# alex-petrenko/sample-factory

Hardware: AMD Instinct MI355X
Metric: env-steps/sec (whole node), 4096 envs, 84x84x4 obs (higher is better)
Workload: dtype f32

## Files before the change

### include/sf_hip.h

```cpp
#ifndef SF_HIP_H
#define SF_HIP_H

#include <stdint.h>

#ifdef __cplusplus
extern "C" {
#endif

#define SF_OK 0
#define SF_ERR_ARG (-1)
#define SF_ERR_LAUNCH (-2)
#define SF_ERR_UNSUPPORTED (-3)
#define SF_MAX_ACTION_HEADS 64

const char *sf_last_error(void);
int sf_abi_version(void);

int sf_valid_mask(const int32_t *policy_id, const float *policy_version, uint8_t *valids, uint8_t *valids_flat,
                  float *actions, int num_actions, float *log_prob_actions, int E, int T, int my_policy_id,
                  int train_step, int max_policy_lag, int32_t *num_invalid, void *stream);

int sf_gae_returns(float *rewards, const uint8_t *dones, const uint8_t *time_outs, const float *values,
                   const uint8_t *valids, const double *rms_stats, int E, int T, float gamma, float gae_lambda,
                   int value_bootstrap, float *advantages, float *returns, void *stream);
// ... 197 lines not shown
                       int R, int Cn, int H, int env_major, void *stream);

#define SF_DP_UNIQUE_ID_BYTES 128
int sf_dp_unique_id(void *out_id);
int sf_dp_comm_create(const void *id_bytes, int nranks, int rank, void **comm_out);
int sf_dp_comm_destroy(void *comm);
int sf_dp_comm_info(void *comm, int *nranks, int *rank);
int sf_allreduce_grads(void *comm, float *grads, int64_t n, void *stream);
int sf_dp_allreduce_f64(void *comm, double *buf, int64_t n, int op, void *stream);
int sf_dp_broadcast(void *comm, void *buf, int64_t nbytes, int root, void *stream);

#define SF_DP_IPC_HANDLE_BYTES 64
int sf_dp_oneshot_create(int nranks, int rank, int64_t max_bytes, void **ctx_out, void *handle_out);
int sf_dp_oneshot_connect(void *ctx, const void *all_handles );
int sf_dp_oneshot_allreduce_f32(void *ctx, float *buf, int64_t n, void *stream);
int sf_dp_oneshot_allreduce_f64(void *ctx, double *buf, int64_t n, int op, void *stream);
int sf_dp_oneshot_status(void *ctx);
int sf_dp_oneshot_destroy(void *ctx);

int sf_tanh_scale_fwd(float *x, int ld, int64_t n, int col0, int ncols, float scale, void *stream);
int sf_tanh_scale_bwd(float *g, const float *y, int ld, int64_t n, int col0, int ncols, float scale, void *stream);

int sf_linear_fwd_dual_supported(int64_t n, int N, int K1, int K2);
int sf_linear_fwd_dual(const float *a1, int64_t lda1, const float *w1t, const float *bias1, int K1, const float *a2,
                       int64_t lda2, const float *w2t, const float *bias2, int K2, float *out, int64_t n, int N,
                       int gru_H, void *stream);

int sf_conv_fwd_t_supported(int64_t n, const sf_conv_desc *desc);
int64_t sf_conv_fwd_t_workspace(int64_t n, const sf_conv_desc *desc);
int sf_conv_fwd_t(const float *in, int64_t in_sample_stride, const float *wt, const float *bias, float *out,
                  int64_t n, const sf_conv_desc *desc, void *workspace, int64_t workspace_bytes, void *stream);
int sf_transpose(const float *w, float *wt, int K, int N, void *stream);

int sf_conv_kernel_name(int op, int64_t n, const sf_conv_desc *desc, int split_k_allowed, char *out, int cap);
int sf_linear_fwd(const float *in, const float *w, const float *bias, float *out, int64_t M, int K, int N, int relu,
                  void *stream);
int64_t sf_linear_wgrad_workspace(int64_t M, int K, int N);
int sf_linear_wgrad(const float *in, const float *dout, float *dw, float *db, int64_t M, int K, int N,
                    void *workspace, void *stream);
int sf_linear_dgrad(const float *dout, const float *w, const float *in_act, float *din, int64_t M, int K, int N,
                    void *stream);
int sf_relu_mask(float *g, const float *act, int64_t n, void *stream);

typedef struct {
    int32_t Cin, H, W, Cout;
    int32_t in_u8;
    int32_t act_in;
    int32_t traj_T;
    float sub_mean, inv_scale;
} sf_res_desc;

int sf_res_conv_fwd(const void *in, int64_t in_sample_stride, const int32_t *index, int64_t offset, const float *w,
                    const float *bias, const float *residual, float *out, float *out_act, int act_out, int64_t n,
                    const sf_res_desc *h_desc, void *stream);
int sf_res_conv_fwd_norm(const void *in, int64_t in_sample_stride, const int32_t *index, int64_t offset, const float *mu,
                         const float *rstd, const float *w, const float *bias, float *out, int64_t n,
                         const sf_res_desc *h_desc, void *stream);
int sf_res_pool_fwd(const float *in, float *out, uint8_t *argmax, int64_t n, int H, int W, int C, void *stream);
int sf_res_pool_bwd(const float *dout, const uint8_t *argmax, float *din, int64_t n, int H, int W, int C, void *stream);
int sf_res_conv_dgrad(const float *dout, const float *w, const float *pre, const float *g_add, float *din, int64_t n,
                      const sf_res_desc *h_desc, void *stream);
int64_t sf_res_conv_wgrad_workspace(int64_t n, const sf_res_desc *h_desc);
int sf_res_conv_wgrad(const void *in, int64_t in_sample_stride, const int32_t *index, int64_t offset, const float *dout,
                      float *dw, float *db, int64_t n, const sf_res_desc *h_desc, void *workspace,
                      int64_t workspace_bytes, void *stream);
int sf_res_conv_wgrad_norm(const void *in, int64_t in_sample_stride, const int32_t *index, int64_t offset, const float *mu,
// ... 8 lines not shown
```

### sample_factory_amd/algo/learning/learner.py

```python
from __future__ import annotations

import glob
import time
import os
from os.path import join
from typing import Dict, List, Optional, Tuple

import numpy as np
import torch

from sample_factory_amd import lib
from sample_factory_amd.algo.learning.dp import ReplicaGroup
from sample_factory_amd.algo.utils.tensor_dict import TensorDict
from sample_factory_amd.envs.spaces import (action_head_sizes, calc_num_action_parameters, calc_num_actions, is_box,
                                             is_discrete)
from sample_factory_amd.model.actor_critic import ActorCritic
from sample_factory_amd.model.model_factory import create_actor_critic
from sample_factory_amd.utils.attr_dict import AttrDict
from sample_factory_amd.utils.decay import LinearDecay

LEARNER_ENV_STEPS, POLICY_ID_KEY, STATS_KEY, TRAIN_STATS = "learner_env_steps", "policy_id", "stats", "train"


class LearningRateScheduler:
# ... 81 lines not shown

    def init(self, actor_critic, policy_version, device):
        self.actor_critic, self.device = actor_critic, device
        self.policy_versions[self.policy_id] = policy_version


class Learner:
    def __init__(self, cfg, env_info, policy_versions_tensor: torch.Tensor, policy_id: int, param_server,
                 process_group=None):
        self.cfg = cfg
        self.env_info = env_info
        self.policy_id = policy_id
        self.policy_versions_tensor = policy_versions_tensor
        self.param_server = param_server
        self.device: Optional[torch.device] = None
        self.actor_critic: Optional[ActorCritic] = None
        self.curr_lr: Optional[float] = None
        self.lr_scheduler: Optional[LearningRateScheduler] = None
        self.train_step = 0
        self.env_steps = 0
        self.best_performance = -1e9
        self.new_cfg: Optional[Dict] = None
        self.policy_to_load = None
        self.is_initialized = False
        self.last_summary: Dict = {}
        self.pg = process_group
        dp_on = process_group is not None or (getattr(cfg, "data_parallel", False) and torch.distributed.is_initialized())
        self.group = ReplicaGroup(process_group, bool(getattr(cfg, "dp_force_collectives", False)),
                                  bool(getattr(cfg, "dp_native_rccl", False)),
                                  oneshot_bytes=int(getattr(cfg, "dp_oneshot_bytes", 0) or 0)) if dp_on else None
        self.world = self.group.world if self.group is not None else 1
        self.dp = self.group is not None and self.group.on
        self._grad_norms: List[float] = []

    def _all_reduce(self, t: torch.Tensor) -> None:
        if self.dp:
            self.group.all_reduce_sum(t)

    def init(self):
        cfg = self.cfg
        if cfg.exploration_loss not in ("entropy", "symmetric_kl"):
            raise NotImplementedError(f"{cfg.exploration_loss} not supported!")
        if cfg.optimizer not in ("adam", "lamb"):
            raise RuntimeError(f"Unknown optimizer {cfg.optimizer}")
        if cfg.seed is not None:
            torch.manual_seed(cfg.seed)
            np.random.seed(cfg.seed)
        if not torch.cuda.is_available():
            raise lib.SfHipError("Learner.init(): no GPU visible. sample_factory_amd has no CPU path.")
        lib.load()
        self.device = torch.device("cuda", torch.cuda.current_device())
        ar = self._all_reduce if self.dp else None
        cfg.dp_world = self.world
        self.actor_critic = create_actor_critic(cfg, self.env_info.obs_space, self.env_info.action_space, self.device,
                                                all_reduce=ar)
        self.actor_critic.train()
        if self.dp:
            self.group.broadcast(self.actor_critic.flat_params, src=0)
            self.actor_critic.params_changed()
        P = self.actor_critic.num_flat
        self.exp_avg = torch.zeros(P, dtype=torch.float32, device=self.device)
        self.exp_avg_sq = torch.zeros(P, dtype=torch.float32, device=self.device)
        self.adam_step_count = 0
        self._dp_reduce_each_mb = True
        self._dp_split = None
        ac_ = self.actor_critic
# ... 216 lines not shown
            idx = torch.empty(experience_size, dtype=torch.int32, device=self.device)
            if getattr(cfg, "device_shuffle", False):
                seed = (cfg.seed or 0) * 7919 + self.policy_id
                lib.minibatch_indices(idx, experience_size, cfg.recurrence, True, seed, self._shuffle_epoch)
                self._shuffle_epoch += 1
            else:
                starts = np.random.permutation(np.arange(0, experience_size, cfg.recurrence))
                starts_dev = torch.from_numpy(starts.astype(np.int32)).to(self.device, non_blocking=True)
                lib.minibatch_expand(starts_dev, idx, experience_size, cfg.recurrence)
            return [(idx[i * batch_size:(i + 1) * batch_size], 0, batch_size) for i in range(experience_size // batch_size)]
        return [(None, i * batch_size, batch_size) for i in range(n_mb)]

    _shuffle_epoch = 0

    def _calculate_losses(self, mb: AttrDict, num_invalids: int):
        from sample_factory_amd.algo.utils.action_distributions import get_action_distribution
        buff, part = (mb if isinstance(mb, tuple) else (mb, None))
        if part is None:
            part = (None, 0, buff.E * buff.T)
        acts, g_heads, sc = self._losses_native(buff, part, num_invalids)
        index, offset, n = part
        heads = acts[-1]
        A = self.num_action_params
        space = self.env_info.action_space
        dist = get_action_distribution(space, heads[:n, 1:1 + A])
        dist.raw_logits, dist.values = heads[:n, 1:1 + A], heads[:n, 0]
        rows = index.long() if index is not None else torch.arange(offset, offset + n, device=self.device)
        kl_old = dist.kl_divergence(get_action_distribution(space, buff.action_logits[rows]))[buff.valids[rows]]
        summaries = AttrDict(adv_mean=sc[6], adv_std=sc[7], num_valid=sc[8], entropy=sc[9], kl_divergence_max=sc[5],
                             kl_old_mean=sc[4].clone(), ratio=self._ratio[:n], values=heads[:n, 0], g_heads=g_heads)
        return dist, sc[0].clone(), sc[1].clone(), kl_old, sc[2].clone(), sc[3].clone(), summaries

    def _losses_native(self, buff: AttrDict, mb, num_invalids: int, scalars_out: Optional[torch.Tensor] = None,
                       moments: Optional[torch.Tensor] = None):
        cfg, ac = self.cfg, self.actor_critic
        index, offset, n = mb
        A = self.num_action_params
        rnn = None
        if cfg.use_rnn:
            R, Cn = cfg.recurrence, n // cfg.recurrence
            keep_tm = ac._buf(("rnn", "keep_tm"), (R, Cn))
            h0 = ac._buf(("rnn", "h0"), (Cn, buff.rnn_states.shape[-1]))
            lib.rnn_chunk_setup(buff.dones, buff.valids, buff.rnn_states, index, offset, Cn, R, keep_tm, h0, traj_T=buff.T)
            rnn = dict(R=R, h0=h0, keep_tm=keep_tm)
        acts = ac.forward_heads(buff.obs, n, sample_stride=ac.obs_elems, index=index, offset=offset,
                                traj_T=buff.T, tag="train", rnn=rnn)
        heads = acts[-1]
        ld = ac.heads_ld
        params, values = heads[:, 1:], heads[:, 0]
        g_heads = ac._zbuf(("g", "heads"), (n, ld))
        if cfg.with_vtrace:
            vs = ac._buf(("vt", "vs"), (n,))
            adv = ac._buf(("vt", "adv"), (n,))
            lib.vtrace(params, ld, values, ld, buff.actions, buff.log_prob_actions, buff.rewards, buff.dones, index,
                       offset, n, A, self.loss_cfg.action_kind, cfg.recurrence, cfg.gamma, cfg.vtrace_rho,
                       cfg.vtrace_c, vs, adv, head_sizes=self._head_sizes)
            lib.moments(adv, buff.valids, index, n, self._moments, offset=offset, dense_x=True)
            adv_arr, tgt_arr = adv, vs
        elif moments is None:
            lib.moments(buff.advantages, buff.valids, index, n, self._moments, offset=offset)
            adv_arr, tgt_arr = buff.advantages, buff.returns
        else:
            adv_arr, tgt_arr = buff.advantages, buff.returns
        if moments is None:
            moments = self._moments
            self._all_reduce(moments)
        self._ratio = ac._buf(("loss", "ratio"), (n,))
        self.loss_cfg.old_values_T = buff.T
        lib.ppo_loss(params, ld, values, ld, buff.actions, buff.log_prob_actions, buff.action_logits, buff["values"],
                     adv_arr, tgt_arr, buff.valids, index, offset, n, A, self.loss_cfg, moments, self._sums,
                     g_heads[:, 1:], g_heads[:, 0], ratio_out=self._ratio, head_sizes=self._head_sizes)
        self._last_mb = (index, offset, n, values, adv_arr)
        if self.dp and self._dp_reduce_each_mb:
            self.group.loss_sums(self._sums)
        out = scalars_out if scalars_out is not None else torch.zeros(16, dtype=torch.float32, device=self.device)
        lib.loss_scalars(self._sums, moments, self.loss_cfg, out)
        return acts, g_heads, out

    def _epoch_moments(self, buff: AttrDict, minibatches) -> Optional[torch.Tensor]:
# ... 1 lines not shown
            return None
        tab = self.actor_critic._buf(("loss", "epoch_moments"), (len(minibatches), 3), dtype=torch.float64)
        for i, (index, offset, n) in enumerate(minibatches):
            lib.moments(buff.advantages, buff.valids, index, n, tab[i], offset=offset)
        self._all_reduce(tab)
        return tab

    def _train(self, buff: AttrDict, batch_size: int, experience_size: int, num_invalids: int) -> Optional[AttrDict]:
        cfg, ac = self.cfg, self.actor_critic
        early_stopping_tolerance = 1e-6
        prev_epoch_actor_loss = 1e9
        recent_kls: List[float] = []
        num_sgd_steps = 0
        n_mb = cfg.num_batches_per_epoch
        self._scalars = ac._buf(("loss", "scalars"), (cfg.num_epochs * n_mb, 16))
        global_size = experience_size * self.world
        need_kl_each_mb = self.lr_scheduler.invoke_after_each_minibatch() and isinstance(self.lr_scheduler, KlAdaptiveScheduler)
        self._dp_reduce_each_mb = need_kl_each_mb
        lr_on_device = need_kl_each_mb and cfg.optimizer == "adam"
        if lr_on_device:
            if not hasattr(self, "_lr_dev"):
                self._lr_dev = torch.zeros(1, dtype=torch.float32, device=self.device)
            self._lr_dev.fill_(float(self.curr_lr))
        self._grad_norms = []
        skip = ac.rnn_abort_word() if hasattr(ac, "rnn_abort_word") else None
        if skip is not None:
            ac.rnn_abort_clear()
        for epoch in range(cfg.num_epochs):
            minibatches = self._get_minibatches(batch_size, experience_size)
            mom_tab = self._epoch_moments(buff, minibatches)
            for batch_num, mb in enumerate(minibatches):
                row = self._scalars[epoch * n_mb + batch_num]
                acts, g_heads, _ = self._losses_native(buff, mb, num_invalids, row,
                                                       moments=None if mom_tab is None else mom_tab[batch_num])
                index, offset, n = mb
                if self._dp_split is not None:
                    cut = ac._segs[self._dp_split][0]
                    pending = []
                    ac.backward(acts, g_heads, buff.obs, n, sample_stride=ac.obs_elems, index=index, offset=offset,
                                traj_T=buff.T,
                                on_layer_done=lambda li: pending.append(self.group.all_reduce_grads_async(
                                    ac.flat_grads[cut:])) if li == self._dp_split else None)
                    self.group.all_reduce_grads(ac.flat_grads[:cut])
                    for work in pending:
                        work.wait()
                else:
                    ac.backward(acts, g_heads, buff.obs, n, sample_stride=ac.obs_elems, index=index, offset=offset,
                                traj_T=buff.T)
                    if self.dp:
                        self.group.all_reduce_grads(ac.flat_grads)
                actual_lr = self.curr_lr
                valid_frac = 1.0
                if self._global_invalids > 0:
                    valid_frac = (global_size - self._global_invalids) / global_size
                    actual_lr = self.curr_lr * valid_frac
                self.adam_step_count += 1
                use_clip = cfg.max_grad_norm > 0.0
                if use_clip or getattr(cfg, "record_grad_norm", False):
                    lib.grad_sumsq(ac.flat_grads, self._sumsq)
                    if getattr(cfg, "record_grad_norm", False):
                        self._grad_norms.append(float(self._sumsq.sqrt().item()))
                if cfg.optimizer == "lamb":
                    if self._lamb is None:
                        seg, nseg = ac.tensor_segment_ids()
                        self._lamb = (seg, nseg, torch.empty_like(ac.flat_params),
                                      torch.zeros(128, dtype=torch.float64, device=self.device))
                    seg, nseg, scratch, seg_sums = self._lamb
# ... 110 lines not shown
```

### sample_factory_amd/algo/sampling/batched_sampling.py

```python
from __future__ import annotations

import ctypes as C
import time
from typing import Dict, Optional

import numpy as np
import torch

from sample_factory_amd import lib
from sample_factory_amd.algo.utils.tensor_dict import TensorDict
from sample_factory_amd.envs.spaces import action_head_sizes, heads_mixed, is_box, split_tuple_actions


class BatchedVectorEnvRunner:
    def __init__(self, cfg, env_info, env, actor_critic, traj: TensorDict, policy_id: int = 0,
                 policy_versions: Optional[torch.Tensor] = None, sample_seed: int = 0, row0: int = 0, tag: str = "inf"):
        self.cfg, self.env_info, self.env, self.ac = cfg, env_info, env, actor_critic
        self.tag = tag
        self.traj = traj
        self.policy_id = policy_id
        self.policy_versions = policy_versions
        self.B = env.num_agents
        self.T = cfg.rollout
        dev = actor_critic.device
# ... 4 lines not shown
        self.env_actions = torch.zeros((self.B, len(self.heads)) if len(self.heads) > 1 else self.B, dtype=torch.int32,
                                       device=dev)
        self.ep_return = torch.zeros(self.B, dtype=torch.float32, device=dev)
        self.ep_len = torch.zeros(self.B, dtype=torch.int32, device=dev)
        self.ep_stats = torch.zeros(3, dtype=torch.float64, device=dev)
        self.sample_seed = int(sample_seed)
        self.row0 = int(row0)
        self.global_step = 0
        self.obs_keys = sorted(k for k in traj["obs"].keys() if k != "action_mask")
        self.multi_key = len(self.obs_keys) > 1
        self.zero_copy = hasattr(env, "step_into") and not self.multi_key
        self.obs = traj["obs"]["obs" if "obs" in traj["obs"] else self.obs_keys[0]]
        self.rnn = actor_critic.rnn_kind is not None
        traj["rnn_states"].zero_()
        self._dummy_state_rows = {traj["rnn_states"].data_ptr()}
        self._started = False
        self.A = actor_critic.num_action_params
        self.ld = actor_critic.heads_ld
        self.continuous = is_box(self.env_info.action_space)
        self.host_env = None
        self.async_env = hasattr(env, "step_async") and hasattr(env, "step_wait")
        self._pin, self._pin_flip, self._direct_ok = {}, {}, {}
        self._act_event = torch.cuda.Event()
        self.h2d_bytes = 0
        self.ingest_prof: Optional[dict] = None
        self._rew = torch.zeros(self.B, dtype=torch.float32, device=dev)
        self._term = torch.zeros(self.B, dtype=torch.bool, device=dev)
        self._trunc = torch.zeros(self.B, dtype=torch.bool, device=dev)
        self._c_step, self._c_ver = C.c_uint32(0), C.c_float(0.0)
        self._progs: Dict = {}
        self._progs_layout = None
        self.program_replays = 0
        self._launch_key = getattr(actor_critic, "launch_key", None) if lib.LAUNCH_PROGRAMS else None
        self.masked = "action_mask" in traj["obs"]
        if self.masked and (self.continuous or len(self.heads) != 1):
            raise NotImplementedError("action masks are supported for a single Discrete action space")
        if self.masked and self.zero_copy:
            raise NotImplementedError("action masks with a zero-copy (step_into) env")

    def reset(self) -> None:
        if self.zero_copy:
            self.env.reset_into(self.obs[:, 0])
        else:
            o, _ = self.env.reset()
            first = (o["obs"] if "obs" in o else o[self.obs_keys[0]]) if isinstance(o, dict) else o
            self.host_env = not (isinstance(first, torch.Tensor) and first.is_cuda)
            self._store_obs(o, 0)
        self._started = True

    def _pinned(self, key, shape, dtype, nbuf=1):
        bufs = self._pin.get(key)
        if bufs is None or bufs[0].shape != torch.Size(shape) or bufs[0].dtype != dtype:
            bufs = [torch.empty(shape, dtype=dtype, pin_memory=True) for _ in range(nbuf)]
            self._pin[key] = bufs
        self._pin_flip[key] = (self._pin_flip.get(key, -1) + 1) % len(bufs)
        return bufs[self._pin_flip[key]]

    def _to_device(self, key, src, dst: torch.Tensor) -> None:
        if isinstance(src, torch.Tensor) and src.is_cuda:
            dst.copy_(src)
            return
        prof = self.ingest_prof
        t0 = time.perf_counter() if prof is not None else 0.0
        a = np.asarray(src.cpu() if isinstance(src, torch.Tensor) else src)
        stage = None
        if getattr(self.env, "pages_registered", False) and isinstance(src, np.ndarray) and src.flags.c_contiguous and \
# ... 59 lines not shown
        self.rollout_step_finish(t)

    def _program(self, half: str, t: int, extra=()):
        if self._launch_key is None:
            return None, None
        layout, weights = self._launch_key(self.tag)
        if layout != self._progs_layout:
            self._progs.clear()
            self._progs_layout = layout
        key = (half, t, self.traj["rewards"].data_ptr(), self._deterministic, torch.cuda.current_stream().cuda_stream,
               weights, extra)
        slot = self._progs.get(key)
        if slot is None:
            if len(self._progs) > 64 * self.T:
                self._progs.clear()
            self._progs[key] = False
            return None, None
        if slot is False:
            return None, key
        return (slot, None) if slot.unsafe is None else (None, None)

    def rollout_step_begin(self, t: int) -> None:
        self._c_step.value, self._c_ver.value = self.global_step & 0xFFFFFFFF, self._ver
        prog, rec_key = self._program("policy", t)
        if prog is not None:
            prog.replay()
            self.program_replays += 1
        elif rec_key is not None:
            with lib.record_launches() as prog:
                self._policy_and_sample(t)
            self._progs[rec_key] = prog
        else:
            self._policy_and_sample(t)
        tr = self.traj
        env_actions = tr["actions"][:, t] if (self.continuous or self.mixed) else self.env_actions
        if self.async_env:
            self.env.step_async(self._actions_to_host(env_actions))
            return
        self._env_step_and_record(t, env_actions)

    def _policy_and_sample(self, t: int) -> None:
        tr, T, B, A = self.traj, self.T, self.B, self.A
        ver, deterministic, cfg, step = self._c_ver, self._deterministic, self.cfg, self._c_step
        rnn = dict(states=tr["rnn_states"][:, t]) if self.rnn else None
        x = {k: tr["obs"][k][:, t] for k in self.obs_keys} if self.multi_key else self.obs[:, t]
        heads = self.ac.forward_heads(x, B, sample_stride=self.obs.stride(0), tag=self.tag, rnn=rnn)[-1]
        if self.masked:
            mk = tr["obs"]["action_mask"][:, t]
            lib.sample_write_step_masked(heads[:, 1:], self.ld, heads[:, 0], self.ld, mk, mk.stride(0), B, A, T, t,
                                         self.sample_seed, step, self.row0, ver, deterministic,
                                         tr["actions"], tr["action_logits"], tr["log_prob_actions"], tr["values"],
                                         tr["policy_version"], self.env_actions)
        elif len(self.heads) > 1:
            lib.sample_write_step_tuple(heads[:, 1:], self.ld, heads[:, 0], self.ld, B, self.heads, T, t,
                                        self.sample_seed, step, self.row0, ver, deterministic,
                                        tr["actions"], tr["action_logits"], tr["log_prob_actions"], tr["values"],
                                        tr["policy_version"], None if self.mixed else self.env_actions)
        else:
            lib.sample_write_step(heads[:, 1:], self.ld, heads[:, 0], self.ld, B, A, T, t, self.sample_seed,
                                  step, self.row0, ver, deterministic, tr["actions"],
                                  tr["action_logits"], tr["log_prob_actions"], tr["values"], tr["policy_version"],
                                  None if self.continuous else self.env_actions, action_kind=int(self.continuous))

    def rollout_step_finish(self, t: int) -> None:
        if self.async_env:
            self._env_step_and_record(t, None)

    def _env_step_and_record(self, t: int, env_actions) -> None:
        tr, T, cfg = self.traj, self.T, self.cfg
        if self.zero_copy:
            if self.mixed:
                env_actions = split_tuple_actions(env_actions, self.heads)
            rew, term, trunc = self.env.step_into(env_actions, self.obs[:, t + 1])
        else:
            if self.host_env is None:
                self.host_env = False
            t0 = time.perf_counter()
            if self.async_env:
                o, rew, term, trunc, _ = self.env.step_wait()
# ... 78 lines not shown
```

### sample_factory_amd/cfg/arguments.py

```python
from __future__ import annotations

import argparse
import os
from typing import List, Optional, Tuple


def _bool(v):
    if isinstance(v, bool):
        return v
    if v.lower() in ("true", "1", "yes", "y", "t"):
        return True
    if v.lower() in ("false", "0", "no", "n", "f"):
        return False
    raise argparse.ArgumentTypeError(f"boolean expected, got {v}")


FLAGS = [
    ("algo", str, "APPO"), ("env", str, None), ("experiment", str, "default_experiment"),
    ("train_dir", str, os.path.join(os.getcwd(), "train_dir")), ("restart_behavior", str, "resume"),
    ("device", str, "gpu"), ("seed", int, None),
    ("num_policies", int, 1), ("async_rl", _bool, True), ("serial_mode", _bool, False),
    ("batched_sampling", _bool, False), ("num_batches_to_accumulate", int, 2), ("worker_num_splits", int, 2),
    ("policy_workers_per_policy", int, 1), ("max_policy_lag", int, 1000),
    ("num_workers", int, 8), ("num_envs_per_worker", int, 2),
# ... 10 lines not shown
    ("lr_schedule_kl_threshold", float, 0.008), ("lr_adaptive_min", float, 1e-6), ("lr_adaptive_max", float, 1e-2),
    ("obs_subtract_mean", float, 0.0), ("obs_scale", float, 1.0), ("normalize_input", _bool, True),
    ("normalize_input_keys", str, None, "*"),
    ("decorrelate_experience_max_seconds", int, 0), ("decorrelate_envs_on_one_worker", _bool, True),
    ("actor_worker_gpus", int, [], "*"), ("set_workers_cpu_affinity", _bool, True),
    ("force_envs_single_thread", _bool, False), ("default_niceness", int, 0),
    ("log_to_file", _bool, True), ("experiment_summaries_interval", int, 10), ("flush_summaries_interval", int, 30),
    ("stats_avg", int, 100), ("summaries_use_frameskip", _bool, True), ("heartbeat_interval", int, 20),
    ("heartbeat_reporting_interval", int, 180),
    ("train_for_env_steps", int, int(1e10)), ("train_for_seconds", int, int(1e10)),
    ("save_every_sec", int, 120), ("keep_checkpoints", int, 2), ("load_checkpoint_kind", str, "latest"),
    ("save_milestones_sec", int, -1), ("save_best_every_sec", int, 5), ("save_best_metric", str, "reward"),
    ("save_best_after", int, 100000), ("benchmark", _bool, False),
    ("encoder_mlp_layers", int, [512, 512], "*"), ("encoder_conv_architecture", str, "convnet_simple"),
    ("encoder_conv_mlp_layers", int, [512], "*"), ("use_rnn", _bool, True), ("rnn_size", int, 512),
    ("rnn_type", str, "gru"), ("rnn_num_layers", int, 1), ("decoder_mlp_layers", int, [], "*"),
    ("nonlinearity", str, "elu"), ("policy_initialization", str, "orthogonal"), ("policy_init_gain", float, 1.0),
    ("actor_critic_share_weights", _bool, True), ("adaptive_stddev", _bool, True),
    ("continuous_tanh_scale", float, 0.0), ("initial_stddev", float, 1.0),
    ("use_env_info_cache", _bool, False), ("env_gpu_actions", _bool, False), ("env_gpu_observations", _bool, True),
    ("env_frameskip", int, 1), ("env_framestack", int, 1), ("pixel_format", str, "CHW"),
    ("use_record_episode_statistics", _bool, False), ("with_wandb", _bool, False), ("with_pbt", _bool, False),
    ("help", _bool, False),
]


ENGINE_FLAGS = [
    ("data_parallel", _bool, False),
    ("dp_overlap", _bool, True),
    ("dp_epoch_moments", _bool, True),
    ("dp_oneshot_bytes", int, 0),
    ("dp_native_rccl", _bool, False),
    ("dp_force_collectives", _bool, False),
    ("device_shuffle", _bool, False),
    ("sampler_thread", _bool, None),
    ("record_grad_norm", _bool, False),
    ("env_workers_mode", str, "auto"),
    ("env_worker_start_method", str, "spawn"),
]


def parse_sf_args(argv: Optional[List[str]] = None, evaluation: bool = False) -> Tuple[argparse.ArgumentParser, argparse.Namespace]:
    import sys

    if argv is None:
        argv = sys.argv[1:]
    p = argparse.ArgumentParser(formatter_class=argparse.ArgumentDefaultsHelpFormatter, add_help=False)
    for spec in FLAGS + ENGINE_FLAGS:
        name, typ, default = spec[:3]
        kw = dict(type=typ, default=default)
        if len(spec) > 3:
            kw["nargs"] = spec[3]
        p.add_argument(f"--{name}", **kw)
    if evaluation:
        p.add_argument("--max_num_episodes", type=int, default=int(1e9))
        p.add_argument("--max_num_frames", type=int, default=int(1e9))
        p.add_argument("--eval_deterministic", type=_bool, default=False)
        p.add_argument("--no_render", type=_bool, default=True)
        p.add_argument("--policy_index", type=int, default=0)
    args, _ = p.parse_known_args(argv)
    return p, args


def parse_full_cfg(parser: argparse.ArgumentParser, argv: Optional[List[str]] = None) -> argparse.Namespace:
    import sys

# ... 18 lines not shown
    return cfg


def preprocess_cfg(cfg, env_info) -> bool:
    if cfg.recurrence == -1:
        cfg.recurrence = cfg.rollout if cfg.use_rnn else 1
    return verify_cfg(cfg, env_info)


def verify_cfg(cfg, env_info) -> bool:
    ok = True

    def err(msg):
        nonlocal ok
        ok = False
        print(f"[sample_factory_amd] config error: {msg}")

    if cfg.num_policies != 1:
        err(f"{cfg.num_policies=}: this engine trains ONE policy per process group (multi-policy / PBT populations are "
            "outside the hot-path scope)")
    if cfg.num_envs_per_worker % cfg.worker_num_splits != 0:
        err(f"{cfg.num_envs_per_worker=} must be a multiple of {cfg.worker_num_splits=}"
            " (for double-buffered sampling you need to use even number of envs per worker)")
    if cfg.normalize_returns and cfg.with_vtrace:
        err("Normalized returns are not supported with vtrace!")
    if cfg.with_vtrace and not (cfg.recurrence == cfg.rollout and cfg.recurrence > 1):
        err("V-trace requires recurrence == rollout > 1")
    if cfg.rollout % cfg.recurrence != 0:
        err(f"{cfg.rollout=} must be a multiple of {cfg.recurrence=}")
    if cfg.batch_size % cfg.rollout != 0:
        err(f"{cfg.batch_size=} must be a multiple of {cfg.rollout=}")
    if cfg.use_rnn and cfg.recurrence <= 1:
        err("RNN policies need recurrence > 1")
    total_agents = cfg.num_workers * cfg.num_envs_per_worker * env_info.num_agents
    per_iter = cfg.num_batches_per_epoch * cfg.batch_size
    per_rollout = total_agents * cfg.rollout // cfg.num_policies
    if not cfg.async_rl and not (per_iter % per_rollout == 0 and per_iter >= per_rollout):
        err(f"sync mode needs batch_size*num_batches_per_epoch ({per_iter}) to be a multiple of "
            f"agents*rollout ({per_rollout})")
    return ok


def cfg_dict(cfg) -> dict:
    return dict(cfg) if isinstance(cfg, dict) else dict(vars(cfg))


def cfg_str(cfg) -> str:
    return "\n".join(f"{k}={v}" for k, v in cfg_dict(cfg).items())


def load_from_checkpoint(cfg):
    import json

    from sample_factory_amd.utils.attr_dict import AttrDict
    name = os.path.join(cfg.train_dir, cfg.experiment, "config.json")
    if not os.path.isfile(name):
        raise FileNotFoundError(f"Could not load saved parameters for experiment {cfg.experiment} (file {name} not found). "
                                "Check that you have the correct experiment name and --train_dir is set correctly.")
    with open(name) as f:
        loaded = AttrDict(json.load(f))
    for key, value in getattr(cfg, "cli_args", {}).items():
        if key in loaded and loaded[key] != value:
            loaded[key] = value
    for key, value in cfg_dict(cfg).items():
        if key not in loaded:
            loaded[key] = value
# ... 20 lines not shown
```

### sample_factory_amd/csrc/sf_nn.hip

```cpp
#include "sf_common.h"
#include <stdarg.h>
#include <stdlib.h>
#include <string.h>
#ifndef SF_GLDS_ABLATE
#define SF_GLDS_ABLATE 0
#endif
#include <type_traits>
#include <algorithm>

#define STREAM(s) reinterpret_cast<hipStream_t>(s)

typedef float f32x16 __attribute__((ext_vector_type(16)));

struct FastDiv {
    uint32_t d, mul, shr;
};
static inline FastDiv make_fastdiv(uint32_t d) {
    FastDiv f;
    f.d = d;
    if (d <= 1) { f.mul = 0; f.shr = 0; return f; }
    uint32_t s = 0;
    while ((1u << s) < d) ++s;
    f.mul = (uint32_t)((((uint64_t)1) << (31 + s)) / d + 1);
    f.shr = s - 1;
// ... 267 lines not shown
}

#define FRAG_ROW(r, lane) (((r) & 3) + 8 * ((r) >> 2) + 4 * ((lane) >> 5))

template <int KIND>
__device__ __forceinline__ float act_fwd_c(float x, int kind) {
    if (KIND == 0) return x;
    if (KIND == 1) return fmaxf(x, 0.f);
    return act_fwd(x, kind);
}

template <int TM, int TN, int KIND, bool FULL>
__device__ __forceinline__ void store_fwd_tile(const f32x16 (&acc)[TM][TN], float *__restrict__ ob, uint32_t voff, int N,
                                               int rows_left, int cols_left, const float *__restrict__ bias0, int lcol,
                                               int kind) {
#pragma unroll
    for (int tn = 0; tn < TN; ++tn) {
        const bool cok = FULL || tn * 32 < cols_left;
        const float bv = (bias0 && cok) ? bias0[tn * 32 + lcol] : 0.f;
#pragma unroll
        for (int tm = 0; tm < TM; ++tm)
#pragma unroll
            for (int r = 0; r < 16; ++r) {
                const int rr = tm * 32 + (r & 3) + 8 * (r >> 2);
                float *p = ob + (int64_t)rr * N + tn * 32;
                const float v = act_fwd_c<KIND>(acc[tm][tn][r] + bv, kind);
#if SF_GLDS_ABLATE & 4
                if (v == 1.2345e30f) p[voff] = v;
#else
                if (FULL || (cok && rr < rows_left)) p[voff] = v;
#endif
            }
    }
}

template <int TM, int TN, int KIND, bool FULL>
__device__ __forceinline__ void store_dgrad_tile(const f32x16 (&acc)[TM][TN], float *__restrict__ ob,
                                                 const float *__restrict__ mk, uint32_t voff, int N, int rows_left,
                                                 int cols_left, int kind) {
#pragma unroll
    for (int tn = 0; tn < TN; ++tn) {
        const bool cok = FULL || tn * 32 < cols_left;
#pragma unroll
        for (int tm = 0; tm < TM; ++tm) {
            float y[16];
#pragma unroll
            for (int r = 0; r < 16; ++r) {
                const int rr = tm * 32 + (r & 3) + 8 * (r >> 2);
                const bool ok = FULL || (cok && rr < rows_left);
                y[r] = (KIND != 0 && ok) ? (mk + (int64_t)rr * N + tn * 32)[voff] : 1.f;
            }
#pragma unroll
            for (int r = 0; r < 16; ++r) {
                const int rr = tm * 32 + (r & 3) + 8 * (r >> 2);
                const float v = act_bwd_mul<KIND>(acc[tm][tn][r], y[r], kind);
                if (FULL || (cok && rr < rows_left)) (ob + (int64_t)rr * N + tn * 32)[voff] = v;
            }
        }
    }
}


template <int BM, int BN, int WM, int WN>
struct Tile {
    static constexpr int TM = BM / WM / 32, TN = BN / WN / 32;
    static constexpr int SA = BM / 32, SB = BN / 32;
// ... 476 lines not shown
};
struct TileArgs { int BM, BN, WM, WN; };
struct ConvPlan {
    int kernel;
    char name[64];
    TileArgs t;
    int variant;
    dim3 grid, block;
    unsigned lds;
    int splits;
    int64_t per_split;
    int partials;
    int rx, ry, rtot;
    int main_tiles;
    QuadrowClasses qr;
    bool recommended;
};
static ConvPlan plan_init() {
    ConvPlan p{};
    p.block = dim3(256); p.splits = p.partials = 1;
    return p;
}
static void plan_kernel(ConvPlan &p, int kernel, const char *fmt, ...) {
    p.kernel = kernel;
    va_list ap;
    va_start(ap, fmt);
    vsnprintf(p.name, sizeof(p.name), fmt, ap);
    va_end(ap);
}
static void plan_tile(ConvPlan &p, int kernel, const char *base, TileArgs t, const char *tail = "") {
    p.t = t;
    plan_kernel(p, kernel, "%s<%d, %d, %d, %d%s>", base, t.BM, t.BN, t.WM, t.WN, tail);
}
static void plan_raster(ConvPlan &p, bool on) {
    p.rx = (int)p.grid.x; p.ry = (int)p.grid.y;
    p.rtot = on ? (int)(p.grid.x * p.grid.y * p.grid.z) : 0;
    if (p.rtot > 0) p.grid = dim3((unsigned)(8 * ((p.rtot + 7) / 8)), 1, 1);
}

struct Operands {
    const void *in;
    int64_t stride;
    bool index;
    const void *w, *dout, *out;
    int64_t ws_floats;
};
static Operands query_operands(const sf_conv_desc *d, bool split_k_workspace) {
    return Operands{nullptr, (int64_t)d->H * d->W * d->Cin, false, nullptr, nullptr, nullptr, split_k_workspace ? (int64_t)1 << 60 : 0};
}
static bool aligned(const void *p, uintptr_t a) { return ((uintptr_t)p & (a - 1)) == 0; }
static const float TABLE_PROBE[4] __attribute__((aligned(16))) = {0.f, 0.f, 0.f, 0.f};

static int pick_mode(const ConvG &g) {
    if (!g.vecA || !g.vecB) return MODE_GENERIC;
    if (in_is_u8(g.in_u8)) return g.nmu ? MODE_U8_NORM : MODE_U8;
    if (g.in_u8 == IN_F32_FRAME) return g.nmu ? MODE_F32F_NORM : MODE_F32F;
    return MODE_F32;
}

static bool act_aligned(const ConvG &g, const void *in, int64_t in_sample_stride) {
    return aligned(in, in_is_u8(g.in_u8) ? 4 : 16) && in_sample_stride % 4 == 0 && aligned(g.nmu, 16) && aligned(g.nrstd, 16);
}

static bool in4(const Operands &o) { return aligned(o.in, 4) && o.stride % 4 == 0; }
static bool tabs16(const ConvG &g) { return aligned(g.nmu, 16) && aligned(g.nrstd, 16); }

// ... 93 lines not shown
    const FwdPlan p = plan_fwd(Mtot, N, K, (int64_t)1 << 60);
    return p.splits > 1 ? (int64_t)sizeof(float) * p.splits * Mtot * N + 256 : 0;
}

#define TILE_IS(BM_, BN_) (p.t.BM == BM_ && p.t.BN == BN_)
static void launch_splitk_finish(const float *partial, const float *bias, float *out, int64_t MN, const ConvG &g, int Z, hipStream_t st) {
    k_splitk_finish<<<dim3(cdiv64(MN, 256) < 4096 ? cdiv64(MN, 256) : 4096), dim3(256), 0, st>>>(partial, bias, out, MN, g.Cout, Z, g.relu);
}
#define BY_MODE(L, ...)                                                          \
    switch (p.variant) {                                                         \
        case MODE_F32: L(__VA_ARGS__, MODE_F32); break;                          \
        case MODE_U8: L(__VA_ARGS__, MODE_U8); break;                            \
        case MODE_F32F: L(__VA_ARGS__, MODE_F32F); break;                        \
        case MODE_F32F_NORM: L(__VA_ARGS__, MODE_F32F_NORM); break;              \
        case MODE_U8_NORM: L(__VA_ARGS__, MODE_U8_NORM); break;                  \
        default: L(__VA_ARGS__, MODE_GENERIC);                                   \
    }
#define FWD_LAUNCH(BM, BN, WM, WN, MODE)                          \
    k_conv_fwd<BM, BN, WM, WN, MODE><<<p.grid, p.block, 0, st>>>( \
        g, in, in_sample_stride, index, offset, w, bias, out, Mtot, (int)p.per_split, partial)

static bool relu_mask_ok(const sf_conv_desc *d, int64_t n) {
    if (!sw().relu_mask || !in_is_u8(d->in_u8) || d->relu != 1 || d->Cout != 32) return false;
    const int k = plan_conv_fwd(d, make_geom(d), n, query_operands(d, false)).kernel;
    return k == K_CONV1_U8_BF16 || k == K_CONV1_U8_BF16_W;
}
extern "C" int sf_conv_relu_mask_supported(int64_t n, const sf_conv_desc *h_desc) {
    return h_desc && n > 0 && check_desc(h_desc, "sf_conv_relu_mask_supported") == 0 && relu_mask_ok(h_desc, n) ? 1 : 0;
}

static int conv_fwd_impl(const void *in, int64_t in_sample_stride, const int32_t *index, int64_t offset, const float *w,
                         const float *bias, float *out, uint32_t *relu_mask, int64_t n, const sf_conv_desc *h_desc,
                         void *workspace, int64_t workspace_bytes, void *stream, const float *mu = nullptr,
                         const float *rstd = nullptr) {
    int rc = check_desc(h_desc, "sf_conv_fwd");
    if (rc) return rc;
    SF_REQUIRE(in && w && out && n > 0, "sf_conv_fwd: bad args");
    SF_REQUIRE(((uintptr_t)workspace & 15) == 0, "sf_conv_fwd: workspace must be 16-byte aligned");
    ConvG g = make_geom(h_desc);
    g.nmu = mu; g.nrstd = rstd;
    const int64_t Mtot = n * g.OH * g.OW;
    SF_REQUIRE(Mtot < (1LL << 31), "sf_conv_fwd: M=%lld exceeds 2^31 rows; split the batch", (long long)Mtot);
    const Operands o = {in, in_sample_stride, index != nullptr, w, nullptr, out, workspace ? workspace_bytes / (int64_t)sizeof(float) : 0};
    const ConvPlan p = plan_conv_fwd(h_desc, g, n, o);
    hipStream_t st = STREAM(stream);
    const bool bf16 = p.kernel == K_CONV1_U8_BF16 || p.kernel == K_CONV1_U8_BF16_W;
    SF_REQUIRE(relu_mask == nullptr || bf16,
               "sf_conv_fwd_relu_mask: operands not eligible for the sign-bit kernel (sf_conv_relu_mask_supported, 4-byte "
               "aligned frames and sample stride, 16-byte aligned weights)");
    if (bf16 && sw().debug_occ) {
        const unsigned img_bytes = 2u * 4u * 20u * (unsigned)SF_CONV1_WP * (unsigned)sizeof(uint16_t);
        fprintf(stderr, "k_conv1_u8_bf16 occupancy: %d (dword stores, %u B LDS) / %d (whole-line stores, %u B LDS) work-groups per CU\n",
                occupancy_of(k_conv1_u8_bf16<false>, 256, img_bytes), img_bytes,
                occupancy_of(k_conv1_u8_bf16_w<false>, 256, img_bytes + 2u * 80u * 36u * 4u), img_bytes + 2u * 80u * 36u * 4u);
    }
    const uint8_t *in8 = reinterpret_cast<const uint8_t *>(in);
    float *partial = p.splits > 1 ? reinterpret_cast<float *>(workspace) : nullptr;
#define CONV1_LAUNCH(KERN, ...) \
    KERN<<<p.grid, p.block, p.lds, st>>>(g, in8, in_sample_stride, index, offset, w, bias, out, ##__VA_ARGS__, (int)n)
    switch (p.kernel) {
        case K_CONV1_U8_BF16_W:
            if (p.variant) CONV1_LAUNCH(k_conv1_u8_bf16_w<true>, relu_mask); else CONV1_LAUNCH(k_conv1_u8_bf16_w<false>, relu_mask);
            break;
        case K_CONV1_U8_BF16:
            if (p.variant) CONV1_LAUNCH(k_conv1_u8_bf16<true>, relu_mask); else CONV1_LAUNCH(k_conv1_u8_bf16<false>, relu_mask);
            break;
        case K_CONV_U8_IMG:
            if (p.variant) CONV1_LAUNCH((k_conv_u8_img<2, 4, 5, 16, true>)); else CONV1_LAUNCH((k_conv_u8_img<2, 4, 5, 16, false>));
            break;
        default:
            if (TILE_IS(256, 32)) { BY_MODE(FWD_LAUNCH, 256, 32, 4, 1) }
            else if (TILE_IS(128, 32)) { BY_MODE(FWD_LAUNCH, 128, 32, 4, 1) }
            else if (TILE_IS(128, 64)) { BY_MODE(FWD_LAUNCH, 128, 64, 2, 2) }
            else { BY_MODE(FWD_LAUNCH, 64, 64, 2, 2) }
            if (partial) launch_splitk_finish(partial, bias, out, Mtot * g.Cout, g, p.splits, st);
    }
#undef CONV1_LAUNCH
    return sf_launch_status("sf_conv_fwd");
}

extern "C" int sf_conv_fwd(const void *in, int64_t in_sample_stride, const int32_t *index, int64_t offset,
                           const float *w, const float *bias, float *out, int64_t n, const sf_conv_desc *h_desc,
                           void *workspace, int64_t workspace_bytes, void *stream) {
    return conv_fwd_impl(in, in_sample_stride, index, offset, w, bias, out, nullptr, n, h_desc, workspace, workspace_bytes,
                         stream);
}
extern "C" int sf_conv_fwd_relu_mask(const void *in, int64_t in_sample_stride, const int32_t *index, int64_t offset,
                                     const float *w, const float *bias, float *out, uint32_t *relu_mask, int64_t n,
                                     const sf_conv_desc *h_desc, void *stream) {
    SF_REQUIRE(relu_mask && ((uintptr_t)relu_mask & 3) == 0, "sf_conv_fwd_relu_mask: relu_mask must be a 4-byte aligned device buffer");
    SF_REQUIRE(h_desc && n > 0 && relu_mask_ok(h_desc, n) && ((uintptr_t)in & 3) == 0 && in_sample_stride % 4 == 0,
               "sf_conv_fwd_relu_mask: unsupported layer / launch (see sf_conv_relu_mask_supported)");
    return conv_fwd_impl(in, in_sample_stride, index, offset, w, bias, out, relu_mask, n, h_desc, nullptr, 0, stream);
}

#ifndef SF_IMG_TMF
#define SF_IMG_TMF 2
#endif
#define IMG_FWD_GEOMS(X) X(64, 9, 9, 3, 1, SF_IMG_TMF, 1, 7)
static int plan_img_fwd(ConvPlan &p, const ConvG &g, int64_t n) {
    if (!sw().fwd_img || g.Cout != 64 || g.KH != g.KW || n < 512) return -1;
    int idx = 0;
#define X(CIN, HH, WW, KS, ST, TMF, WS, R)                                                                         \
    if (g.Cin == CIN && g.H == HH && g.W == WW && g.KH == KS && g.S == ST) {                                       \
        static const int bpc = occupancy_of(k_fwd_img<CIN, HH, WW, KS, ST, TMF, WS, R>, 256 * WS);                 \
        p.variant = idx; p.grid = dim3(num_cus() * (bpc > 0 ? bpc : 1)); p.block = dim3(256 * WS);                 \
        plan_kernel(p, K_FWD_IMG, "k_fwd_img<%d, %d, %d, %d, %d, %d, %d, %d>", CIN, HH, WW, KS, ST, TMF, WS, R);   \
        return idx;                                                                                                \
    }                                                                                                              \
    ++idx;
    IMG_FWD_GEOMS(X)
#undef X
    return -1;
}

static bool glds_fwd_ok(const sf_conv_desc *d) {
    return d->in_u8 == IN_F32_NHWC && d->Cin % 32 == 0 && d->traj_T == 0;
}
struct GldsFwdPlan {
    bool ok, wide, sq64;
    int Z, k_per_split;
};
static int split_k(int K, int64_t want, int64_t tiles, int *k_per_split) {
    int z = (int)((want + tiles - 1) / tiles);
    z = z > K / 256 ? K / 256 : z;
    z = z > 16 ? 16 : z;
    if (z <= 1) return 1;
    *k_per_split = (((K + 31) / 32 + z - 1) / z) * 32;
    return (K + *k_per_split - 1) / *k_per_split;
}
static GldsFwdPlan plan_fwd_t(int64_t Mtot, int N, int K) {
    const Switches &s = sw();
    static const int occ64 = occupancy_of(k_fwd_glds<128, 64, 2, 2, 2>), occ128 = occupancy_of(k_fwd_glds<128, 128, 2, 2, 2>);
    GldsFwdPlan p;
// ... 15 lines not shown
        return p;
    }
    if (s.glds_fc64 == 1 && N >= 128 && K >= 1024 && cdiv64(Mtot, 64) * (int64_t)cdiv64(N, 64) >= 512) {
        p.ok = true; p.sq64 = true;
        return p;
    }
    const int64_t t6464 = cdiv64(Mtot, 64) * (int64_t)cdiv64(N, 64);
    if (s.glds_split64 && s.glds_splitk && N >= 128 && K >= 1024 && t6464 >= s.glds_split64 && t6464 < 512) {
        p.Z = split_k(K, 512, t6464, &p.k_per_split);
        if (p.Z > 1) { p.ok = true; p.sq64 = true; return p; }
    }
    if (s.glds_splitk && N >= 128 && K >= 1024 && t128 >= 32) {
        p.Z = split_k(K, 256 * occ128, t128, &p.k_per_split);
        p.ok = p.wide = p.Z > 1;
    }
    return p;
}
static bool linear_1x1(const sf_conv_desc *d) {
    return d->in_u8 == IN_F32_NHWC && d->traj_T == 0 && d->KH == 1 && d->KW == 1 && d->H == 1 && d->W == 1;
}
static bool small_linear_wgrad_ok(const sf_conv_desc *d) {
    return sw().linear_narrow && linear_1x1(d) && d->Cout <= 64 && d->Cin <= 64;
}
static bool narrow_fwd_ok(const sf_conv_desc *d, int64_t n) {
    return sw().linear_narrow && linear_1x1(d) && d->Cout <= 32 && d->Cin % 16 == 0 && n < (1 << 30);
}
static int fwd_tail_split(const ConvG &g, int64_t Mtot, int Z, bool zl_ok) {
    if (!sw().glds_tailsplit || !zl_ok || sw().glds_zl < 1 || Z != 1 || g.Cout > 64 || sw().xcd_rows) return 0;
    static const int occ = occupancy_of(k_fwd_glds_zt<128, 64, 2, 2>, 256, (128 + 64) * 32 * 2 * sizeof(float));
    const int64_t tiles = cdiv64(Mtot, 128), resident = (int64_t)num_cus() * occ, tail = tiles % resident;
    if (tiles <= resident || tail == 0 || 2 * tail > resident) return (int)tiles;
    return (int)(tiles - tail);
}
static ConvPlan plan_conv_fwd_t(const sf_conv_desc *d, int64_t n, int64_t in_sample_stride, ConvG *g_out = nullptr) {
    ConvPlan p = plan_init();
    if (narrow_fwd_ok(d, n)) {
        p.recommended = true; p.variant = d->Cout <= 16 ? 1 : 2;
        p.grid = dim3((unsigned)cdiv64(n, 16)); p.block = dim3(64);
        plan_kernel(p, K_LINEAR_NARROW, "k_linear_narrow<%d>", p.variant);
        return p;
    }
    if (!glds_fwd_ok(d)) return p;
    const ConvG g = make_geom(d);
    if (g_out) *g_out = g;
    const int64_t Mtot = n * g.OH * g.OW;
    if (n * in_sample_stride < ((int64_t)1 << 40) && plan_img_fwd(p, g, n) >= 0) { p.recommended = true; return p; }
    GldsFwdPlan q = plan_fwd_t(Mtot, g.Cout, g.K);
    p.recommended = q.ok;
    if (!q.ok) { q.Z = 1; q.k_per_split = (g.K + 31) / 32 * 32; }
    p.splits = q.Z; p.per_split = q.k_per_split;
    const bool zl_ok = sw().glds_zl && (n - 1) * in_sample_stride + (int64_t)g.H * g.W * g.Cin < (1LL << 30) &&
                       (int64_t)g.Cout * g.K < (1LL << 30);
    const bool col64 = !q.sq64 && !q.wide && q.Z == 1 && g.Cout <= 64 && zl_ok;
    if (sw().glds_persist && col64) {
        static const int occp = occupancy_of(k_fwd_glds_zp<128, 64, 2, 2>);
        const int64_t tiles = cdiv64(Mtot, 128), slots = (int64_t)num_cus() * occp;
        p.grid = dim3((unsigned)(tiles < slots ? tiles : slots));
        plan_tile(p, K_FWD_GLDS_ZP, "k_fwd_glds_zp", TileArgs{128, 64, 2, 2});
        return p;
    }
    if (sw().glds_tall && col64 && cdiv64(Mtot, 256) >= (unsigned)sw().glds_tall) {
        p.grid = dim3(cdiv64(Mtot, 256), 1, 1);
        plan_tile(p, K_FWD_GLDS_Z, "k_fwd_glds_z", TileArgs{256, 64, 4, 1});
        return p;
    }
    if (!q.sq64 && !q.wide) {
        p.main_tiles = fwd_tail_split(g, Mtot, q.Z, zl_ok);
        if (p.main_tiles > 0) {
            const int tail = (int)cdiv64(Mtot, 128) - p.main_tiles;
            p.grid = dim3((unsigned)(p.main_tiles + 2 * tail));
            p.lds = (128 + 64) * 32 * 2 * sizeof(float);
            plan_tile(p, K_FWD_GLDS_ZT, "k_fwd_glds_zt", TileArgs{128, 64, 2, 2});
            return p;
        }
    }
    const TileArgs t = q.sq64 ? TileArgs{64, 64, 2, 2} : q.wide ? TileArgs{128, 128, 2, 2} : TileArgs{128, 64, 2, 2};
    p.grid = dim3(cdiv64(Mtot, t.BM), cdiv64(g.Cout, t.BN), (unsigned)q.Z);
    plan_raster(p, sw().xcd_raster && (p.grid.y > 1 || (sw().xcd_rows && p.grid.x >= 64)));
    if (zl_ok && ((t.BM / t.WM / 32) * (t.BN / t.WN / 32) <= 2 || sw().glds_zl >= 2)) plan_tile(p, K_FWD_GLDS_Z, "k_fwd_glds_z", t);
    else plan_tile(p, K_FWD_GLDS, "k_fwd_glds", t, ", 2");
    return p;
}
extern "C" int sf_conv_fwd_t_supported(int64_t n, const sf_conv_desc *h_desc) {
    return h_desc && n > 0 && plan_conv_fwd_t(h_desc, n, query_operands(h_desc, false).stride).recommended ? 1 : 0;
}
extern "C" int64_t sf_conv_fwd_t_workspace(int64_t n, const sf_conv_desc *h_desc) {
// ... 34 lines not shown
        SF_REQUIRE(workspace && ((uintptr_t)workspace & 15) == 0 &&
                       workspace_bytes >= (int64_t)sizeof(float) * p.splits * Mtot * g.Cout,
                   "sf_conv_fwd_t: this launch is split along K and needs sf_conv_fwd_t_workspace() bytes of workspace");
        partial = reinterpret_cast<float *>(workspace);
    }
    switch (p.kernel) {
        case K_FWD_IMG: {
            int idx = 0;
#define X(CIN, HH, WW, KS, ST, TMF, WS, R)                                                                           \
    if (p.variant == idx++) {                                                                                        \
        if (sw().debug_img) fprintf(stderr, "k_fwd_img R=%d: %d work-groups per CU\n", R, (int)p.grid.x / num_cus()); \
        k_fwd_img<CIN, HH, WW, KS, ST, TMF, WS, R><<<p.grid, p.block, 0, st>>>(in, in_sample_stride, wt, bias, out, (int)n, g.relu); \
    }
            IMG_FWD_GEOMS(X)
#undef X
            break;
        }
        case K_FWD_GLDS_ZP:
            k_fwd_glds_zp<128, 64, 2, 2><<<p.grid, p.block, 0, st>>>(g, in, in_sample_stride, wt, bias, out, Mtot, (int)p.per_split);
            break;
        case K_FWD_GLDS_ZT:
            k_fwd_glds_zt<128, 64, 2, 2><<<p.grid, p.block, p.lds, st>>>(g, in, in_sample_stride, wt, bias, out, Mtot, (int)p.per_split,
                                                                          p.main_tiles, sw().tap_perm);
            break;
        default:
            if (TILE_IS(256, 64)) k_fwd_glds_z<256, 64, 4, 1><<<p.grid, p.block, 0, st>>>(GLDS_FWD_ARGS);
            else if (TILE_IS(64, 64)) GLDS_FWD(64, 64, 2, 2);
            else if (TILE_IS(128, 128)) GLDS_FWD(128, 128, 2, 2);
            else GLDS_FWD(128, 64, 2, 2);
    }
    if (partial) launch_splitk_finish(partial, bias, out, Mtot * g.Cout, g, p.splits, st);
    return sf_launch_status("sf_conv_fwd_t");
}
extern "C" int sf_linear_fwd_dual_supported(int64_t n, int N, int K1, int K2) {
    return sw().linear_dual && n > 0 && N >= 64 && K1 > 0 && K2 > 0 && K1 % 32 == 0 && K2 % 32 == 0 && n < (1LL << 31) &&
           cdiv64(n, 128) * (int64_t)cdiv64(N, 64) >= 256;
}
extern "C" int sf_linear_fwd_dual(const float *a1, int64_t lda1, const float *w1t, const float *bias1, int K1,
                                  const float *a2, int64_t lda2, const float *w2t, const float *bias2, int K2, float *out,
                                  int64_t n, int N, int gru_H, void *stream) {
    SF_REQUIRE(a1 && w1t && a2 && w2t && out && n > 0 && N > 0, "sf_linear_fwd_dual: bad args");
    SF_REQUIRE(K1 > 0 && K2 > 0 && K1 % 32 == 0 && K2 % 32 == 0 && lda1 % 4 == 0 && lda2 % 4 == 0 && n < (1LL << 31),
               "sf_linear_fwd_dual: K1, K2 must be multiples of 32 and the row strides multiples of 4 (K1=%d K2=%d)", K1, K2);
    SF_REQUIRE((((uintptr_t)a1 | (uintptr_t)a2 | (uintptr_t)w1t | (uintptr_t)w2t) & 15) == 0,
               "sf_linear_fwd_dual: operands must be 16-byte aligned");
    SF_REQUIRE(gru_H == 0 || (gru_H > 0 && gru_H % 64 == 0 && N == 4 * gru_H),
               "sf_linear_fwd_dual: the GRU column layout needs N == 4 * gru_H and gru_H %% 64 == 0 (N=%d gru_H=%d)", N, gru_H);
    k_fwd_glds2<128, 64, 2, 2><<<dim3(cdiv64(n, 128), cdiv64(N, 64)), dim3(256), 0, STREAM(stream)>>>(
        a1, lda1, w1t, bias1, K1, a2, lda2, w2t, bias2, K2, out, n, N, gru_H);
    return sf_launch_status("sf_linear_fwd_dual");
}
extern "C" int sf_transpose(const float *w, float *wt, int K, int N, void *stream) {
    SF_REQUIRE(w && wt && K > 0 && N > 0, "sf_transpose: bad args");
    k_transpose<<<dim3(cdiv64(K, 32), cdiv64(N, 32)), dim3(256), 0, STREAM(stream)>>>(w, wt, K, N);
    return sf_launch_status("sf_transpose");
}

struct SplitPlan {
    int Z;
    int64_t m_per_split;
};
static SplitPlan plan_splits(int64_t Mtot, int K, int N, int BM, int BN, int bpc = 0) {
    const int64_t tiles = (int64_t)((K + BM - 1) / BM) * ((N + BN - 1) / BN);
    const int64_t chunks = (Mtot + 31) / 32;
    int64_t zcap = (2304 + tiles - 1) / tiles;
    const int64_t zmax = (chunks + 7) / 8;
// ... 392 lines not shown
            if (TILE_IS(128, 128)) DGRAD_LINEAR(128, 128); else DGRAD_LINEAR(64, 64);
            break;
        }
#define QUADROW_ARGS g, dout, w, in_act, din, p.qr
        case K_DGRAD_QUADROW_Z: k_dgrad_quadrow_z<128, 128, 2, 2><<<p.grid, p.block, 0, st>>>(QUADROW_ARGS); break;
        case K_DGRAD_QUADROW: k_dgrad_quadrow<128, 128, 2, 2><<<p.grid, p.block, 0, st>>>(QUADROW_ARGS); break;
#undef QUADROW_ARGS
        case K_DGRAD_PIX:
        case K_DGRAD_PIX_Z:
            if (TILE_IS(128, 32)) DGRAD_PIX(128, 32, 4, 1);
            else if (TILE_IS(256, 32)) DGRAD_PIX(256, 32, 4, 1);
            else DGRAD_PIX(128, 64, 2, 2);
            break;
        default:
            if (TILE_IS(128, 32)) DGRAD_LAUNCH(128, 32, 4, 1);
            else if (TILE_IS(64, 64)) DGRAD_LAUNCH(64, 64, 2, 2);
            else DGRAD_LAUNCH(128, 64, 2, 2);
    }
    return sf_launch_status("sf_conv_dgrad");
}

#if SF_CONV1_TRACE
extern "C" int sf_debug_conv1_trace(unsigned long long *host_out12) {
    hipDeviceSynchronize();
    if (hipMemcpyFromSymbol(host_out12, HIP_SYMBOL(sf_conv1_trace_acc), 12 * sizeof(unsigned long long)) != hipSuccess) return 1;
    unsigned long long z[12] = {0, 0, 0, 0, 0, 0, 0, 0, 0, 0, 0, 0};
    return hipMemcpyToSymbol(HIP_SYMBOL(sf_conv1_trace_acc), z, sizeof(z)) == hipSuccess ? 0 : 1;
}
#endif
extern "C" int sf_conv_kernel_name(int op, int64_t n, const sf_conv_desc *h_desc, int split_k_allowed, char *out,
                                   int cap) {
    int rc = check_desc(h_desc, "sf_conv_kernel_name");
    if (rc) return rc;
    SF_REQUIRE(out && cap >= 48 && n > 0 && op >= 0 && op <= 5, "sf_conv_kernel_name: bad args");
    const Operands o = query_operands(h_desc, split_k_allowed != 0);
    ConvG g = make_geom(h_desc);
    if (op >= 4) g.nmu = g.nrstd = TABLE_PROBE;
    const ConvPlan p = op == 3 ? plan_conv_fwd_t(h_desc, n, o.stride) : op == 2 ? plan_conv_dgrad(g, n, o)
                       : (op == 0 || op == 4) ? plan_conv_fwd(h_desc, g, n, o) : plan_conv_wgrad(h_desc, g, n, o);
    SF_REQUIRE(p.kernel != K_NONE, "sf_conv_kernel_name: not a launch %s accepts",
               op >= 4 ? "sf_conv_norm_supported" : "sf_conv_fwd_t");
    strncpy(out, p.name, (size_t)cap - 1);
    out[cap - 1] = 0;
    return SF_OK;
}

static sf_conv_desc linear_desc(int K, int N, int relu) {
    sf_conv_desc d;
    d.Cin = K; d.H = 1; d.W = 1; d.Cout = N; d.KH = 1; d.KW = 1; d.stride = 1; d.OH = 1; d.OW = 1;
    d.in_u8 = 0; d.relu = relu; d.traj_T = 0; d.sub_mean = 0.f; d.inv_scale = 1.f;
    return d;
}

extern "C" int sf_linear_fwd(const float *in, const float *w, const float *bias, float *out, int64_t M, int K, int N,
                             int relu, void *stream) {
    SF_REQUIRE(M > 0 && K > 0 && N > 0, "sf_linear_fwd: bad shape");
    const sf_conv_desc d = linear_desc(K, N, relu);
    return sf_conv_fwd(in, K, nullptr, 0, w, bias, out, M, &d, nullptr, 0, stream);
}
extern "C" int64_t sf_linear_wgrad_workspace(int64_t M, int K, int N) {
    const sf_conv_desc d = linear_desc(K, N, 0);
    return sf_conv_wgrad_workspace(M, &d);
}
extern "C" int sf_linear_wgrad(const float *in, const float *dout, float *dw, float *db, int64_t M, int K, int N,
                               void *workspace, void *stream) {
    SF_REQUIRE(M > 0 && K > 0 && N > 0, "sf_linear_wgrad: bad shape");
    const sf_conv_desc d = linear_desc(K, N, 0);
    return sf_conv_wgrad(in, K, nullptr, 0, dout, dw, db, M, &d, workspace, stream);
}
extern "C" int sf_linear_dgrad(const float *dout, const float *w, const float *in_act, float *din, int64_t M, int K,
                               int N, void *stream) {
    SF_REQUIRE(M > 0 && K > 0 && N > 0, "sf_linear_dgrad: bad shape");
    const sf_conv_desc d = linear_desc(K, N, in_act ? 1 : 0);
    return sf_conv_dgrad(dout, w, in_act, din, M, &d, stream);
// ... 10 lines not shown
```

### sample_factory_amd/csrc/sf_nn_glds.h

```cpp
#pragma once

#ifndef SF_GLDS_ABLATE
#define SF_GLDS_ABLATE 0
#endif
#define GLDS16(gsrc, ldst)                                                                       \
    __builtin_amdgcn_global_load_lds((const __attribute__((address_space(1))) void *)(gsrc),    \
                                     (__attribute__((address_space(3))) void *)(ldst), 16, 0, 0)

#define BARRIER_NOFENCE()                  \
    do {                                   \
        asm volatile("" ::: "memory");     \
        __builtin_amdgcn_s_barrier();      \
        asm volatile("" ::: "memory");     \
    } while (0)

template <int TM, int TN>
__device__ __forceinline__ void mma_chunk_rows(const float *__restrict__ As, const float *__restrict__ Bs, int arow0,
                                               int brow0, int lane, f32x16 (&acc)[TM][TN]) {
    const int r = lane & 31, h = lane >> 5, sw = (r >> 1) & 7;
    const float *ap = As + (arow0 + r) * 32, *bp = Bs + (brow0 + r) * 32;
#pragma unroll
    for (int c = 0; c < 4; ++c) {
        const int pos = (((2 * c + h) ^ sw) << 2);
        float4 a[TM], b[TN];
// ... 178 lines not shown
            __builtin_amdgcn_sched_barrier(0);
        }
        if (c == 3 && SF_FRAG_DB_SINK == 2 * PER) __builtin_amdgcn_sched_barrier(0);
        mfmas(c, 2);
        if (c == 3 && SF_FRAG_DB_SINK == PER) __builtin_amdgcn_sched_barrier(0);
        mfmas(c, 3);
        if (c == 0) hook(HookPt<3>{});
        if (c == 3 && SF_FRAG_DB_SINK == 0) __builtin_amdgcn_sched_barrier(0);
    }
}

#ifndef SF_PIX_INCR
#define SF_PIX_INCR 1
#endif
#ifndef SF_PIX_LDSIMM
#define SF_PIX_LDSIMM 1
#endif
#ifndef SF_QUADROW_ROT
#define SF_QUADROW_ROT 0
#endif
#ifndef SF_QUADROW_PREP
#define SF_QUADROW_PREP 1
#endif
#ifndef SF_DGRAD_PIX_ZL_LITE
#define SF_DGRAD_PIX_ZL_LITE 1
#endif
template <int TM, int TN, int STAGE_F>
__device__ __forceinline__ void mma_chunk_stage(const float *const (&ap)[4], const float *const (&bp)[4], int stage,
                                                f32x16 (&acc)[TM][TN]) {
    if (stage == 0) mma_chunk_ptrs<TM, TN, 0>(ap, bp, acc);
    else mma_chunk_ptrs<TM, TN, STAGE_F>(ap, bp, acc);
}

template <int BM, int BN, int WM, int WN, int NS, bool ZL, bool PERSIST = false, bool DYNLDS = false>
__device__ __forceinline__ void fwd_glds_body(ConvG g, const float *__restrict__ in, int64_t in_stride,
                                              const float *__restrict__ wt, const float *__restrict__ bias,
                                              float *__restrict__ out, int64_t Mtot, int k_per_split,
                                              float *__restrict__ partial, const float *__restrict__ dmask,
                                              int dmask_on, int rx, int ry, int rtot, int tap_perm, int bx_shift = 0) {
    constexpr int TM = BM / WM / 32, TN = BN / WN / 32;
    constexpr int AI = BM / 32, BI = BN / 32;
    constexpr int STAGE = (BM + BN) * 32;
    static_assert(WM * WN == 4 && TM >= 1 && TN >= 1 && (NS == 2 || NS == 3), "4 waves per block");
    __shared__ __attribute__((aligned(1024))) float lds_static[DYNLDS ? 1 : NS * STAGE];
    extern __shared__ __attribute__((aligned(1024))) float lds_dynamic[];
    float *const lds = DYNLDS ? lds_dynamic : lds_static;
    const int tid = threadIdx.x, lane = tid & 63, wave = __builtin_amdgcn_readfirstlane(tid >> 6);
    const int wm = wave / WN, wn = wave % WN;
    const int ptiles = PERSIST ? (int)((Mtot + BM - 1) / BM) : 1;
    for (int ptile = PERSIST ? (int)blockIdx.x : 0; ptile < ptiles; ptile += PERSIST ? (int)gridDim.x : 1) {
    int bx = PERSIST ? ptile : (int)blockIdx.x + bx_shift, by = blockIdx.y, bz = blockIdx.z;
    if (rtot > 0) {
        const int per = (rtot + 7) >> 3, L = (int)(blockIdx.x & 7u) * per + (int)(blockIdx.x >> 3);
        if (L >= rtot) return;
        by = L % ry;
        const int t = L / ry;
        bx = t % rx;
        bz = t / rx;
    }
    const int64_t m0 = (int64_t)bx * BM;
    const int n0 = by * BN;
    const int N = g.Cout, K = g.K;
    const int kbeg = bz * k_per_split, kend = min(K, kbeg + k_per_split);

    const int lrow = lane >> 3, lpos = lane & 7;
    const float *asrc[AI], *bsrc[BI];
#pragma unroll
    for (int i = 0; i < AI; ++i) {
        const int row = (i * 4 + wave) * 8 + lrow;
        int64_t m = m0 + row;
        m = m < Mtot ? m : Mtot - 1;
        const uint32_t smp = fdiv((uint32_t)m, g.dOHOW), pix = (uint32_t)m - smp * (uint32_t)(g.OH * g.OW);
// ... 25 lines not shown
        for (int i = 0; i < BI; ++i) GLDS16(bsrc[i] + k0, sb + (i * 4 + wave) * 256);
    };
    static_assert(NS == 2, "two LDS stages");
    const bool tapperm = tap_perm && g.KH == 4 && g.KW == 4 && g.S == 2 && g.Cin == 32 && kbeg == 0 && kend == K;
    auto kord = [&](int k0) {
        if (!tapperm) return k0;
        const int p = k0 >> 5, grp = p >> 2, e = p & 3;
        const int kh = ((grp >> 1) & 1) + 2 * (e >> 1), kw = (grp & 1) + 2 * (e & 1);
        return (kh * 4 + kw) << 5;
    };
    int stage = 0, k0 = kbeg;
    constexpr bool MASK_PRE = ZL && TM * TN == 4;
    float mpre[MASK_PRE ? TM : 1][MASK_PRE ? TN : 1][16];
    bool mask_pre = false;
    auto prefetch_mask = [&]() {
        if constexpr (MASK_PRE) {
            if (dmask_on && dmask && g.relu == 1 && m0 + BM <= Mtot && n0 + BN <= N) {
                const float *mk = dmask + (m0 + wm * TM * 32) * N + (n0 + wn * TN * 32);
                const uint32_t vo = (uint32_t)(4 * (lane >> 5)) * (uint32_t)N + (uint32_t)(lane & 31);
#pragma unroll
                for (int tm = 0; tm < TM; ++tm)
#pragma unroll
                    for (int tn = 0; tn < TN; ++tn)
#pragma unroll
                        for (int r = 0; r < 16; ++r)
                            mpre[tm][tn][r] = (mk + (int64_t)(tm * 32 + (r & 3) + 8 * (r >> 2)) * N + tn * 32)[vo];
                mask_pre = true;
            }
        }
    };
    if constexpr (ZL) {

        uint32_t avoff[AI], bvoff[BI];
#pragma unroll
        for (int i = 0; i < AI; ++i) avoff[i] = (uint32_t)((asrc[i] - in) * (int64_t)sizeof(float));
#pragma unroll
        for (int i = 0; i < BI; ++i) bvoff[i] = (uint32_t)((bsrc[i] - wt) * (int64_t)sizeof(float));
        const uint32_t lds0 = (uint32_t)(uintptr_t)(__attribute__((address_space(3))) float *)lds;
        const int r = lane & 31, h = lane >> 5, sw = (r >> 1) & 7;
        const float *apl[4], *bpl[4];
#pragma unroll
        for (int c = 0; c < 4; ++c) {
            const int pos = (((2 * c + h) ^ sw) << 2);
            apl[c] = lds + (wm * TM * 32 + r) * 32 + pos;
            bpl[c] = lds + BM * 32 + (wn * TN * 32 + r) * 32 + pos;
        }
        auto chunk_off = [&](int kn) {
            const uint32_t tap = fdiv((uint32_t)kn, g.dCin), c0 = (uint32_t)kn - tap * (uint32_t)g.Cin;
            const uint32_t kh = fdiv(tap, g.dKW), kw = tap - kh * (uint32_t)g.KW;
            return (int)((kh * (uint32_t)g.W + kw) * (uint32_t)g.Cin + c0);
        };
        auto dma = [&](int q, const float *abase, const float *bbase, int st) {
            if (q < AI) glds16_s(abase, avoff[q < AI ? q : 0], lds0 + (uint32_t)((st * STAGE + (q * 4 + wave) * 256) * 4));
            else glds16_s(bbase, bvoff[q >= AI ? q - AI : 0], lds0 + (uint32_t)((st * STAGE + BM * 32 + ((q - AI) * 4 + wave) * 256) * 4));
        };
        {
            const int kf = kord(kbeg);
            const float *ab = in + chunk_off(kf), *bb = wt + kf;
#pragma unroll
            for (int q = 0; q < AI + BI; ++q) dma(q, ab, bb, 0);
        }
        auto step = [&](auto stc, bool prefetch) {
            constexpr int ST = decltype(stc)::value;
            asm volatile("s_waitcnt vmcnt(0)" ::: "memory");
            BARRIER_NOFENCE();
            const int kn = prefetch ? kord(k0 + 32) : 0;
            const float *ab = in + chunk_off(kn), *bb = wt + kn;
            if (!prefetch) prefetch_mask();
            if constexpr (TM * TN <= 2) {
                mma_chunk_ptrs_mid<TM, TN, ST * STAGE>(apl, bpl, acc, [&](int c) {
                    constexpr int TOT = AI + BI, PER = (TOT + 2) / 3;
                    if (prefetch) {
#pragma unroll
                        for (int q = 0; q < TOT; ++q)
                            if (q / PER == c) dma(q, ab, bb, ST ^ 1);
                    }
                });
            } else {
                auto burst = [&](int qlo, int qhi) {
                    if (prefetch) {
#pragma unroll
                        for (int q = 0; q < AI + BI; ++q)
                            if (q >= qlo && q < qhi) dma(q, ab, bb, ST ^ 1);
                    }
                };
                if constexpr (SF_FWD_FRAG_DB >= 2) {
                    mma_chunk_ptrs_db<TM, TN, ST * STAGE, false, SF_FWD_FRAG_DB == 3>(apl, bpl, acc, [&](auto pt) {
                        constexpr int P = decltype(pt)::value, HALF = (AI + BI) / 2;
                        if constexpr (SF_FWD_FRAG_DB == 2) {
                            if constexpr (P == 0) burst(0, AI + BI);
                        } else {
                            if constexpr (P == 1) burst(0, HALF);
                            if constexpr (P == 2) burst(HALF, AI + BI);
                        }
                    });
                } else {
                    burst(0, AI + BI);
                    if constexpr (SF_FWD_FRAG_DB == 1) mma_chunk_ptrs_db<TM, TN, ST * STAGE>(apl, bpl, acc, [](auto) {});
                    else mma_chunk_ptrs<TM, TN, ST * STAGE>(apl, bpl, acc);
                }
// ... 25 lines not shown
            float *na = lds + (stage ^ 1) * STAGE, *nb = na + BM * 32;
            const float *sa = lds + stage * STAGE;
            mma_chunk_rows_mid<TM, TN>(sa, sa + BM * 32, wm * TM * 32, wn * TN * 32, lane, acc, [&](int c) {
                constexpr int TOT = AI + BI, PER = (TOT + 2) / 3;
#pragma unroll
                for (int q = 0; q < TOT; ++q) {
                    if (q / PER != c || (SF_GLDS_ABLATE & 1)) continue;
                    if (q < AI) GLDS16(asrc[q < AI ? q : 0] + aoff, na + (q * 4 + wave) * 256);
                    else GLDS16(bsrc[q >= AI ? q - AI : 0] + kn, nb + ((q - AI) * 4 + wave) * 256);
                }
            });
        }
    } else {
        for (; k0 + 32 < kend; k0 += 32, stage ^= 1) {
            asm volatile("s_waitcnt vmcnt(0)" ::: "memory");
            BARRIER_NOFENCE();
            issue(k0 + 32, stage ^ 1);
            const float *sa = lds + stage * STAGE;
            mma_chunk_rows<TM, TN>(sa, sa + BM * 32, wm * TM * 32, wn * TN * 32, lane, acc);
        }
    }
    asm volatile("s_waitcnt vmcnt(0)" ::: "memory");
    BARRIER_NOFENCE();
    {
        const float *sa = lds + stage * STAGE;
        mma_chunk_rows<TM, TN>(sa, sa + BM * 32, wm * TM * 32, wn * TN * 32, lane, acc);
    }
    }
    float *ob = (partial ? partial + (int64_t)bz * Mtot * N : out) + (m0 + wm * TM * 32) * N + (n0 + wn * TN * 32);
    const int rows_left = (int)min((int64_t)(TM * 32), Mtot - m0 - wm * TM * 32) - 4 * (lane >> 5);
    const int cols_left = N - (n0 + wn * TN * 32) - (lane & 31);
    const uint32_t voff = (uint32_t)(4 * (lane >> 5)) * (uint32_t)N + (uint32_t)(lane & 31);
    const bool full = m0 + BM <= Mtot && n0 + BN <= N;
    if (dmask_on) {
        const float *mk = dmask ? dmask + (m0 + wm * TM * 32) * N + (n0 + wn * TN * 32) : nullptr;
        if (!dmask) {
            if (full) store_dgrad_tile<TM, TN, 0, true>(acc, ob, mk, voff, N, rows_left, cols_left, 0);
            else store_dgrad_tile<TM, TN, 0, false>(acc, ob, mk, voff, N, rows_left, cols_left, 0);
        } else if (MASK_PRE && mask_pre) {
#pragma unroll
            for (int tn = 0; tn < TN; ++tn)
#pragma unroll
                for (int tm = 0; tm < TM; ++tm)
#pragma unroll
                    for (int r = 0; r < 16; ++r) {
                        const int rr = tm * 32 + (r & 3) + 8 * (r >> 2);
                        (ob + (int64_t)rr * N + tn * 32)[voff] = act_bwd_mul<1>(acc[tm][tn][r], mpre[MASK_PRE ? tm : 0][MASK_PRE ? tn : 0][r], 1);
                    }
        } else if (g.relu == 1) {
            if (full) store_dgrad_tile<TM, TN, 1, true>(acc, ob, mk, voff, N, rows_left, cols_left, 1);
            else store_dgrad_tile<TM, TN, 1, false>(acc, ob, mk, voff, N, rows_left, cols_left, 1);
        } else {
            store_dgrad_tile<TM, TN, -1, false>(acc, ob, mk, voff, N, rows_left, cols_left, g.relu);
        }
    } else if (partial) {
        if (full) store_fwd_tile<TM, TN, 0, true>(acc, ob, voff, N, rows_left, cols_left, nullptr, lane & 31, 0);
        else store_fwd_tile<TM, TN, 0, false>(acc, ob, voff, N, rows_left, cols_left, nullptr, lane & 31, 0);
    } else if (g.relu == 1) {
        if (full) store_fwd_tile<TM, TN, 1, true>(acc, ob, voff, N, rows_left, cols_left, bias ? bias + n0 + wn * TN * 32 : nullptr, lane & 31, 1);
        else store_fwd_tile<TM, TN, 1, false>(acc, ob, voff, N, rows_left, cols_left, bias ? bias + n0 + wn * TN * 32 : nullptr, lane & 31, 1);
    } else {
        store_fwd_tile<TM, TN, -1, false>(acc, ob, voff, N, rows_left, cols_left, bias ? bias + n0 + wn * TN * 32 : nullptr, lane & 31, g.relu);
    }
    if (PERSIST) BARRIER_NOFENCE();
    }
}

template <int BM, int BN, int WM, int WN, int NS>
__global__ __launch_bounds__(256) void k_fwd_glds(ConvG g, const float *__restrict__ in, int64_t in_stride,
                                                  const float *__restrict__ wt, const float *__restrict__ bias,
                                                  float *__restrict__ out, int64_t Mtot, int k_per_split,
                                                  float *__restrict__ partial, const float *__restrict__ dmask,
                                                  int dmask_on, int rx = 0, int ry = 0, int rtot = 0, int tap_perm = 0) {
    fwd_glds_body<BM, BN, WM, WN, NS, false>(g, in, in_stride, wt, bias, out, Mtot, k_per_split, partial, dmask, dmask_on, rx,
                                             ry, rtot, tap_perm);
}
template <int BM, int BN, int WM, int WN>
__global__ __launch_bounds__(256, 2) void k_fwd_glds_zp(ConvG g, const float *__restrict__ in, int64_t in_stride,
                                                       const float *__restrict__ wt, const float *__restrict__ bias,
                                                       float *__restrict__ out, int64_t Mtot, int k_per_split) {
    fwd_glds_body<BM, BN, WM, WN, 2, true, true>(g, in, in_stride, wt, bias, out, Mtot, k_per_split, nullptr, nullptr, 0, 0, 0, 0, 0);
}
template <int BM, int BN, int WM, int WN>
__global__ __launch_bounds__(256, 2) void k_fwd_glds_zt(ConvG g, const float *__restrict__ in, int64_t in_stride,
                                                       const float *__restrict__ wt, const float *__restrict__ bias,
                                                       float *__restrict__ out, int64_t Mtot, int k_per_split, int main_tiles,
                                                       int tap_perm) {
    if ((int)blockIdx.x < main_tiles)
        fwd_glds_body<BM, BN, WM, WN, 2, true, false, true>(g, in, in_stride, wt, bias, out, Mtot, k_per_split, nullptr, nullptr, 0,
                                                            0, 0, 0, tap_perm);
    else
        fwd_glds_body<BM / 2, BN, WM, WN, 2, true, false, true>(g, in, in_stride, wt, bias, out, Mtot, k_per_split, nullptr,
                                                                nullptr, 0, 0, 0, 0, tap_perm, main_tiles);
}
template <int BM, int BN, int WM, int WN>
__global__ __launch_bounds__(256, 2) void k_fwd_glds_z(ConvG g, const float *__restrict__ in, int64_t in_stride,
                                                    const float *__restrict__ wt, const float *__restrict__ bias,
                                                    float *__restrict__ out, int64_t Mtot, int k_per_split,
                                                    float *__restrict__ partial, const float *__restrict__ dmask,
                                                    int dmask_on, int rx = 0, int ry = 0, int rtot = 0, int tap_perm = 0) {
    fwd_glds_body<BM, BN, WM, WN, 2, true>(g, in, in_stride, wt, bias, out, Mtot, k_per_split, partial, dmask, dmask_on, rx, ry,
                                           rtot, tap_perm);
}

template <int BM, int BN, int WM, int WN>
__global__ __launch_bounds__(256) void k_fwd_glds2(const float *__restrict__ a1, int64_t lda1, const float *__restrict__ w1t,
                                                   const float *__restrict__ bias1, int K1, const float *__restrict__ a2,
                                                   int64_t lda2, const float *__restrict__ w2t,
                                                   const float *__restrict__ bias2, int K2, float *__restrict__ out,
                                                   int64_t Mtot, int N, int gru_H) {
    constexpr int TM = BM / WM / 32, TN = BN / WN / 32;
    constexpr int AI = BM / 32, BI = BN / 32;
    constexpr int STAGE = (BM + BN) * 32;
    static_assert(WM * WN == 4 && TM >= 1 && TN >= 1, "4 waves per block");
    __shared__ __attribute__((aligned(1024))) float lds[2 * STAGE];
    const int tid = threadIdx.x, lane = tid & 63, wave = __builtin_amdgcn_readfirstlane(tid >> 6);
    const int wm = wave / WN, wn = wave % WN;
    const int64_t m0 = (int64_t)blockIdx.x * BM;
    const int n0 = blockIdx.y * BN;
    const bool use1 = gru_H == 0 || n0 < 3 * gru_H, use2 = gru_H == 0 || n0 < 2 * gru_H || n0 >= 3 * gru_H;
    const int row2_off = (gru_H > 0 && n0 >= 3 * gru_H) ? -gru_H : 0;
    const int kbeg = use1 ? 0 : K1, K = use2 ? K1 + K2 : K1;
    const int lrow = lane >> 3, lpos = lane & 7;
    const float *as1[AI], *as2[AI], *bs1[BI], *bs2[BI];
#pragma unroll
    for (int i = 0; i < AI; ++i) {
// ... 1291 lines not shown
```

### sample_factory_amd/csrc/sf_nn_img.h

```cpp
#pragma once

#ifndef SF_IMG_FLIP
#define SF_IMG_FLIP 1
#endif
#ifndef SF_IMG_PRIO
#define SF_IMG_PRIO 0
#endif
#ifndef SF_IMG_HALFSTEP
#define SF_IMG_HALFSTEP 1
#endif
template <int CIN, int H, int W, int KS, int ST, int TMF, int WSETS, int R>
struct ImgFwdGeom {
    static constexpr int OH = (H - KS) / ST + 1, OW = (W - KS) / ST + 1, OHW = R * OW;
    static constexpr int U = OH / R, HU = (R - 1) * ST + KS;
    static constexpr int K = KS * KS * CIN, KG = K / 16;
    static constexpr int C4 = CIN / 4, WQ = W / ST;
    static constexpr int PLANE_USED = ST * HU * WQ;
    static constexpr int PLANE = SF_IMG_FLIP ? (PLANE_USED + 15) / 16 * 16 : PLANE_USED;
    static constexpr int IMG_CH = C4 * PLANE;
    static constexpr int IMG_B = (IMG_CH * 16 + 1023) / 1024 * 1024;
    static constexpr int BROWS = WSETS * TMF * 16;
    static constexpr int RING = (2 * BROWS - 2) / OHW + 2;
    static_assert(CIN % 16 == 0 && W % ST == 0 && K % 16 == 0 && OH % R == 0, "geometry");
    static_assert(RING * IMG_B <= 160 * 1024, "LDS");
};

template <int CIN, int H, int W, int KS, int ST, int TMF, int WSETS, int R>
__global__ __launch_bounds__(256 * WSETS, 1) void k_fwd_img(const float *__restrict__ in, int64_t in_stride,
                                                    const float *__restrict__ wt, const float *__restrict__ bias,
                                                    float *__restrict__ out, int nsamples, int act) {
    typedef ImgFwdGeom<CIN, H, W, KS, ST, TMF, WSETS, R> G;
    constexpr int NW = 4 * WSETS, TB = TMF * WSETS;
    constexpr int OW = G::OW, OHW = G::OHW, K = G::K, KG = G::KG, WQ = G::WQ, PLANE = G::PLANE, RING = G::RING;
    constexpr int IMG_B = G::IMG_B, N = 64, U = G::U, HU = G::HU;
    __shared__ __attribute__((aligned(1024))) char ring[RING * IMG_B];
    const int tid = threadIdx.x, lane = tid & 63, wave = __builtin_amdgcn_readfirstlane(tid >> 6);
    const int col = lane & 15, kg = lane >> 4, n = (wave & 3) * 16 + col, wset = wave >> 2;
#if SF_IMG_PRIO
    if (__builtin_amdgcn_s_getreg((3 << 11) | (0 << 6) | 4) & 1u) __builtin_amdgcn_s_setprio(SF_IMG_PRIO);
#endif
    const int nunits = nsamples * U;
    const int64_t Mtot = (int64_t)nunits * OHW;
    const int total_frags = (int)((Mtot + 15) >> 4);
    const int per = (total_frags + (int)gridDim.x - 1) / (int)gridDim.x;
    const int f_beg = (int)blockIdx.x * per, f_end = min(total_frags, f_beg + per);
    if (f_beg >= f_end) return;
    f32x4 breg[KG];
#pragma unroll
    for (int g = 0; g < KG; ++g)
        breg[g] = *reinterpret_cast<const f32x4 *>(__builtin_assume_aligned(wt + (int64_t)n * K + 16 * g + 4 * kg, 16));
    const float bv = bias ? bias[n] : 0.f;

    constexpr int NDMA = IMG_B / 1024, NI = (NDMA + NW - 1) / NW;
    int srcoff[NI];
#pragma unroll
    for (int j = 0; j < NI; ++j) {
        int q = (wave + NW * j) * 64 + lane;
        q = q < G::IMG_CH ? q : 0;
        const int c = q / PLANE;
        int r0 = q - c * PLANE;
        r0 = r0 < G::PLANE_USED ? r0 : 0;
        const int pw = r0 / (HU * WQ), r1 = r0 - pw * (HU * WQ);
        const int ihl = r1 / WQ, iwq = r1 - ihl * WQ;
        const int ih = SF_IMG_FLIP ? HU - 1 - ihl : ihl;
        srcoff[j] = (ih * W + iwq * ST + pw) * CIN + c * 4;
    }
    auto load_image = [&](int s) {
        const int u = s < nunits ? s : nunits - 1, smp = u / U, strip = u - smp * U;
        const float *img = in + (int64_t)smp * in_stride + strip * (R * ST * W * CIN);
        char *dst = ring + (s % RING) * IMG_B;
#pragma unroll
        for (int j = 0; j < NI; ++j)
            if (wave + NW * j < NDMA) GLDS16(img + srcoff[j], dst + (wave + NW * j) * 1024);
    };
    const uint32_t M32 = (uint32_t)Mtot;
    auto last_sample = [&](int fb, int nf) {
        uint32_t m = (uint32_t)(fb + nf) * 16u - 1u;
        m = m < M32 ? m : M32 - 1u;
        return (int)(m / (uint32_t)OHW);
    };
    int loaded = (int)(((uint32_t)f_beg * 16u) / (uint32_t)OHW);
    {
        const int hi = last_sample(f_beg, min(TB, f_end - f_beg));
        for (; loaded <= hi; ++loaded) load_image(loaded);
    }
    f32x4 pend[TMF];
    int pend_fb = -1, pend_nf = 0;
    auto store_pend = [&]() {
        float *ob = out + ((int64_t)pend_fb * 16 + 4 * kg) * N + n;
        const int rows_left = (int)(M32 - ((uint32_t)pend_fb * 16u + 4u * (uint32_t)kg));
#pragma unroll
        for (int f = 0; f < TMF; ++f)
#pragma unroll
            for (int r = 0; r < 4; ++r)
                if (f < pend_nf && f * 16 + r < rows_left) ob[(f * 16 + r) * N] = pend[f][r];
    };
    for (int fb0 = f_beg; fb0 < f_end; fb0 += TB) {
        const int fb = fb0 + wset * TMF;
        const int nf = max(0, min(TMF, f_end - fb));
        asm volatile("s_waitcnt vmcnt(0)" ::: "memory");
        __syncthreads();
        if (fb0 + TB < f_end) {
            const int hi = last_sample(fb0 + TB, min(TB, f_end - fb0 - TB));
            for (; loaded <= hi; ++loaded) load_image(loaded);
        }
        if (pend_fb >= 0) store_pend();
        int base[TMF];
#pragma unroll
        for (int f = 0; f < TMF; ++f) {
            uint32_t m = (uint32_t)(nf > 0 ? fb + (f < nf ? f : 0) : fb0) * 16u + (uint32_t)col;
            m = m < M32 ? m : M32 - 1u;
            const uint32_t s = m / (uint32_t)OHW, p = m - s * (uint32_t)OHW, oh = p / (uint32_t)OW, ow = p - oh * (uint32_t)OW;
            const uint32_t prow = SF_IMG_FLIP ? ((uint32_t)(R - 1) - oh) * ST : oh * ST;
            base[f] = (int)((s % (uint32_t)RING) * (uint32_t)IMG_B + ((uint32_t)kg * PLANE + prow * WQ + ow) * 16u);
        }
        auto compute = [&](auto nfc) {
        constexpr int NF = decltype(nfc)::value;
        f32x4 acc[NF];
#pragma unroll
        for (int f = 0; f < NF; ++f) acc[f] = f32x4{0.f, 0.f, 0.f, 0.f};
        static_assert(KG % 2 == 0, "k-groups come in pairs");
// ... 13 lines not shown
                    acc[f] = __builtin_amdgcn_mfma_f32_16x16x4f32(a[slot][g & 1][f][j], breg[g][j], acc[f], 0, 0, 0);
        };
        fetch(0, 0);
        fetch(1, 0);
#pragma unroll
        for (int gp = 0; gp < KG / 2; ++gp) {
            mfmas(2 * gp, gp & 1);
            __builtin_amdgcn_sched_barrier(0);
            if (gp + 1 < KG / 2) {
                fetch(2 * gp + 2, (gp + 1) & 1);
                fetch(2 * gp + 3, (gp + 1) & 1);
            }
            __builtin_amdgcn_sched_barrier(0);
            mfmas(2 * gp + 1, gp & 1);
            __builtin_amdgcn_sched_barrier(0);
        }
        auto park = [&](auto kc) {
            constexpr int KIND = decltype(kc)::value;
#pragma unroll
            for (int f = 0; f < NF; ++f)
#pragma unroll
                for (int r = 0; r < 4; ++r) pend[f][r] = act_fwd_c<KIND>(acc[f][r] + bv, act);
        };
        if (act == 1) park(std::integral_constant<int, 1>{});
        else park(std::integral_constant<int, -1>{});
        };
        if (SF_IMG_HALFSTEP && TMF == 2 && nf == 1) compute(std::integral_constant<int, 1>{});
        else compute(std::integral_constant<int, TMF>{});
        pend_fb = fb;
        pend_nf = nf;
    }
    if (pend_fb >= 0) store_pend();
}
```

### sample_factory_amd/csrc/sf_nn_u8.h

```cpp
#ifndef SF_CONV1_WP
#define SF_CONV1_WP 84
#endif
#ifndef SF_CONV1_TRACE
#define SF_CONV1_TRACE 0
#endif
#if SF_CONV1_TRACE
__device__ unsigned long long sf_conv1_trace_acc[12];
#define SF_C1T(i)                                 \
    do {                                          \
        const unsigned long long tn_ = clock64(); \
        tacc_[i] += tn_ - tprev_;                 \
        tprev_ = tn_;                             \
    } while (0)
#else
#define SF_C1T(i)
#endif
typedef short s16x4 __attribute__((ext_vector_type(4)));
typedef short s16x8 __attribute__((ext_vector_type(8)));
typedef __bf16 bf16x8 __attribute__((ext_vector_type(8)));

__device__ __forceinline__ void split3_bf16(float w, uint32_t &hi, uint32_t &mid, uint32_t &lo) {
    const uint32_t b = __float_as_uint(w);
    hi = b >> 16;
    const float r1 = w - __uint_as_float(b & 0xFFFF0000u);
    const uint32_t b1 = __float_as_uint(r1);
    mid = b1 >> 16;
    const float r2 = r1 - __uint_as_float(b1 & 0xFFFF0000u);
    lo = __float_as_uint(r2) >> 16;
}

template <bool SUB, int NCT, bool WIDE>
__device__ __forceinline__ void conv1_u8_bf16_body(ConvG g, const uint8_t *__restrict__ in, int64_t in_stride,
                                                   const int32_t *__restrict__ index, int64_t offset,
                                                   const float *__restrict__ w, const float *__restrict__ bias,
                                                   float *__restrict__ out, uint32_t *__restrict__ mask_out,
                                                   int nsamples) {
    constexpr int SMP = 2 * NCT, R = 4, TMF = 5, KB = 8;
    constexpr int H = 84, W = 84, WP = SF_CONV1_WP, Cin = 4, KH = 8, S = 4, OH = 20, OW = 20, OHOW = OH * OW;
    constexpr int RS = (R - 1) * S + KH;
    constexpr int W4 = W >> 2;
    constexpr int WORDS = Cin * RS * W4;
    constexpr int NLD = (WORDS + 255) / 256;
    constexpr int nstrips = OH / R;
    static_assert(R * OW == TMF * 16 && KB * 32 == Cin * KH * 8, "Nature-CNN conv1 geometry");
    extern __shared__ __attribute__((aligned(16))) uint16_t img[];
    constexpr int SP = 36;
    float *const stg = reinterpret_cast<float *>(img + SMP * Cin * RS * WP);
    static_assert((SMP * Cin * RS * WP * 2) % 16 == 0, "staging tile must start 16-byte aligned");
    const int tid = threadIdx.x, lane = tid & 63, wave = __builtin_amdgcn_readfirstlane(tid >> 6);
    const int N = g.Cout;
    const int wsmp = NCT == 2 ? wave : (wave >> 1), ct0 = NCT == 2 ? 0 : (wave & 1);
    const int nquads = (nsamples + SMP - 1) / SMP;
    const int my_quads = (int)blockIdx.x < nquads ? (nquads - 1 - (int)blockIdx.x) / (int)gridDim.x + 1 : 0;
    const int total_units = my_quads * nstrips;
    if (total_units == 0) return;
    int gofs[NLD], lofs[NLD];
#pragma unroll
    for (int i = 0; i < NLD; ++i) {
        int q = tid + 256 * i;
        const bool ok = q < WORDS;
        q = ok ? q : 0;
        const int x4 = q % W4, t1 = q / W4, row = t1 % RS, c = t1 / RS;
        gofs[i] = (c * H + row) * W + x4 * 4;
        lofs[i] = ok ? (c * RS + row) * WP + x4 * 4 : -1;
    }
    uint32_t pre[SMP][NLD];
    auto load_strip = [&](int unit) {
        const int lq = unit / nstrips, st = unit - lq * nstrips;
        const int s0u = ((int)blockIdx.x + lq * (int)gridDim.x) * SMP;
// ... 131 lines not shown
                            sl[(t * 16 + r) * SP + ct * 16] = act_fwd_c<KIND>(acc[t][ct][r] * scl + bv[ct], g.relu);
                return;
            }
#pragma unroll
            for (int t = 0; t < TMF; ++t)
#pragma unroll
                for (int ct = 0; ct < NCT; ++ct) {
                    const int cc = (ct0 + ct) * 16 + col;
#pragma unroll
                    for (int r = 0; r < 4; ++r) {
                        const float v = act_fwd_c<KIND>(acc[t][ct][r] * scl + bv[ct], g.relu);
                        if (sok && cc < N) ob[(int64_t)(t * 16 + 4 * kg + r) * N + cc] = v;
                        if (KIND == 1 && NCT == 1 && mb) {
                            const unsigned long long bits = __ballot(v > 0.f);
                            if (col == 0 && sok) mb[(t * 16 + 4 * kg + r) * 2] = (uint16_t)(bits >> (16 * kg));
                        }
                    }
                }
        };
        if (g.relu == 1) epilogue(std::integral_constant<int, 1>{});
        else epilogue(std::integral_constant<int, -1>{});
        SF_C1T(4);
        __syncthreads();
        SF_C1T(5);
        if constexpr (WIDE) {
            constexpr int QS = R * OW * 8;
#pragma unroll
            for (int k = 0; k < (SMP * QS + 255) / 256; ++k) {
                const int q = tid + 256 * k, z = q >= QS ? 1 : 0, qq = q - z * QS, px = qq >> 3, ch = qq & 7;
                if (SMP * QS % 256 != 0 && q >= SMP * QS) break;
                const float4 v = *reinterpret_cast<const float4 *>(stg + (z * (R * OW) + px) * SP + ch * 4);
                const bool sok = s0 + z < nsamples;
                const int64_t pix0 = (int64_t)(s0 + z) * OHOW + st * (R * OW);
                if (sok) *reinterpret_cast<float4 *>(out + pix0 * 32 + qq * 4) = v;
                if (g.relu == 1 && mask_out) {
                    int nib = (v.x > 0.f ? 1 : 0) | (v.y > 0.f ? 2 : 0) | (v.z > 0.f ? 4 : 0) | (v.w > 0.f ? 8 : 0);
                    nib <<= 4 * ch;
                    nib |= __builtin_amdgcn_update_dpp(0, nib, 0xB1 , 0xF, 0xF, true);
                    nib |= __builtin_amdgcn_update_dpp(0, nib, 0x4E , 0xF, 0xF, true);
                    nib |= __builtin_amdgcn_update_dpp(0, nib, 0x141 , 0xF, 0xF, true);
                    if (ch == 0 && sok) mask_out[pix0 + px] = (uint32_t)nib;
                }
            }
            SF_C1T(6);
        }
    }
#if SF_CONV1_TRACE
    if (lane == 0) {
#pragma unroll
        for (int i = 0; i < 7; ++i) atomicAdd(&sf_conv1_trace_acc[i], tacc_[i]);
        atomicAdd(&sf_conv1_trace_acc[7], (unsigned long long)total_units);
        atomicAdd(&sf_conv1_trace_acc[8], clock64() - tc0_);
        atomicAdd(&sf_conv1_trace_acc[9], wall_clock64() - tw0_);
        atomicAdd(&sf_conv1_trace_acc[10], 1ull);
    }
#endif
}

template <bool SUB>
__global__ __launch_bounds__(256, 2)
void k_conv1_u8_bf16(ConvG g, const uint8_t *__restrict__ in, int64_t in_stride, const int32_t *__restrict__ index,
                     int64_t offset, const float *__restrict__ w, const float *__restrict__ bias,
                     float *__restrict__ out, uint32_t *__restrict__ mask_out, int nsamples) {
    conv1_u8_bf16_body<SUB, 1, false>(g, in, in_stride, index, offset, w, bias, out, mask_out, nsamples);
}
template <bool SUB>
__global__ __launch_bounds__(256, 2)
void k_conv1_u8_bf16_w(ConvG g, const uint8_t *__restrict__ in, int64_t in_stride, const int32_t *__restrict__ index,
                       int64_t offset, const float *__restrict__ w, const float *__restrict__ bias,
                       float *__restrict__ out, uint32_t *__restrict__ mask_out, int nsamples) {
    conv1_u8_bf16_body<SUB, 1, true>(g, in, in_stride, index, offset, w, bias, out, mask_out, nsamples);
}

template <bool SUB>
__global__ __launch_bounds__(256, 2)
void k_conv1_wgrad_bf16(ConvG g, const uint8_t *__restrict__ in, int64_t in_stride, const int32_t *__restrict__ index,
                        int64_t offset, const float *__restrict__ dy, const uint32_t *__restrict__ dmask,
                        float *__restrict__ partial, float *__restrict__ partial_b, int nsamples, int npairs) {
    constexpr int SMP = 2, R = 4, H = 84, W = 84, Cin = 4, S = 4, OH = 20, OW = 20, OHOW = OH * OW, N = 32, K = 256;
    constexpr int RS = (R - 1) * S + 8, W4 = W >> 2;
    constexpr int WP2 = (W4 + 1) / 2, PAIRS = Cin * RS * WP2, NLD = (PAIRS + 255) / 256;
    constexpr int QP = 36;
    constexpr int PIX = SMP * R * OW;
    constexpr int DP = 168;
    constexpr int IMG_E = SMP * Cin * RS * 4 * QP;
    constexpr int NDY = (PIX / 2 * (N / 4) + 255) / 256;
    constexpr int nstrips = OH / R;
    extern __shared__ __attribute__((aligned(16))) uint16_t smem16[];
    uint16_t *img = smem16;
    uint16_t *dyT = smem16 + IMG_E;
    const int tid = threadIdx.x, lane = tid & 63, wave = __builtin_amdgcn_readfirstlane(tid >> 6);
    const int i16 = lane & 15, kg = lane >> 4;
    int gofs[NLD], gofs2[NLD], lofs[NLD];
#pragma unroll
    for (int i = 0; i < NLD; ++i) {
        int u = tid + 256 * i;
        const bool ok = u < PAIRS;
        u = ok ? u : 0;
        const int xp = u % WP2, t1 = u / WP2, row = t1 % RS, c = t1 / RS;
        gofs[i] = (c * H + row) * W + xp * 8;
        gofs2[i] = gofs[i] + (2 * xp + 1 < W4 ? 4 : 0);
        lofs[i] = ok ? ((c * RS + row) * 4) * QP + 2 * xp : -1;
    }
    const int n4 = tid & 7;
// ... 178 lines not shown
```

### sample_factory_amd/lib.py

```python
from __future__ import annotations

import ctypes as C
import os
import threading
from typing import Optional

import torch

_HERE = os.path.dirname(os.path.abspath(__file__))
LIB_PATH = os.environ.get("SF_HIP_LIB") or os.path.join(_HERE, "libsf_hip.so")


class SfHipError(RuntimeError):
    pass


class sf_loss_cfg(C.Structure):
    _fields_ = [("clip_ratio", C.c_float), ("clip_value", C.c_float), ("value_loss_coeff", C.c_float),
                ("exploration_coeff", C.c_float), ("kl_coeff", C.c_float), ("exploration_kind", C.c_int32),
                ("action_kind", C.c_int32), ("dense_adv", C.c_int32), ("num_heads", C.c_int32),
                ("head_n", C.c_int32 * 8), ("old_values_T", C.c_int32)]


class sf_conv_desc(C.Structure):
    _fields_ = [("Cin", C.c_int32), ("H", C.c_int32), ("W", C.c_int32), ("Cout", C.c_int32), ("KH", C.c_int32),
                ("KW", C.c_int32), ("stride", C.c_int32), ("OH", C.c_int32), ("OW", C.c_int32),
                ("in_u8", C.c_int32), ("relu", C.c_int32), ("traj_T", C.c_int32), ("sub_mean", C.c_float),
                ("inv_scale", C.c_float)]


IN_F32_NHWC, IN_U8_FRAME, IN_F32_FRAME = 0, 1, 2


class sf_res_desc(C.Structure):
    _fields_ = [("Cin", C.c_int32), ("H", C.c_int32), ("W", C.c_int32), ("Cout", C.c_int32), ("in_u8", C.c_int32),
                ("act_in", C.c_int32), ("traj_T", C.c_int32), ("sub_mean", C.c_float), ("inv_scale", C.c_float)]


SYMBOLS = [
    "sf_last_error", "sf_abi_version", "sf_valid_mask", "sf_gae_returns", "sf_moments", "sf_rms_update",
    "sf_rms_apply", "sf_vtrace", "sf_ppo_loss", "sf_ppo_loss_heads", "sf_loss_scalars", "sf_train_summaries", "sf_minibatch_indices", "sf_minibatch_expand", "sf_grad_sumsq",
    "sf_adam_step", "sf_adam_step_dlr", "sf_lr_kl_adaptive", "sf_clock_probe", "sf_lamb_step", "sf_rnn_cell_fwd", "sf_rnn_cell_bwd", "sf_rows_add_scale", "sf_mlp2_fwd", "sf_rnn_store_state", "sf_rnn_chunk_setup", "sf_lstm_seq_supported", "sf_lstm_seq_fwd", "sf_lstm_seq_bwd", "sf_gru_seq_fwd", "sf_gru_seq_bwd", "sf_seq_fwd_x_supported", "sf_lstm_seq_fwd_x", "sf_gru_seq_fwd_x", "sf_rnn_rowseq_supported", "sf_rnn_rowseq_fwd", "sf_rnn_rowseq_bwd", "sf_rnn_wideseq_supported", "sf_rnn_seq_slab_rows", "sf_rnn_wideseq_fwd", "sf_rnn_wideseq_bwd", "sf_linear_fwd_dual_supported", "sf_linear_fwd_dual",
    "sf_obsnorm_moments", "sf_obsnorm_update", "sf_obsnorm_apply", "sf_sample_write_step",
    "sf_sample_write_step_tuple", "sf_sample_write_step_masked", "sf_traj_write_env_step", "sf_synth_obs",
    "sf_synth_step", "sf_synth_vec_step", "sf_h2d_rows", "sf_copy_rows", "sf_conv_fwd", "sf_conv_fwd_workspace", "sf_conv_wgrad_workspace", "sf_conv_wgrad",
    "sf_conv_dgrad", "sf_conv_norm_supported", "sf_conv_fwd_norm", "sf_conv_wgrad_norm", "sf_conv_relu_mask_supported", "sf_conv_fwd_relu_mask", "sf_conv_wgrad_relu_mask", "sf_conv_kernel_name", "sf_conv_fwd_t_supported", "sf_conv_fwd_t_workspace", "sf_conv_fwd_t", "sf_transpose",
    "sf_tanh_scale_fwd", "sf_tanh_scale_bwd",
    "sf_linear_fwd", "sf_linear_wgrad_workspace", "sf_linear_wgrad", "sf_linear_dgrad", "sf_relu_mask",
    "sf_dp_unique_id", "sf_dp_comm_create", "sf_dp_comm_destroy", "sf_dp_comm_info", "sf_allreduce_grads",
    "sf_dp_allreduce_f64", "sf_dp_broadcast", "sf_dp_oneshot_create", "sf_dp_oneshot_connect", "sf_dp_oneshot_allreduce_f32",
    "sf_dp_oneshot_allreduce_f64", "sf_dp_oneshot_status", "sf_dp_oneshot_destroy",
    "sf_res_conv_fwd", "sf_res_pool_fwd", "sf_res_pool_bwd", "sf_res_conv_dgrad", "sf_res_conv_wgrad_workspace",
    "sf_res_conv_wgrad", "sf_res_conv_fwd_norm", "sf_res_conv_wgrad_norm",
]

_lib: Optional[C.CDLL] = None

_REC = threading.local()
_QUERIES = ("_supported", "_workspace", "_kernel_name", "sf_last_error", "sf_abi_version")
_HOST_STATE = ("sf_h2d_rows", "sf_dp_", "sf_allreduce_grads", "sf_clock_probe")
LAUNCH_PROGRAMS = os.environ.get("SF_LAUNCH_PROGRAMS", "1") != "0"


class LaunchProgram:
    __slots__ = ("calls", "keep", "unsafe")

    def __init__(self):
        self.calls = []
        self.keep = []
        self.unsafe = None

    def replay(self) -> None:
        if PROFILE is None:
            for fn, args, what, _ in self.calls:
                rc = fn(*args)
                if rc:
                    _check(rc, what)
        else:
            for fn, args, what, key in self.calls:
# ... 65 lines not shown


class _timed:
    def __init__(self, key):
        self.rec = getattr(_REC, "rec", None)
        if self.rec is not None:
            self.rec.key = key
        self.key = key if PROFILE is not None and key is not None and \
            (PROFILE_ONLY is None or key in PROFILE_ONLY) else None
        if self.key is not None and PROFILE_STRIDE > 1:
            seen = PROFILE_SEEN.get(self.key, 0)
            PROFILE_SEEN[self.key] = seen + 1
            if seen % PROFILE_STRIDE:
                self.key = None

    def __enter__(self):
        if self.key is not None:
            self.s = torch.cuda.Event(enable_timing=True)
            self.e = torch.cuda.Event(enable_timing=True)
            if PROFILE_SYNC:
                torch.cuda.synchronize()
            self.s.record()
        return self

    def __exit__(self, *a):
        if self.key is not None:
            self.e.record()
            PROFILE.setdefault(self.key, []).append((self.s, self.e))
        if self.rec is not None:
            self.rec.key = None
        return False


_OPS = {"fwd": 0, "wgrad": 1, "dgrad": 2, "fwd_t": 3, "fwd_norm": 4, "wgrad_norm": 5}
_names: dict = {}


def _dkey(op, n, d):
    if not _keys_wanted():
        return None
    k = (op, int(n), d.Cin, d.H, d.W, d.Cout, d.KH, d.stride, d.OH, d.OW, d.in_u8)
    name = _names.get(k)
    if name is None:
        name = _names[k] = conv_kernel_name(_OPS[op], n, d)
    return k[:-1] + (name,)


def conv_kernel_name(op: int, n: int, desc) -> str:
    buf = C.create_string_buffer(96)
    _check(load().sf_conv_kernel_name(int(op), i64(n), C.byref(desc), 1, buf, 96), "sf_conv_kernel_name")
    return buf.value.decode()


def load() -> C.CDLL:
    global _lib
    rec = getattr(_REC, "rec", None)
    if rec is not None:
        return rec
    if _lib is None:
        if not os.path.exists(LIB_PATH):
            raise SfHipError(
                f"{LIB_PATH} not found: build it with `python -m sample_factory_amd.build` (hipcc, gfx950). "
                "sample_factory_amd has no CPU/PyTorch fallback for the hot path.")
        lib = C.CDLL(LIB_PATH)
        lib.sf_last_error.restype = C.c_char_p
        lib.sf_conv_wgrad_workspace.restype = C.c_int64
        lib.sf_conv_fwd_workspace.restype = C.c_int64
# ... 636 lines not shown


def conv_wgrad_norm(inp, in_sample_stride, index, offset, mu, rstd, dout, dw, db, n, desc: sf_conv_desc, workspace) -> None:
    with _timed(_nkey("wgrad", n, desc, "wgrad_norm")):
        _check(load().sf_conv_wgrad_norm(_raw_in(inp, desc), i64(in_sample_stride), ptr(index, "i32", "index"),
                                         i64(offset), ptr(mu, "f32", "mu"), ptr(rstd, "f32", "rstd"),
                                         ptr(dout, "f32", "dout"), ptr(dw, "f32", "dw"), ptr(db, "f32", "db"), i64(n),
                                         C.byref(desc), ptr(workspace, "u8", "workspace"), stream()), "sf_conv_wgrad_norm")


def conv_dgrad(dout, w, in_act, din, n, desc: sf_conv_desc) -> None:
    with _timed(_dkey("dgrad", n, desc)):
        _check(load().sf_conv_dgrad(ptr(dout, "f32", "dout"), ptr(w, "f32", "w"), ptr(in_act, "f32", "in_act"),
                                  ptr(din, "f32", "din"), i64(n), C.byref(desc), stream()), "sf_conv_dgrad")


def conv_fwd_t_supported(n, desc: sf_conv_desc) -> bool:
    return bool(load().sf_conv_fwd_t_supported(i64(n), C.byref(desc)))


def conv_fwd_t_workspace(n, desc: sf_conv_desc) -> int:
    return int(load().sf_conv_fwd_t_workspace(i64(n), C.byref(desc)))


def conv_fwd_t(inp, in_sample_stride, wt, bias, out, n, desc: sf_conv_desc, workspace=None) -> None:
    with _timed(_dkey("fwd_t", n, desc)):
        _check(load().sf_conv_fwd_t(_raw_in(inp, desc), i64(in_sample_stride), ptr(wt, "f32", "wt"),
                                    ptr(bias, "f32", "bias"), ptr(out, "f32", "out"), i64(n), C.byref(desc),
                                    ptr(workspace, "u8", "workspace"),
                                    i64(workspace.numel() if workspace is not None else 0), stream()),
               "sf_conv_fwd_t")


def tanh_scale_fwd(x, ld, n, col0, ncols, scale) -> None:
    _check(load().sf_tanh_scale_fwd(ptr(x, "f32", "x"), int(ld), i64(n), int(col0), int(ncols), C.c_float(scale), stream()),
           "sf_tanh_scale_fwd")


def tanh_scale_bwd(g, y, ld, n, col0, ncols, scale) -> None:
    _check(load().sf_tanh_scale_bwd(ptr(g, "f32", "g"), ptr(y, "f32", "y"), int(ld), i64(n), int(col0), int(ncols),
                                    C.c_float(scale), stream()), "sf_tanh_scale_bwd")


def transpose(w, wt, K, N) -> None:
    _check(load().sf_transpose(ptr(w, "f32", "w"), ptr(wt, "f32", "wt"), int(K), int(N), stream()), "sf_transpose")


def linear_fwd(inp, w, bias, out, M, K, N, relu) -> None:
    _check(load().sf_linear_fwd(ptr(inp, "f32", "in"), ptr(w, "f32", "w"), ptr(bias, "f32", "bias"),
                                ptr(out, "f32", "out"), i64(M), int(K), int(N), int(bool(relu)), stream()),
           "sf_linear_fwd")


def linear_wgrad_workspace(M, K, N) -> int:
    return int(load().sf_linear_wgrad_workspace(i64(M), int(K), int(N)))


def linear_wgrad(inp, dout, dw, db, M, K, N, workspace) -> None:
    _check(load().sf_linear_wgrad(ptr(inp, "f32", "in"), ptr(dout, "f32", "dout"), ptr(dw, "f32", "dw"),
                                  ptr(db, "f32", "db"), i64(M), int(K), int(N), ptr(workspace, "u8", "workspace"),
                                  stream()), "sf_linear_wgrad")


def linear_dgrad(dout, w, in_act, din, M, K, N) -> None:
    _check(load().sf_linear_dgrad(ptr(dout, "f32", "dout"), ptr(w, "f32", "w"), ptr(in_act, "f32", "in_act"),
                                  ptr(din, "f32", "din"), i64(M), int(K), int(N), stream()), "sf_linear_dgrad")
# ... 149 lines not shown
```

### sample_factory_amd/model/actor_critic.py

```python
from __future__ import annotations

import math
import threading
from typing import Dict, List, Optional

import numpy as np
import torch

from sample_factory_amd import lib
from sample_factory_amd.algo.utils.running_mean_std import RunningMeanStdInPlace
from sample_factory_amd.envs.spaces import is_box, calc_num_action_parameters

import os

_LSTM_SEQ = os.environ.get("SF_LSTM_SEQ", "1") != "0"
_CONV1_NORM = os.environ.get("SF_CONV1_NORM", "1") != "0"
_MLP2 = os.environ.get("SF_MLP2", "1") != "0"

ACT_KIND = {"relu": 1, "tanh": 2, "elu": 3}
FRAME_KINDS = {"conv_u8": lib.IN_U8_FRAME, "conv_f32frame": lib.IN_F32_FRAME}

CONV_ARCHS = {
    "convnet_simple": [[32, 8, 4], [64, 4, 2], [128, 3, 2]],
    "convnet_impala": [[16, 8, 4], [32, 4, 2]],
    "convnet_atari": [[32, 8, 4], [64, 4, 2], [64, 3, 1]],
}


def get_rnn_size(cfg) -> int:
    size = cfg.rnn_size * cfg.rnn_num_layers if cfg.use_rnn else 1
    if cfg.rnn_type == "lstm":
        size *= 2
    if not cfg.actor_critic_share_weights:
        size *= 2
    return size


def _pad(n: int, q: int = 64) -> int:
    return (n + q - 1) // q * q


class _Layer:

    def __init__(self, name, desc: lib.sf_conv_desc, ref_w_shape, kind, first_fc_chw=None, wname=None, bname=None,
                 role="chain"):
        self.name = name
        self.wname = wname or name + ".weight"
        self.bname = bname or name + ".bias"
        self.role = role
        self.in_act_kind = 0
# ... 241 lines not shown
                continue
            L.in_act_kind = prev_kind
            prev_kind = 0 if L.role == "rnn_ih" else L.desc.relu
        self.obs_elems = int(np.prod(self.obs_shape))
        self._mlp2_ok = (len(self.obs_shape) == 1 and len(self.layers) >= (2 if self.headless else 3) and not self.features_in and
                         all(L.kind == "linear" and L.role == "chain" and L.desc.relu == act for L in self.layers[:2]) and
                         len(cfg.encoder_mlp_layers) == 2 and
                         lib.mlp2_supported(self.obs_shape[0], self.layers[0].N, self.layers[1].N))

        off = 0
        self._segs = []
        for L in self.layers:
            self._segs.append((off, off + _pad(L.K * L.N)))
            off = self._segs[-1][1] + _pad(L.N)
        self.num_flat = off
        self.seat_flat(torch.zeros(off, dtype=torch.float32, device=self.device),
                       torch.zeros(off, dtype=torch.float32, device=self.device),
                       torch.zeros(off, dtype=torch.float32, device=self.device))
        self.obs_normalizer = None
        if norm_input:
            from sample_factory_amd.utils.normalize import ObservationNormalizer
            self.obs_normalizer = ObservationNormalizer(cfg, self.obs_shape, self.obs_u8, self.device,
                                                        all_reduce=all_reduce, world=getattr(cfg, "dp_world", 1))
            if obs_key != "obs":
                self.obs_normalizer.sub_mean, self.obs_normalizer.inv_scale = 0.0, 1.0
        self._xn: Dict = {}
        self.returns_normalizer: Optional[RunningMeanStdInPlace] = None
        if cfg.normalize_returns and not self.headless:
            self.returns_normalizer = RunningMeanStdInPlace((1,), self.device, all_reduce=all_reduce)
        self._init_scratch()
        self._ctx: Dict = {}
        self._rnn_out: Dict = {}
        self._rnn_saved_l: Dict = {}
        self.initialize_weights()

    def seat_flat(self, flat_params: torch.Tensor, flat_grads: torch.Tensor, flat_params_t: torch.Tensor) -> None:
        old = getattr(self, "flat_params", None)
        if old is not None:
            flat_params.copy_(old)
            flat_params_t.copy_(self.flat_params_t)
        self.flat_params, self.flat_grads, self.flat_params_t = flat_params, flat_grads, flat_params_t
        self._layout_gen = getattr(self, "_layout_gen", 0) + 1
        for L, (o, ob) in zip(self.layers, self._segs):
            L.w = flat_params[o:o + L.K * L.N].view(L.K, L.N)
            L.b = flat_params[ob:ob + L.N]
            L.gw = flat_grads[o:o + L.K * L.N].view(L.K, L.N)
            L.gb = flat_grads[ob:ob + L.N]
            ok = not L.desc.in_u8 and ((L.desc.Cin % 32 == 0 and L.N >= 32) or (L.kind == "heads" and L.K % 16 == 0))
            L.wt = flat_params_t[o:o + L.K * L.N].view(L.N, L.K) if ok else None

    def num_params(self) -> int:
        n = sum(L.K * L.N + L.N for L in self._body())
        return n if self.headless else n + (self.feat + 1) * (1 + self.num_action_params)

    def _body(self):
        return self.layers if self.headless else self.layers[:-1]

    @property
    def heads_layer(self):
        return self.layers[-1]

    def share_normalizers_from(self, other) -> None:
        self.obs_normalizer = other.obs_normalizer
        self.returns_normalizer = None

    def share_seq_sync_from(self, other) -> None:
        self._bufs[("rnn", "seq_sync")] = other._seq_sync_buf()

    def share_snapshot_tables_from(self, other) -> None:
        self._snap_tabs = other._snap_tabs

    def train(self, mode=True):
        self.training = mode
        if self.returns_normalizer is not None:
# ... 16 lines not shown
            return out
        A, F = self.num_action_params, self.feat
        out += [("critic_linear.weight", (1, F)), ("critic_linear.bias", (1,))]
        if self.nonadaptive_std:
            out += [("action_parameterization.learned_stddev", (A // 2,)),
                    ("action_parameterization.distribution_linear.weight", (A // 2, F)),
                    ("action_parameterization.distribution_linear.bias", (A // 2,))]
        else:
            out += [("action_parameterization.distribution_linear.weight", (A, F)),
                    ("action_parameterization.distribution_linear.bias", (A,))]
        return out

    def state_dict(self) -> Dict[str, torch.Tensor]:
        sd = self.normalizer_state()
        if self.returns_normalizer is not None:
            sd.update(self.returns_normalizer.state_dict("returns_normalizer."))
        for L in self._body():
            sd[L.wname] = L.w_to_ref(L.w.detach()).cpu()
            sd[L.bname] = L.b.detach().cpu().clone()
        if self.headless:
            return sd
        H, A = self.layers[-1], self.num_action_params
        w = H.w.detach().cpu()
        sd["critic_linear.weight"] = w[:, 0:1].t().contiguous()
        sd["critic_linear.bias"] = H.b.detach().cpu()[0:1].clone()
        Aw = A // 2 if self.nonadaptive_std else A
        sd["action_parameterization.distribution_linear.weight"] = w[:, 1:1 + Aw].t().contiguous()
        sd["action_parameterization.distribution_linear.bias"] = H.b.detach().cpu()[1:1 + Aw].clone()
        if self.nonadaptive_std:
            sd["action_parameterization.learned_stddev"] = H.b.detach().cpu()[1 + Aw:1 + A].clone()
        return sd

    def load_state_dict(self, sd, strict=True):
        with torch.no_grad():
            for L in self._body():
                L.w.copy_(L.w_from_ref(torch.as_tensor(sd[L.wname], dtype=torch.float32)))
                L.b.copy_(torch.as_tensor(sd[L.bname], dtype=torch.float32))
            if self.headless:
                self.params_changed()
                self.load_normalizer_state(sd)
                return
            H, A = self.layers[-1], self.num_action_params
            cw = torch.as_tensor(sd["critic_linear.weight"], dtype=torch.float32)
            aw = torch.as_tensor(sd["action_parameterization.distribution_linear.weight"], dtype=torch.float32)
            pad = self.heads_ld - 1 - A
            ab = torch.as_tensor(sd["action_parameterization.distribution_linear.bias"], dtype=torch.float32).reshape(-1)
            if self.nonadaptive_std:
                aw = torch.cat([aw, torch.zeros((A // 2, self.feat))], dim=0)
                ab = torch.cat([ab, torch.as_tensor(sd["action_parameterization.learned_stddev"],
                                                    dtype=torch.float32).reshape(-1)])
            H.w.copy_(torch.cat([cw, aw, torch.zeros((pad, self.feat))], dim=0).t().contiguous())
            H.b.copy_(torch.cat([torch.as_tensor(sd["critic_linear.bias"], dtype=torch.float32).reshape(1), ab,
                                 torch.zeros(pad)]))
            self.params_changed()
            self.load_normalizer_state(sd)
            if self.returns_normalizer is not None and "returns_normalizer.running_mean" in sd:
                self.returns_normalizer.load_state_dict(sd, "returns_normalizer.")
            elif strict and self.returns_normalizer is not None:
                raise KeyError("returns_normalizer.* missing from state dict")

    def flat_to_ref(self, flat: torch.Tensor) -> Dict[str, torch.Tensor]:
        out = {}
        for L, (o, ob) in zip(self._body(), self._segs):
            out[L.wname] = L.w_to_ref(flat[o:o + L.K * L.N].view(L.K, L.N)).cpu()
            out[L.bname] = flat[ob:ob + L.N].cpu().clone()
        if self.headless:
# ... 19 lines not shown
        out = self._buf((tag, "frames_aligned"), (n, self.obs_elems), dtype=x.dtype)
        lib.recording_unsafe("frames gathered by a torch op")
        torch.index_select(flat, 0, pos, out=out)
        return out, self.obs_elems, None, 0, 0

    def _frames_vector_geometry(self) -> bool:
        d = self.layers[0].desc
        return d.KW % 4 == 0 and d.stride % 4 == 0 and d.W % 4 == 0

    def tensor_segment_ids(self):
        seg = torch.full((self.num_flat,), 255, dtype=torch.uint8)
        nseg = 0
        for L, (o, ob) in zip(self._body(), self._segs):
            seg[o:o + L.K * L.N] = nseg
            seg[ob:ob + L.N] = nseg + 1
            nseg += 2
        if self.headless:
            return seg.to(self.device), nseg
        H, (o, ob), A = self.layers[-1], self._segs[-1], self.num_action_params
        hw = torch.full((H.K, H.N), 255, dtype=torch.uint8)
        hw[:, 0] = nseg
        Aw = A // 2 if self.nonadaptive_std else A
        hw[:, 1:1 + Aw] = nseg + 2
        seg[o:o + H.K * H.N] = hw.reshape(-1)
        hb = torch.full((H.N,), 255, dtype=torch.uint8)
        hb[0] = nseg + 1
        hb[1:1 + Aw] = nseg + 3
        if self.nonadaptive_std:
            hb[1 + Aw:1 + A] = nseg + 4
        seg[ob:ob + H.N] = hb
        return seg.to(self.device), nseg + (5 if self.nonadaptive_std else 4)

    def params_changed(self) -> None:
        for L in self.layers:
            if L.wt is not None:
                lib.transpose(L.w, L.wt, L.K, L.N)

    def enable_weight_snapshots(self) -> None:
        self._snap = [self.flat_params.clone(), self.flat_params.clone()]
        self._snap_t = [self.flat_params_t.clone(), self.flat_params_t.clone()]
        self._snap_views = []
        for buf, buft in zip(self._snap, self._snap_t):
            self._snap_views.append([(buf[o:o + L.K * L.N].view(L.K, L.N), buf[ob:ob + L.N],
                                      buft[o:o + L.K * L.N].view(L.N, L.K) if L.wt is not None else None)
                                     for L, (o, ob) in zip(self.layers, self._segs)])
        self.snap_read = 0
        self._layout_gen += 1
        on = self.obs_normalizer
        self._snap_tabs = [(on.mu_tab.clone(), on.rstd_tab.clone()) for _ in range(2)] if on is not None else None

    def publish_weights(self, slot: int) -> None:
        self._snap[slot].copy_(self.flat_params)
        self._snap_t[slot].copy_(self.flat_params_t)
        if self._snap_tabs is not None:
            self._snap_tabs[slot][0].copy_(self.obs_normalizer.mu_tab)
            self._snap_tabs[slot][1].copy_(self.obs_normalizer.rstd_tab)

    def _wb(self, li, tag):
        if tag.startswith("inf") and self._snap is not None:
            return self._snap_views[self.snap_read][li]
        L = self.layers[li]
        return L.w, L.b, L.wt

    def _gemm(self, li, x, stride, index, offset, traj_T, out, n, tag):
        L = self.layers[li]
        d = L.desc
        if traj_T:
            d = lib.sf_conv_desc.from_buffer_copy(L.desc)
            d.traj_T = int(traj_T)
        w, b, wt = self._wb(li, tag)
        if wt is not None and index is None and not traj_T and lib.conv_fwd_t_supported(n, d):
            wsb = lib.conv_fwd_t_workspace(n, d)
            lib.conv_fwd_t(x, stride, wt, b, out, n, d, self._workspace(wsb) if wsb else None)
            return
        wsb = lib.conv_fwd_workspace(n, d) if index is None and not traj_T else 0
        lib.conv_fwd_raw(x, stride, index, offset, w, b, out, n, d, self._workspace(wsb) if wsb else None)

    def forward_heads(self, obs: torch.Tensor, n: int, *, sample_stride: int, index=None, offset: int = 0,
                      traj_T: int = 0, tag="inf", rnn=None) -> List[torch.Tensor]:
        acts: List[Optional[torch.Tensor]] = [None] * len(self.layers)
        inputs: List[Optional[torch.Tensor]] = [None] * len(self.layers)
        relu_mask0 = None
        self._tls.role = "rollout" + tag[3:] if tag.startswith("inf") else "learner"
        x, stride, idx, off, tT = obs, sample_stride, index, offset, traj_T
        first_layer = 0
        if self._mlp2_ok and tag.startswith("inf") and index is None and not traj_T and _MLP2:
            on = self.obs_normalizer
            tabs = None
            if on is not None:
                tabs = self._snap_tabs[self.snap_read] if self._snap is not None else (on.mu_tab, on.rstd_tab)
            (w1, b1, _), (w2, b2, _) = self._wb(0, tag), self._wb(1, tag)
            out = self._buf((tag, 1), (n, self.layers[1].N))
            lib.mlp2_fwd(obs, sample_stride, n, self.obs_elems, on.sub_mean if on is not None else 0.0,
                         on.inv_scale if on is not None else 1.0, tabs[0] if tabs else None, tabs[1] if tabs else None,
                         w1, b1, w2, b2, self.act_kind, out)
            acts[1] = out
            x, stride, idx, off, tT = out, self.layers[1].N, None, 0, 0
            first_layer = 2
        norm_tabs = None
        if self.obs_normalizer is not None and first_layer == 0:
            on = self.obs_normalizer
            tabs = self._snap_tabs[self.snap_read] if (tag.startswith("inf") and self._snap is not None) else None
            if self._fused_norm:
                norm_tabs = tabs if tabs is not None else (on.mu_tab, on.rstd_tab)
                if self.obs_u8 and (x.data_ptr() % 4 or stride % 4) and self._frames_vector_geometry():
                    x, stride, idx, off, tT = self._aligned_frames(tag, x, stride, idx, off, tT, n)
                elif not self.obs_u8 and (x.data_ptr() % 16 or stride % 4) and self._frames_vector_geometry():
                    x, stride, idx, off, tT = self._aligned_frames(tag, x, stride, idx, off, tT, n)
            else:
                xn = self._buf((tag, "obsn"), (n, self.obs_elems))
                on.apply(obs, sample_stride, n, xn, index=index, offset=offset, traj_T=traj_T, tabs=tabs)
                x, stride, idx, off, tT = xn, self.obs_elems, None, 0, 0
        first_in = (x, stride, idx, off, tT)
        seq = rnn is not None and "R" in rnn
        for li, L in enumerate(self.layers):
            if L.role == "rnn_hh" or li < first_layer:
                continue
            if L.role == "rnn_ih" and seq:
                R, Cn = rnn["R"], n // rnn["R"]
                xt = self._buf((tag, "x_tm", li), (n, L.K))
                xt.view(R, Cn, L.K).copy_(x.view(Cn, R, L.K).transpose(0, 1))
                x = xt
            inputs[li] = x
            out = self._buf((tag, li), (n * L.out_pixels, L.N))
            mask = None
            if tag == "train" and li == 0 and norm_tabs is None and li + 1 < len(self.layers) and self.layers[1].role == "chain":
                d0 = L.desc
                if tT:
                    d0 = lib.sf_conv_desc.from_buffer_copy(L.desc)
                    d0.traj_T = int(tT)
                w_, b_, _ = self._wb(li, tag)
                aligned = x.data_ptr() % 4 == 0 and stride % 4 == 0 and w_.data_ptr() % 16 == 0 and out.data_ptr() % 16 == 0
                if aligned and lib.conv_relu_mask_supported(n, d0):
                    mask = self._buf((tag, "relu_mask0"), (n * L.out_pixels,), dtype=torch.int32)
                    lib.conv_fwd_relu_mask(x, stride, idx, off, w_, b_, out, mask, n, d0)
            fuse_x = False
            if L.role == "rnn_ih" and seq and _LSTM_SEQ and L.wt is not None and idx is None and not tT:
                fuse_x = lib.lstm_seq_supported(n // rnn["R"], self.rnn_H) and lib.seq_fwd_x_supported(n // rnn["R"], self.rnn_H, L.K)
            fuse_dual = False
            if L.role == "rnn_ih" and rnn is not None and not seq and idx is None and not tT:
                fuse_dual = (self._wb(li, tag)[2] is not None and self._wb(li + 1, tag)[2] is not None and
                             self.rnn_H % 64 == 0 and lib.linear_fwd_dual_supported(n, 4 * self.rnn_H, L.K, self.rnn_H))
            if li == 0 and norm_tabs is not None:
                w_, b_, _ = self._wb(li, tag)
                dn = L.desc
                if tT:
                    dn = lib.sf_conv_desc.from_buffer_copy(L.desc)
                    dn.traj_T = int(tT)
                lib.conv_fwd_norm(x, stride, idx, off, norm_tabs[0], norm_tabs[1], w_, b_, out, n, dn)
            elif mask is None and not fuse_x and not fuse_dual:
                self._gemm(li, x, stride, idx, off, tT, out, n, tag)
            if li == 0:
                relu_mask0 = mask
            acts[li] = out
            x = out
            if L.role == "rnn_ih":
                if fuse_x:
                    acts[li] = None
                    x = self._rnn_sequence_fwd(li, None, n, rnn, tag, x_tm=inputs[li])
                elif fuse_dual:
                    acts[li] = None
                    x = self._rnn_step(li, None, n, rnn, tag, x_in=inputs[li], x_stride=stride)
                else:
                    x = self._rnn_sequence_fwd(li, out, n, rnn, tag) if seq else self._rnn_step(li, out, n, rnn, tag)
            stride, idx, off, tT = x.numel() // n, None, 0, 0
        if self.tanh_scale > 0:
            lib.tanh_scale_fwd(acts[-1], self.heads_ld, n, 1, self.num_action_params // 2, self.tanh_scale)
        self._ctx[tag] = dict(acts=acts, inputs=inputs, first_in=first_in, rnn=rnn, relu_mask0=relu_mask0,
                              norm_tabs=norm_tabs)
        return acts

    def _rnn_step(self, li, gx, n, rnn, tag, x_in=None, x_stride=0):
        Lh, H, S, kind = self.layers[li + 1], self.rnn_H, self.rnn_S, self.rnn_kind
        l, SL = self.layers[li].rnn_l, self.rnn_SL
        assert rnn["states"].shape == (n, S) and rnn["states"].stride(1) == 1
        st = rnn["states"][:, l * SL:(l + 1) * SL]
        gh = self._buf((tag, "gh", l), (n, Lh.N))
        w_hh, b_hh, wt_hh = self._wb(li + 1, tag)
        if x_in is not None:
            _, b_ih, wt_ih = self._wb(li, tag)
            gpre = self._buf((tag, "gpre", l), (n, 4 * H))
            lib.linear_fwd_dual(x_in, x_stride, wt_ih, b_ih, st, st.stride(0), wt_hh, b_hh, gpre, n, gru_H=H if kind == 0 else 0)
            gx, gh = gpre, None
        elif wt_hh is not None and lib.conv_fwd_t_supported(n, Lh.desc):
            wsb = lib.conv_fwd_t_workspace(n, Lh.desc)
            lib.conv_fwd_t(st, st.stride(0), wt_hh, b_hh, gh, n, Lh.desc, self._workspace(wsb) if wsb else None)
        else:
            lib.conv_fwd_raw(st, st.stride(0), None, 0, w_hh, b_hh, gh, n, Lh.desc)
        h_out = self._buf((tag, "h_out", l), (n, H))
        c_out = self._buf((tag, "c_out", l), (n, H)) if kind == 1 else None
        lib.rnn_cell_fwd(kind, gx, gh, st, st.stride(0), st[:, H:] if kind == 1 else None, st.stride(0), None, n, H,
                         None, h_out, c_out, None, None)
        if l == 0:
            self._rnn_out[tag] = []
        self._rnn_out[tag].append((h_out, c_out))
        return h_out

    def _rnn_sequence_fwd(self, li, GX, n, rnn, tag, x_tm=None):
        Lh, H, kind = self.layers[li + 1], self.rnn_H, self.rnn_kind
        R, Cn = rnn["R"], n // rnn["R"]
        l, SL = self.layers[li].rnn_l, self.rnn_SL
        h0, keep = rnn["h0"][:, l * SL:(l + 1) * SL], rnn["keep_tm"]
        GH = Lh.N
        gates = self._buf((tag, "gates", li), (R, Cn, 4 * H))
# ... 192 lines not shown
```

### sample_factory_amd/train.py

```python
from __future__ import annotations

import json
import os
import threading
import time
from collections import deque
from typing import Any, Callable, Dict, List, Tuple

import numpy as np

import torch

from sample_factory_amd.algo.learning.learner import Learner, ParameterServer
from sample_factory_amd.algo.sampling.batched_sampling import BatchedVectorEnvRunner
from sample_factory_amd.algo.utils.env_info import extract_env_info
from sample_factory_amd.algo.learning.batcher import Batcher
from sample_factory_amd.algo.utils.shared_buffers import BufferMgr
from sample_factory_amd.cfg.arguments import cfg_dict, preprocess_cfg
from sample_factory_amd.envs.env_utils import create_env, find_training_info_interface, set_training_info
from sample_factory_amd.algo.sampling.parallel_env import ParallelVecEnvView
from sample_factory_amd.utils.attr_dict import AttrDict
from sample_factory_amd.utils.timing import Timing
from sample_factory_amd.utils.utils import init_file_logger, log

# ... 188 lines not shown
        self.env = self.envs[0]
        self.env_info = extract_env_info(self.env, cfg)
        n = self.env_info.num_agents
        if any(env.num_agents != n for env in self.envs):
            raise ValueError("all env instances must have the same number of agents")
        if int(cfg.num_envs_per_worker) % int(cfg.worker_num_splits) != 0:
            cfg.worker_num_splits = 1
        if not preprocess_cfg(cfg, self.env_info):
            self.close_envs()
            return ExperimentStatus.FAILURE
        self.user_cfg.recurrence = cfg.recurrence
        if self.rank == 0:
            self._save_cfg()
            init_file_logger(cfg)
        dev = torch.device("cuda", torch.cuda.current_device())
        cfg.batched_sampling = True
        self.buffer_mgr = BufferMgr(cfg, self.env_info, dev)
        self.batcher = Batcher(self.buffer_mgr, cfg)
        self.traj = self.buffer_mgr.traj_tensors
        self.policy_versions = self.buffer_mgr.policy_versions
        self.learner = Learner(cfg, self.env_info, self.policy_versions, 0, ParameterServer(0, self.policy_versions))
        self.learner.init()
        self.num_rows = E * n
        per_unit = int(cfg.num_envs_per_worker) // int(cfg.worker_num_splits)
        self.unit_rows = per_unit * n
        assert self.unit_rows == self.buffer_mgr.sampling_trajectories_per_iteration
        self.units = [list(range(e0, e0 + per_unit)) for e0 in range(0, E, per_unit)]
        self.samplers = [BatchedVectorEnvRunner(cfg, self.env_info, env, self.learner.actor_critic,
                                                self.traj[e * n:(e + 1) * n], 0, self.policy_versions,
                                                sample_seed=(cfg.seed or 0), row0=self.rank * self.num_rows + e * n,
                                                tag="inf" if e == 0 else f"inf{e}")
                         for e, env in enumerate(self.envs)]
        self.sampler = self.samplers[0]
        self._prev_rows: List = [None] * E
        S = max(1, min(int(cfg.worker_num_splits), E))
        prio = -1 if (cfg.async_rl and os.environ.get("SF_ROLLOUT_PRIORITY", "0") == "1") else 0
        self.split_streams = [torch.cuda.Stream(priority=prio) for _ in range(S)] if E > 1 else None
        self._ev_fork = torch.cuda.Event()
        self._ev_join = [torch.cuda.Event() for _ in range(S)]
        self._training_info_ifaces = [env if isinstance(env, ParallelVecEnvView) else find_training_info_interface(env)
                                      for env in self.envs]
        self._cv = threading.Condition(threading.RLock())
        self._ready: List[slice] = []
        self._round_events: Dict[int, torch.cuda.Event] = {}
        self._free_events: Dict[int, torch.cuda.Event] = {}
        self.sampling_rounds = 0
        if cfg.async_rl:
            self.rollout_stream = torch.cuda.Stream(priority=prio)
            self.ev_publish = torch.cuda.Event()
            self.learner.actor_critic.enable_weight_snapshots()
            self._pub_slot = 0
            self._slot_last_read = [None, None]
            self._reading_slot = None
            self.published_version = float(self.learner.train_step)
        for sm in self.samplers:
            sm.reset()
        if cfg.async_rl:
            ev_reset = torch.cuda.Event()
            ev_reset.record()
            self.rollout_stream.wait_event(ev_reset)
        want = getattr(cfg, "sampler_thread", None)
        self.threaded = bool(cfg.async_rl and (want if want is not None else any(sm.host_env for sm in self.samplers)))
        self._thread, self._stop, self._thread_error = None, False, None
        self._ep_stats_request, self._ep_stats_result = False, None
        self._observers_call("on_init", self)
        self._observers_call("on_connect_components", self)
# ... 335 lines not shown
```

Measured before the change: 2.145 million.

## Reuse rollout conv activations for the first training minibatch

During rollout, the first few conv layers write their outputs and the ReLU mask into per-row, per-timestep keep buffers through new strided-output kernel variants. In the first minibatch of the first epoch, the learner then skips recomputing those layers when the weights generation, trajectory layout and kernel choice all match. This removes part of the learner's forward pass at the cost of extra device memory and strided stores during rollout. It is gated by many conditions (no RNN, no normaliser, no shuffle, sync RL), so it may rarely engage.

```diff
diff --git a/include/sf_hip.h b/include/sf_hip.h
--- a/include/sf_hip.h
+++ b/include/sf_hip.h
@@ -253,6 +253,15 @@
                   int64_t n, const sf_conv_desc *desc, void *workspace, int64_t workspace_bytes, void *stream);
 int sf_transpose(const float *w, float *wt, int K, int N, void *stream);
 
+int sf_conv_fwd_os_supported(int op, int64_t n, const sf_conv_desc *desc, int64_t in_sample_stride,
+                             int64_t out_sample_stride);
+int sf_conv_fwd_relu_mask_os(const void *in, int64_t in_sample_stride, const int32_t *index, int64_t offset,
+                             const float *w, const float *bias, float *out, int64_t out_sample_stride,
+                             uint32_t *relu_mask, int64_t mask_sample_stride, int64_t n, const sf_conv_desc *h_desc,
+                             void *stream);
+int sf_conv_fwd_t_os(const float *in, int64_t in_sample_stride, const float *wt, const float *bias, float *out,
+                     int64_t out_sample_stride, int64_t n, const sf_conv_desc *desc, void *stream);
+
 int sf_conv_kernel_name(int op, int64_t n, const sf_conv_desc *desc, int split_k_allowed, char *out, int cap);
 int sf_linear_fwd(const float *in, const float *w, const float *bias, float *out, int64_t M, int K, int N, int relu,
                   void *stream);
diff --git a/sample_factory_amd/algo/learning/learner.py b/sample_factory_amd/algo/learning/learner.py
--- a/sample_factory_amd/algo/learning/learner.py
+++ b/sample_factory_amd/algo/learning/learner.py
@@ -137,6 +137,7 @@
         self.world = self.group.world if self.group is not None else 1
         self.dp = self.group is not None and self.group.on
         self._grad_norms: List[float] = []
+        self.reuse_stats = dict(reused=0, plain=0, last_prefix=0, last_reason="")
 
     def _all_reduce(self, t: torch.Tensor) -> None:
         if self.dp:
@@ -419,7 +420,7 @@
         return dist, sc[0].clone(), sc[1].clone(), kl_old, sc[2].clone(), sc[3].clone(), summaries
 
     def _losses_native(self, buff: AttrDict, mb, num_invalids: int, scalars_out: Optional[torch.Tensor] = None,
-                       moments: Optional[torch.Tensor] = None):
+                       moments: Optional[torch.Tensor] = None, first_of: Optional[Tuple[int, int]] = None):
         cfg, ac = self.cfg, self.actor_critic
         index, offset, n = mb
         A = self.num_action_params
@@ -430,8 +431,16 @@
             h0 = ac._buf(("rnn", "h0"), (Cn, buff.rnn_states.shape[-1]))
             lib.rnn_chunk_setup(buff.dones, buff.valids, buff.rnn_states, index, offset, Cn, R, keep_tm, h0, traj_T=buff.T)
             rnn = dict(R=R, h0=h0, keep_tm=keep_tm)
+        kw = {}
+        if first_of == (0, 0):
+            resume, why = ac.kept_resume(buff.obs, index, offset, n, buff.T, 0, 0) if hasattr(ac, "kept_resume") else (None, "model")
+            st = self.reuse_stats
+            st["reused" if resume is not None else "plain"] += 1
+            st["last_prefix"], st["last_reason"] = (resume["prefix"] if resume is not None else 0), why
+            if resume is not None:
+                kw["resume_from"] = resume
         acts = ac.forward_heads(buff.obs, n, sample_stride=ac.obs_elems, index=index, offset=offset,
-                                traj_T=buff.T, tag="train", rnn=rnn)
+                                traj_T=buff.T, tag="train", rnn=rnn, **kw)
         heads = acts[-1]
         ld = ac.heads_ld
         params, values = heads[:, 1:], heads[:, 0]
@@ -499,7 +508,8 @@
             for batch_num, mb in enumerate(minibatches):
                 row = self._scalars[epoch * n_mb + batch_num]
                 acts, g_heads, _ = self._losses_native(buff, mb, num_invalids, row,
-                                                       moments=None if mom_tab is None else mom_tab[batch_num])
+                                                       moments=None if mom_tab is None else mom_tab[batch_num],
+                                                       first_of=(epoch, batch_num))
                 index, offset, n = mb
                 if self._dp_split is not None:
                     cut = ac._segs[self._dp_split][0]
diff --git a/sample_factory_amd/algo/learning/rollout_reuse.py b/sample_factory_amd/algo/learning/rollout_reuse.py
--- /dev/null
+++ b/sample_factory_amd/algo/learning/rollout_reuse.py
@@ -0,0 +1,56 @@
+from __future__ import annotations
+
+from typing import Dict, NamedTuple, Sequence, Tuple
+
+
+class SlotRecord(NamedTuple):
+    row0: int
+    row1: int
+    t: int
+    generation: int
+    obs_ptr: int
+
+
+def twin_name(dense: str) -> str:
+    return dense.replace("<", "_os<", 1)
+
+
+def reuse_prefix(*, epoch: int, batch_num: int, indexed: bool, offset: int, n: int, T: int, keep_T: int, keep_rows: int,
+                 records: Dict[Tuple[int, int], SlotRecord], generation: int, obs_ptr: int, obs_row_bytes: int,
+                 obs_step_bytes: int, has_normalizer: bool, has_rnn: bool, async_rl: bool, snapshot_reads: bool,
+                 layer_ok: Sequence[bool]) -> Tuple[int, str]:
+    if epoch != 0 or batch_num != 0:
+        return 0, "not the first minibatch"
+    if indexed:
+        return 0, "minibatch gathered through an index"
+    if async_rl or snapshot_reads:
+        return 0, "the rollout does not read the learner's weights"
+    if has_normalizer or has_rnn:
+        return 0, "normaliser or recurrent core"
+    if keep_T <= 0 or T != keep_T:
+        return 0, "trajectory length differs from the kept one"
+    if n <= 0 or offset % T or n % T:
+        return 0, "minibatch does not consist of whole trajectories"
+    e0, e1 = offset // T, (offset + n) // T
+    if e1 > keep_rows:
+        return 0, "rows beyond the kept buffer"
+    for t in range(T):
+        covered = e0
+        for (row0, tt), r in sorted(records.items()):
+            if tt != t or r.row1 <= e0 or r.row0 >= e1:
+                continue
+            if r.row0 > covered:
+                return 0, f"rows {covered}..{r.row0} of step {t} were never kept"
+            if r.generation != generation:
+                return 0, "the weights changed since the rollout"
+            if r.t != t or r.obs_ptr != obs_ptr + r.row0 * obs_row_bytes + t * obs_step_bytes:
+                return 0, "kept from other slab rows than this dataset's"
+            covered = max(covered, r.row1)
+        if covered < e1:
+            return 0, f"rows {covered}..{e1} of step {t} were never kept"
+    prefix = 0
+    for ok in layer_ok:
+        if not ok:
+            break
+        prefix += 1
+    return prefix, "ok" if prefix else "first layer's launches differ"
diff --git a/sample_factory_amd/algo/sampling/batched_sampling.py b/sample_factory_amd/algo/sampling/batched_sampling.py
--- a/sample_factory_amd/algo/sampling/batched_sampling.py
+++ b/sample_factory_amd/algo/sampling/batched_sampling.py
@@ -60,6 +60,7 @@
         self._progs_layout = None
         self.program_replays = 0
         self._launch_key = getattr(actor_critic, "launch_key", None) if lib.LAUNCH_PROGRAMS else None
+        self.keep_on, self.keep_row0 = False, 0
         self.masked = "action_mask" in traj["obs"]
         if self.masked and (self.continuous or len(self.heads) != 1):
             raise NotImplementedError("action masks are supported for a single Discrete action space")
@@ -185,6 +186,8 @@
             self._progs[rec_key] = prog
         else:
             self._policy_and_sample(t)
+        if self.keep_on:
+            self.ac.keep_note(t, self.keep_row0, self.B, self.obs[:, t].data_ptr())
         tr = self.traj
         env_actions = tr["actions"][:, t] if (self.continuous or self.mixed) else self.env_actions
         if self.async_env:
@@ -197,7 +200,8 @@
         ver, deterministic, cfg, step = self._c_ver, self._deterministic, self.cfg, self._c_step
         rnn = dict(states=tr["rnn_states"][:, t]) if self.rnn else None
         x = {k: tr["obs"][k][:, t] for k in self.obs_keys} if self.multi_key else self.obs[:, t]
-        heads = self.ac.forward_heads(x, B, sample_stride=self.obs.stride(0), tag=self.tag, rnn=rnn)[-1]
+        kw = dict(keep=(t, self.keep_row0)) if self.keep_on else {}
+        heads = self.ac.forward_heads(x, B, sample_stride=self.obs.stride(0), tag=self.tag, rnn=rnn, **kw)[-1]
         if self.masked:
             mk = tr["obs"]["action_mask"][:, t]
             lib.sample_write_step_masked(heads[:, 1:], self.ld, heads[:, 0], self.ld, mk, mk.stride(0), B, A, T, t,
diff --git a/sample_factory_amd/cfg/arguments.py b/sample_factory_amd/cfg/arguments.py
--- a/sample_factory_amd/cfg/arguments.py
+++ b/sample_factory_amd/cfg/arguments.py
@@ -66,6 +66,7 @@
     ("dp_oneshot_bytes", int, 0),
     ("dp_native_rccl", _bool, False),
     ("dp_force_collectives", _bool, False),
+    ("reuse_rollout_activations", str, "auto"),
     ("device_shuffle", _bool, False),
     ("sampler_thread", _bool, None),
     ("record_grad_norm", _bool, False),
@@ -150,6 +151,8 @@
         err(f"{cfg.batch_size=} must be a multiple of {cfg.rollout=}")
     if cfg.use_rnn and cfg.recurrence <= 1:
         err("RNN policies need recurrence > 1")
+    if str(getattr(cfg, "reuse_rollout_activations", "auto")) not in ("auto", "off"):
+        err(f"{cfg.reuse_rollout_activations=} must be 'auto' or 'off'")
     total_agents = cfg.num_workers * cfg.num_envs_per_worker * env_info.num_agents
     per_iter = cfg.num_batches_per_epoch * cfg.batch_size
     per_rollout = total_agents * cfg.rollout // cfg.num_policies
diff --git a/sample_factory_amd/csrc/sf_nn.hip b/sample_factory_amd/csrc/sf_nn.hip
--- a/sample_factory_amd/csrc/sf_nn.hip
+++ b/sample_factory_amd/csrc/sf_nn.hip
@@ -323,6 +323,39 @@
 #endif
             }
     }
+}
+
+template <int TM, int TN, int KIND>
+__device__ __forceinline__ void store_fwd_tile_os(const f32x16 (&acc)[TM][TN], float *__restrict__ out, int64_t mrow0,
+                                                  int64_t Mtot, const ConvG &g, int64_t out_ss, int col,
+                                                  const float *__restrict__ bias, int kind) {
+    const int N = g.Cout;
+    const uint32_t OHOW = (uint32_t)(g.OH * g.OW);
+    bool cok[TN];
+    float bv[TN];
+#pragma unroll
+    for (int tn = 0; tn < TN; ++tn) {
+        cok[tn] = col + tn * 32 < N;
+        bv[tn] = (bias && cok[tn]) ? bias[col + tn * 32] : 0.f;
+    }
+    const int hop = (int)out_ss - (int)OHOW * N;
+#pragma unroll
+    for (int tm = 0; tm < TM; ++tm)
+#pragma unroll
+        for (int q = 0; q < 4; ++q) {
+            const int64_t m0 = mrow0 + tm * 32 + 8 * q;
+            const uint32_t smp = fdiv((uint32_t)(m0 < Mtot ? m0 : 0), g.dOHOW), pix = (uint32_t)m0 - smp * OHOW;
+            float *p0 = out + (int64_t)smp * out_ss + (int64_t)pix * N + col;
+#pragma unroll
+            for (int j = 0; j < 4; ++j) {
+                const int o = j * N + (pix + (uint32_t)j >= OHOW ? hop : 0);
+#pragma unroll
+                for (int tn = 0; tn < TN; ++tn) {
+                    const float v = act_fwd_c<KIND>(acc[tm][tn][4 * q + j] + bv[tn], kind);
+                    if (cok[tn] && m0 + j < Mtot) p0[o + tn * 32] = v;
+                }
+            }
+        }
 }
 
 template <int TM, int TN, int KIND, bool FULL>
@@ -865,6 +898,13 @@
     p.t = t;
     plan_kernel(p, kernel, "%s<%d, %d, %d, %d%s>", base, t.BM, t.BN, t.WM, t.WN, tail);
 }
+static void plan_os_name(ConvPlan &p) {
+    char tmp[64];
+    const char *lt = strchr(p.name, '<');
+    if (!lt) return;
+    snprintf(tmp, sizeof(tmp), "%.*s_os%s", (int)(lt - p.name), p.name, lt);
+    memcpy(p.name, tmp, sizeof(tmp));
+}
 static void plan_raster(ConvPlan &p, bool on) {
     p.rx = (int)p.grid.x; p.ry = (int)p.grid.y;
     p.rtot = on ? (int)(p.grid.x * p.grid.y * p.grid.z) : 0;
@@ -1024,7 +1064,7 @@
 static int conv_fwd_impl(const void *in, int64_t in_sample_stride, const int32_t *index, int64_t offset, const float *w,
                          const float *bias, float *out, uint32_t *relu_mask, int64_t n, const sf_conv_desc *h_desc,
                          void *workspace, int64_t workspace_bytes, void *stream, const float *mu = nullptr,
-                         const float *rstd = nullptr) {
+                         const float *rstd = nullptr, bool os = false, int64_t out_ss = 0, int64_t mask_ss = 0) {
     int rc = check_desc(h_desc, "sf_conv_fwd");
     if (rc) return rc;
     SF_REQUIRE(in && w && out && n > 0, "sf_conv_fwd: bad args");
@@ -1040,6 +1080,8 @@
     SF_REQUIRE(relu_mask == nullptr || bf16,
                "sf_conv_fwd_relu_mask: operands not eligible for the sign-bit kernel (sf_conv_relu_mask_supported, 4-byte "
                "aligned frames and sample stride, 16-byte aligned weights)");
+    SF_REQUIRE(!os || p.kernel == K_CONV1_U8_BF16_W,
+               "sf_conv_fwd_relu_mask_os: not a launch of the whole-line-store conv1 kernel (sf_conv_fwd_os_supported)");
     if (bf16 && sw().debug_occ) {
         const unsigned img_bytes = 2u * 4u * 20u * (unsigned)SF_CONV1_WP * (unsigned)sizeof(uint16_t);
         fprintf(stderr, "k_conv1_u8_bf16 occupancy: %d (dword stores, %u B LDS) / %d (whole-line stores, %u B LDS) work-groups per CU\n",
@@ -1052,6 +1094,11 @@
     KERN<<<p.grid, p.block, p.lds, st>>>(g, in8, in_sample_stride, index, offset, w, bias, out, ##__VA_ARGS__, (int)n)
     switch (p.kernel) {
         case K_CONV1_U8_BF16_W:
+            if (os) {
+                if (p.variant) k_conv1_u8_bf16_w_os<true><<<p.grid, p.block, p.lds, st>>>(g, in8, in_sample_stride, index, offset, w, bias, out, relu_mask, (int)n, out_ss, mask_ss);
+                else k_conv1_u8_bf16_w_os<false><<<p.grid, p.block, p.lds, st>>>(g, in8, in_sample_stride, index, offset, w, bias, out, relu_mask, (int)n, out_ss, mask_ss);
+                break;
+            }
             if (p.variant) CONV1_LAUNCH(k_conv1_u8_bf16_w<true>, relu_mask); else CONV1_LAUNCH(k_conv1_u8_bf16_w<false>, relu_mask);
             break;
         case K_CONV1_U8_BF16:
@@ -1086,12 +1133,28 @@
     return conv_fwd_impl(in, in_sample_stride, index, offset, w, bias, out, relu_mask, n, h_desc, nullptr, 0, stream);
 }
 
+static bool out_stride_ok(const sf_conv_desc *d, const void *out, int64_t out_ss) {
+    return out_ss >= (int64_t)d->OH * d->OW * d->Cout && out_ss < (1LL << 30) && out_ss % 4 == 0 && aligned(out, 16);
+}
+extern "C" int sf_conv_fwd_relu_mask_os(const void *in, int64_t in_sample_stride, const int32_t *index, int64_t offset,
+                                        const float *w, const float *bias, float *out, int64_t out_sample_stride,
+                                        uint32_t *relu_mask, int64_t mask_sample_stride, int64_t n, const sf_conv_desc *h_desc,
+                                        void *stream) {
+    SF_REQUIRE(relu_mask && ((uintptr_t)relu_mask & 3) == 0, "sf_conv_fwd_relu_mask_os: relu_mask must be a 4-byte aligned device buffer");
+    SF_REQUIRE(h_desc && n > 0 && relu_mask_ok(h_desc, n) && ((uintptr_t)in & 3) == 0 && in_sample_stride % 4 == 0,
+               "sf_conv_fwd_relu_mask_os: unsupported layer / launch (see sf_conv_relu_mask_supported)");
+    SF_REQUIRE(out_stride_ok(h_desc, out, out_sample_stride) && mask_sample_stride >= (int64_t)h_desc->OH * h_desc->OW,
+               "sf_conv_fwd_relu_mask_os: output / mask sample stride shorter than a sample, or unaligned output");
+    return conv_fwd_impl(in, in_sample_stride, index, offset, w, bias, out, relu_mask, n, h_desc, nullptr, 0, stream, nullptr,
+                         nullptr, true, out_sample_stride, mask_sample_stride);
+}
+
 #ifndef SF_IMG_TMF
 #define SF_IMG_TMF 2
 #endif
 #define IMG_FWD_GEOMS(X) X(64, 9, 9, 3, 1, SF_IMG_TMF, 1, 7)
-static int plan_img_fwd(ConvPlan &p, const ConvG &g, int64_t n) {
-    if (!sw().fwd_img || g.Cout != 64 || g.KH != g.KW || n < 512) return -1;
+static int plan_img_fwd(ConvPlan &p, const ConvG &g, int64_t n, bool any_n = false) {
+    if (!sw().fwd_img || g.Cout != 64 || g.KH != g.KW || (n < 512 && !any_n)) return -1;
     int idx = 0;
 #define X(CIN, HH, WW, KS, ST, TMF, WS, R)                                                                         \
     if (g.Cin == CIN && g.H == HH && g.W == WW && g.KH == KS && g.S == ST) {                                       \
@@ -1173,7 +1236,8 @@
     if (tiles <= resident || tail == 0 || 2 * tail > resident) return (int)tiles;
     return (int)(tiles - tail);
 }
-static ConvPlan plan_conv_fwd_t(const sf_conv_desc *d, int64_t n, int64_t in_sample_stride, ConvG *g_out = nullptr) {
+static ConvPlan plan_conv_fwd_t(const sf_conv_desc *d, int64_t n, int64_t in_sample_stride, ConvG *g_out = nullptr,
+                                bool os = false) {
     ConvPlan p = plan_init();
     if (narrow_fwd_ok(d, n)) {
         p.recommended = true; p.variant = d->Cout <= 16 ? 1 : 2;
@@ -1185,14 +1249,30 @@
     const ConvG g = make_geom(d);
     if (g_out) *g_out = g;
     const int64_t Mtot = n * g.OH * g.OW;
-    if (n * in_sample_stride < ((int64_t)1 << 40) && plan_img_fwd(p, g, n) >= 0) { p.recommended = true; return p; }
+    if (n * in_sample_stride < ((int64_t)1 << 40) && plan_img_fwd(p, g, n, os) >= 0) {
+        p.recommended = true;
+        if (os) plan_os_name(p);
+        return p;
+    }
     GldsFwdPlan q = plan_fwd_t(Mtot, g.Cout, g.K);
     p.recommended = q.ok;
     if (!q.ok) { q.Z = 1; q.k_per_split = (g.K + 31) / 32 * 32; }
     p.splits = q.Z; p.per_split = q.k_per_split;
-    const bool zl_ok = sw().glds_zl && (n - 1) * in_sample_stride + (int64_t)g.H * g.W * g.Cin < (1LL << 30) &&
+    const int64_t lane_span = os ? 127 / (g.OH * g.OW) + 1 : n - 1;
+    const bool zl_ok = sw().glds_zl && lane_span * in_sample_stride + (int64_t)g.H * g.W * g.Cin < (1LL << 30) &&
                        (int64_t)g.Cout * g.K < (1LL << 30);
     const bool col64 = !q.sq64 && !q.wide && q.Z == 1 && g.Cout <= 64 && zl_ok;
+    if (os) {
+        p.splits = 1; p.per_split = (g.K + 31) / 32 * 32;
+        p.main_tiles = g.K % 32 == 0 && g.OH * g.OW >= 4 ? fwd_tail_split(g, Mtot, 1, zl_ok) : 0;
+        if (p.main_tiles <= 0) return plan_init();
+        const int tail = (int)cdiv64(Mtot, 128) - p.main_tiles;
+        p.grid = dim3((unsigned)(p.main_tiles + 2 * tail));
+        p.lds = (128 + 64) * 32 * 2 * sizeof(float);
+        plan_tile(p, K_FWD_GLDS_ZT, "k_fwd_glds_zt", TileArgs{128, 64, 2, 2});
+        plan_os_name(p);
+        return p;
+    }
     if (sw().glds_persist && col64) {
         static const int occp = occupancy_of(k_fwd_glds_zp<128, 64, 2, 2>);
         const int64_t tiles = cdiv64(Mtot, 128), slots = (int64_t)num_cus() * occp;
@@ -1293,6 +1373,52 @@
     if (partial) launch_splitk_finish(partial, bias, out, Mtot * g.Cout, g, p.splits, st);
     return sf_launch_status("sf_conv_fwd_t");
 }
+extern "C" int sf_conv_fwd_t_os(const float *in, int64_t in_sample_stride, const float *wt, const float *bias, float *out,
+                                int64_t out_sample_stride, int64_t n, const sf_conv_desc *h_desc, void *stream) {
+    int rc = check_desc(h_desc, "sf_conv_fwd_t_os");
+    if (rc) return rc;
+    SF_REQUIRE(in && wt && out && n > 0, "sf_conv_fwd_t_os: bad args");
+    SF_REQUIRE(((uintptr_t)in & 15) == 0 && ((uintptr_t)wt & 15) == 0 && in_sample_stride % 4 == 0,
+               "sf_conv_fwd_t_os: operands must be 16-byte aligned");
+    SF_REQUIRE(out_stride_ok(h_desc, out, out_sample_stride),
+               "sf_conv_fwd_t_os: output sample stride shorter than a sample, or unaligned output");
+    ConvG g;
+    const ConvPlan p = plan_conv_fwd_t(h_desc, n, in_sample_stride, &g, true);
+    SF_REQUIRE((p.kernel == K_FWD_IMG || p.kernel == K_FWD_GLDS_ZT) && p.splits == 1,
+               "sf_conv_fwd_t_os: this launch has no strided-output kernel (sf_conv_fwd_os_supported)");
+    const int64_t Mtot = n * g.OH * g.OW;
+    SF_REQUIRE(Mtot < (1LL << 31), "sf_conv_fwd_t_os: M=%lld exceeds 2^31 rows; split the batch", (long long)Mtot);
+    hipStream_t st = STREAM(stream);
+    if (p.kernel == K_FWD_IMG) {
+        int idx = 0;
+#define X(CIN, HH, WW, KS, ST, TMF, WS, R)                                                                              \
+    if (p.variant == idx++)                                                                                             \
+        k_fwd_img_os<CIN, HH, WW, KS, ST, TMF, WS, R><<<p.grid, p.block, 0, st>>>(in, in_sample_stride, wt, bias, out, (int)n, \
+                                                                                  g.relu, out_sample_stride);
+        IMG_FWD_GEOMS(X)
+#undef X
+    } else {
+        k_fwd_glds_zt_os<128, 64, 2, 2><<<p.grid, p.block, p.lds, st>>>(g, in, in_sample_stride, wt, bias, out, Mtot, (int)p.per_split,
+                                                                         p.main_tiles, sw().tap_perm, out_sample_stride);
+    }
+    return sf_launch_status("sf_conv_fwd_t_os");
+}
+extern "C" int sf_conv_fwd_os_supported(int op, int64_t n, const sf_conv_desc *h_desc, int64_t in_sample_stride,
+                                        int64_t out_sample_stride) {
+    if (!h_desc || n <= 0 || check_desc(h_desc, "sf_conv_fwd_os_supported") != 0 || in_sample_stride % 4 != 0 ||
+        !out_stride_ok(h_desc, nullptr, out_sample_stride) || n * (int64_t)h_desc->OH * h_desc->OW >= (1LL << 31))
+        return 0;
+    if (op == 0) {
+        if (!relu_mask_ok(h_desc, n)) return 0;
+        Operands o = query_operands(h_desc, false);
+        o.stride = in_sample_stride;
+        return plan_conv_fwd(h_desc, make_geom(h_desc), n, o).kernel == K_CONV1_U8_BF16_W ? 1 : 0;
+    }
+    if (op != 3) return 0;
+    const ConvPlan p = plan_conv_fwd_t(h_desc, n, in_sample_stride, nullptr, true);
+    return (p.kernel == K_FWD_IMG || p.kernel == K_FWD_GLDS_ZT) && p.splits == 1 ? 1 : 0;
+}
+
 extern "C" int sf_linear_fwd_dual_supported(int64_t n, int N, int K1, int K2) {
     return sw().linear_dual && n > 0 && N >= 64 && K1 > 0 && K2 > 0 && K1 % 32 == 0 && K2 % 32 == 0 && n < (1LL << 31) &&
            cdiv64(n, 128) * (int64_t)cdiv64(N, 64) >= 256;
@@ -1751,14 +1877,20 @@
                                    int cap) {
     int rc = check_desc(h_desc, "sf_conv_kernel_name");
     if (rc) return rc;
-    SF_REQUIRE(out && cap >= 48 && n > 0 && op >= 0 && op <= 5, "sf_conv_kernel_name: bad args");
+    SF_REQUIRE(out && cap >= 48 && n > 0 && op >= 0 && op <= 7, "sf_conv_kernel_name: bad args");
     const Operands o = query_operands(h_desc, split_k_allowed != 0);
     ConvG g = make_geom(h_desc);
-    if (op >= 4) g.nmu = g.nrstd = TABLE_PROBE;
-    const ConvPlan p = op == 3 ? plan_conv_fwd_t(h_desc, n, o.stride) : op == 2 ? plan_conv_dgrad(g, n, o)
-                       : (op == 0 || op == 4) ? plan_conv_fwd(h_desc, g, n, o) : plan_conv_wgrad(h_desc, g, n, o);
+    if (op == 4 || op == 5) g.nmu = g.nrstd = TABLE_PROBE;
+    ConvPlan p = op == 3 ? plan_conv_fwd_t(h_desc, n, o.stride) : op == 2 ? plan_conv_dgrad(g, n, o)
+                 : op == 7 ? plan_conv_fwd_t(h_desc, n, o.stride, nullptr, true)
+                 : (op == 0 || op == 4 || op == 6) ? plan_conv_fwd(h_desc, g, n, o) : plan_conv_wgrad(h_desc, g, n, o);
+    if (op == 6) {
+        if (p.kernel == K_CONV1_U8_BF16_W && relu_mask_ok(h_desc, n)) plan_os_name(p);
+        else p.kernel = K_NONE;
+    }
+    if (op == 7 && (p.kernel == K_LINEAR_NARROW || p.splits != 1)) p.kernel = K_NONE;
     SF_REQUIRE(p.kernel != K_NONE, "sf_conv_kernel_name: not a launch %s accepts",
-               op >= 4 ? "sf_conv_norm_supported" : "sf_conv_fwd_t");
+               op >= 6 ? "sf_conv_fwd_os_supported" : op >= 4 ? "sf_conv_norm_supported" : "sf_conv_fwd_t");
     strncpy(out, p.name, (size_t)cap - 1);
     out[cap - 1] = 0;
     return SF_OK;
diff --git a/sample_factory_amd/csrc/sf_nn_glds.h b/sample_factory_amd/csrc/sf_nn_glds.h
--- a/sample_factory_amd/csrc/sf_nn_glds.h
+++ b/sample_factory_amd/csrc/sf_nn_glds.h
@@ -234,12 +234,14 @@
     else mma_chunk_ptrs<TM, TN, STAGE_F>(ap, bp, acc);
 }
 
-template <int BM, int BN, int WM, int WN, int NS, bool ZL, bool PERSIST = false, bool DYNLDS = false>
+template <int BM, int BN, int WM, int WN, int NS, bool ZL, bool PERSIST = false, bool DYNLDS = false, bool OS = false>
 __device__ __forceinline__ void fwd_glds_body(ConvG g, const float *__restrict__ in, int64_t in_stride,
                                               const float *__restrict__ wt, const float *__restrict__ bias,
                                               float *__restrict__ out, int64_t Mtot, int k_per_split,
                                               float *__restrict__ partial, const float *__restrict__ dmask,
-                                              int dmask_on, int rx, int ry, int rtot, int tap_perm, int bx_shift = 0) {
+                                              int dmask_on, int rx, int ry, int rtot, int tap_perm, int bx_shift = 0,
+                                              int64_t out_ss = 0) {
+    static_assert(!OS || (ZL && !PERSIST), "the strided output form exists for the zero-VALU forward only");
     constexpr int TM = BM / WM / 32, TN = BN / WN / 32;
     constexpr int AI = BM / 32, BI = BN / 32;
     constexpr int STAGE = (BM + BN) * 32;
@@ -331,8 +333,10 @@
     if constexpr (ZL) {
 
         uint32_t avoff[AI], bvoff[BI];
-#pragma unroll
-        for (int i = 0; i < AI; ++i) avoff[i] = (uint32_t)((asrc[i] - in) * (int64_t)sizeof(float));
+        const float *inb = in;
+        if constexpr (OS) inb = in + (int64_t)fdiv((uint32_t)(m0 < Mtot ? m0 : Mtot - 1), g.dOHOW) * in_stride;
+#pragma unroll
+        for (int i = 0; i < AI; ++i) avoff[i] = (uint32_t)((asrc[i] - inb) * (int64_t)sizeof(float));
 #pragma unroll
         for (int i = 0; i < BI; ++i) bvoff[i] = (uint32_t)((bsrc[i] - wt) * (int64_t)sizeof(float));
         const uint32_t lds0 = (uint32_t)(uintptr_t)(__attribute__((address_space(3))) float *)lds;
@@ -355,7 +359,7 @@
         };
         {
             const int kf = kord(kbeg);
-            const float *ab = in + chunk_off(kf), *bb = wt + kf;
+            const float *ab = inb + chunk_off(kf), *bb = wt + kf;
 #pragma unroll
             for (int q = 0; q < AI + BI; ++q) dma(q, ab, bb, 0);
         }
@@ -364,7 +368,7 @@
             asm volatile("s_waitcnt vmcnt(0)" ::: "memory");
             BARRIER_NOFENCE();
             const int kn = prefetch ? kord(k0 + 32) : 0;
-            const float *ab = in + chunk_off(kn), *bb = wt + kn;
+            const float *ab = inb + chunk_off(kn), *bb = wt + kn;
             if (!prefetch) prefetch_mask();
             if constexpr (TM * TN <= 2) {
                 mma_chunk_ptrs_mid<TM, TN, ST * STAGE>(apl, bpl, acc, [&](int c) {
@@ -456,6 +460,12 @@
     const int cols_left = N - (n0 + wn * TN * 32) - (lane & 31);
     const uint32_t voff = (uint32_t)(4 * (lane >> 5)) * (uint32_t)N + (uint32_t)(lane & 31);
     const bool full = m0 + BM <= Mtot && n0 + BN <= N;
+    if constexpr (OS) {
+        const int64_t mrow0 = m0 + wm * TM * 32 + 4 * (lane >> 5);
+        const int col = n0 + wn * TN * 32 + (lane & 31);
+        if (g.relu == 1) store_fwd_tile_os<TM, TN, 1>(acc, out, mrow0, Mtot, g, out_ss, col, bias, 1);
+        else store_fwd_tile_os<TM, TN, -1>(acc, out, mrow0, Mtot, g, out_ss, col, bias, g.relu);
+    } else
     if (dmask_on) {
         const float *mk = dmask ? dmask + (m0 + wm * TM * 32) * N + (n0 + wn * TN * 32) : nullptr;
         if (!dmask) {
@@ -516,6 +526,18 @@
     else
         fwd_glds_body<BM / 2, BN, WM, WN, 2, true, false, true>(g, in, in_stride, wt, bias, out, Mtot, k_per_split, nullptr,
                                                                 nullptr, 0, 0, 0, 0, tap_perm, main_tiles);
+}
+template <int BM, int BN, int WM, int WN>
+__global__ __launch_bounds__(256, 2) void k_fwd_glds_zt_os(ConvG g, const float *__restrict__ in, int64_t in_stride,
+                                                          const float *__restrict__ wt, const float *__restrict__ bias,
+                                                          float *__restrict__ out, int64_t Mtot, int k_per_split,
+                                                          int main_tiles, int tap_perm, int64_t out_ss) {
+    if ((int)blockIdx.x < main_tiles)
+        fwd_glds_body<BM, BN, WM, WN, 2, true, false, true, true>(g, in, in_stride, wt, bias, out, Mtot, k_per_split, nullptr,
+                                                                  nullptr, 0, 0, 0, 0, tap_perm, 0, out_ss);
+    else
+        fwd_glds_body<BM / 2, BN, WM, WN, 2, true, false, true, true>(g, in, in_stride, wt, bias, out, Mtot, k_per_split, nullptr,
+                                                                      nullptr, 0, 0, 0, 0, tap_perm, main_tiles, out_ss);
 }
 template <int BM, int BN, int WM, int WN>
 __global__ __launch_bounds__(256, 2) void k_fwd_glds_z(ConvG g, const float *__restrict__ in, int64_t in_stride,
diff --git a/sample_factory_amd/csrc/sf_nn_img.h b/sample_factory_amd/csrc/sf_nn_img.h
--- a/sample_factory_amd/csrc/sf_nn_img.h
+++ b/sample_factory_amd/csrc/sf_nn_img.h
@@ -25,10 +25,10 @@
     static_assert(RING * IMG_B <= 160 * 1024, "LDS");
 };
 
-template <int CIN, int H, int W, int KS, int ST, int TMF, int WSETS, int R>
-__global__ __launch_bounds__(256 * WSETS, 1) void k_fwd_img(const float *__restrict__ in, int64_t in_stride,
-                                                    const float *__restrict__ wt, const float *__restrict__ bias,
-                                                    float *__restrict__ out, int nsamples, int act) {
+template <int CIN, int H, int W, int KS, int ST, int TMF, int WSETS, int R, bool OS>
+__device__ __forceinline__ void fwd_img_body(const float *__restrict__ in, int64_t in_stride,
+                                             const float *__restrict__ wt, const float *__restrict__ bias,
+                                             float *__restrict__ out, int nsamples, int act, int64_t out_ss) {
     typedef ImgFwdGeom<CIN, H, W, KS, ST, TMF, WSETS, R> G;
     constexpr int NW = 4 * WSETS, TB = TMF * WSETS;
     constexpr int OW = G::OW, OHW = G::OHW, K = G::K, KG = G::KG, WQ = G::WQ, PLANE = G::PLANE, RING = G::RING;
@@ -87,6 +87,21 @@
     f32x4 pend[TMF];
     int pend_fb = -1, pend_nf = 0;
     auto store_pend = [&]() {
+        if constexpr (OS) {
+            static_assert(!OS || G::U == 1, "strided output: one unit per sample");
+            const uint32_t mb = (uint32_t)pend_fb * 16u + 4u * (uint32_t)kg;
+#pragma unroll
+            for (int f = 0; f < TMF; ++f) {
+                const uint32_t m = mb + (uint32_t)f * 16u, s = m / (uint32_t)OHW, p = m - s * (uint32_t)OHW;
+#pragma unroll
+                for (int r = 0; r < 4; ++r) {
+                    const uint32_t wrap = p + (uint32_t)r >= (uint32_t)OHW ? 1u : 0u;
+                    float *o = out + (int64_t)(s + wrap) * out_ss + (int64_t)(p + (uint32_t)r - wrap * (uint32_t)OHW) * N + n;
+                    if (f < pend_nf && m + (uint32_t)r < M32) *o = pend[f][r];
+                }
+            }
+            return;
+        }
         float *ob = out + ((int64_t)pend_fb * 16 + 4 * kg) * N + n;
         const int rows_left = (int)(M32 - ((uint32_t)pend_fb * 16u + 4u * (uint32_t)kg));
 #pragma unroll
@@ -166,3 +181,16 @@
     }
     if (pend_fb >= 0) store_pend();
 }
+
+template <int CIN, int H, int W, int KS, int ST, int TMF, int WSETS, int R>
+__global__ __launch_bounds__(256 * WSETS, 1) void k_fwd_img(const float *__restrict__ in, int64_t in_stride,
+                                                    const float *__restrict__ wt, const float *__restrict__ bias,
+                                                    float *__restrict__ out, int nsamples, int act) {
+    fwd_img_body<CIN, H, W, KS, ST, TMF, WSETS, R, false>(in, in_stride, wt, bias, out, nsamples, act, 0);
+}
+template <int CIN, int H, int W, int KS, int ST, int TMF, int WSETS, int R>
+__global__ __launch_bounds__(256 * WSETS, 1) void k_fwd_img_os(const float *__restrict__ in, int64_t in_stride,
+                                                       const float *__restrict__ wt, const float *__restrict__ bias,
+                                                       float *__restrict__ out, int nsamples, int act, int64_t out_ss) {
+    fwd_img_body<CIN, H, W, KS, ST, TMF, WSETS, R, true>(in, in_stride, wt, bias, out, nsamples, act, out_ss);
+}
diff --git a/sample_factory_amd/csrc/sf_nn_u8.h b/sample_factory_amd/csrc/sf_nn_u8.h
--- a/sample_factory_amd/csrc/sf_nn_u8.h
+++ b/sample_factory_amd/csrc/sf_nn_u8.h
@@ -29,12 +29,13 @@
     lo = __float_as_uint(r2) >> 16;
 }
 
-template <bool SUB, int NCT, bool WIDE>
+template <bool SUB, int NCT, bool WIDE, bool OS = false>
 __device__ __forceinline__ void conv1_u8_bf16_body(ConvG g, const uint8_t *__restrict__ in, int64_t in_stride,
                                                    const int32_t *__restrict__ index, int64_t offset,
                                                    const float *__restrict__ w, const float *__restrict__ bias,
                                                    float *__restrict__ out, uint32_t *__restrict__ mask_out,
-                                                   int nsamples) {
+                                                   int nsamples, int64_t out_ss = 0, int64_t mask_ss = 0) {
+    static_assert(!OS || WIDE, "the strided output form exists for the whole-line store path only");
     constexpr int SMP = 2 * NCT, R = 4, TMF = 5, KB = 8;
     constexpr int H = 84, W = 84, WP = SF_CONV1_WP, Cin = 4, KH = 8, S = 4, OH = 20, OW = 20, OHOW = OH * OW;
     constexpr int RS = (R - 1) * S + KH;
@@ -232,14 +233,22 @@
                 const float4 v = *reinterpret_cast<const float4 *>(stg + (z * (R * OW) + px) * SP + ch * 4);
                 const bool sok = s0 + z < nsamples;
                 const int64_t pix0 = (int64_t)(s0 + z) * OHOW + st * (R * OW);
-                if (sok) *reinterpret_cast<float4 *>(out + pix0 * 32 + qq * 4) = v;
+                if constexpr (OS) {
+                    if (sok) *reinterpret_cast<float4 *>(out + (int64_t)(s0 + z) * out_ss + st * (R * OW) * 32 + qq * 4) = v;
+                } else {
+                    if (sok) *reinterpret_cast<float4 *>(out + pix0 * 32 + qq * 4) = v;
+                }
                 if (g.relu == 1 && mask_out) {
                     int nib = (v.x > 0.f ? 1 : 0) | (v.y > 0.f ? 2 : 0) | (v.z > 0.f ? 4 : 0) | (v.w > 0.f ? 8 : 0);
                     nib <<= 4 * ch;
                     nib |= __builtin_amdgcn_update_dpp(0, nib, 0xB1 , 0xF, 0xF, true);
                     nib |= __builtin_amdgcn_update_dpp(0, nib, 0x4E , 0xF, 0xF, true);
                     nib |= __builtin_amdgcn_update_dpp(0, nib, 0x141 , 0xF, 0xF, true);
-                    if (ch == 0 && sok) mask_out[pix0 + px] = (uint32_t)nib;
+                    if constexpr (OS) {
+                        if (ch == 0 && sok) mask_out[(int64_t)(s0 + z) * mask_ss + st * (R * OW) + px] = (uint32_t)nib;
+                    } else {
+                        if (ch == 0 && sok) mask_out[pix0 + px] = (uint32_t)nib;
+                    }
                 }
             }
             SF_C1T(6);
@@ -270,6 +279,14 @@
                        int64_t offset, const float *__restrict__ w, const float *__restrict__ bias,
                        float *__restrict__ out, uint32_t *__restrict__ mask_out, int nsamples) {
     conv1_u8_bf16_body<SUB, 1, true>(g, in, in_stride, index, offset, w, bias, out, mask_out, nsamples);
+}
+template <bool SUB>
+__global__ __launch_bounds__(256, 2)
+void k_conv1_u8_bf16_w_os(ConvG g, const uint8_t *__restrict__ in, int64_t in_stride, const int32_t *__restrict__ index,
+                          int64_t offset, const float *__restrict__ w, const float *__restrict__ bias,
+                          float *__restrict__ out, uint32_t *__restrict__ mask_out, int nsamples, int64_t out_ss,
+                          int64_t mask_ss) {
+    conv1_u8_bf16_body<SUB, 1, true, true>(g, in, in_stride, index, offset, w, bias, out, mask_out, nsamples, out_ss, mask_ss);
 }
 
 template <bool SUB>
diff --git a/sample_factory_amd/lib.py b/sample_factory_amd/lib.py
--- a/sample_factory_amd/lib.py
+++ b/sample_factory_amd/lib.py
@@ -45,6 +45,7 @@
     "sf_sample_write_step_tuple", "sf_sample_write_step_masked", "sf_traj_write_env_step", "sf_synth_obs",
     "sf_synth_step", "sf_synth_vec_step", "sf_h2d_rows", "sf_copy_rows", "sf_conv_fwd", "sf_conv_fwd_workspace", "sf_conv_wgrad_workspace", "sf_conv_wgrad",
     "sf_conv_dgrad", "sf_conv_norm_supported", "sf_conv_fwd_norm", "sf_conv_wgrad_norm", "sf_conv_relu_mask_supported", "sf_conv_fwd_relu_mask", "sf_conv_wgrad_relu_mask", "sf_conv_kernel_name", "sf_conv_fwd_t_supported", "sf_conv_fwd_t_workspace", "sf_conv_fwd_t", "sf_transpose",
+    "sf_conv_fwd_os_supported", "sf_conv_fwd_relu_mask_os", "sf_conv_fwd_t_os",
     "sf_tanh_scale_fwd", "sf_tanh_scale_bwd",
     "sf_linear_fwd", "sf_linear_wgrad_workspace", "sf_linear_wgrad", "sf_linear_dgrad", "sf_relu_mask",
     "sf_dp_unique_id", "sf_dp_comm_create", "sf_dp_comm_destroy", "sf_dp_comm_info", "sf_allreduce_grads",
@@ -176,7 +177,7 @@
         return False
 
 
-_OPS = {"fwd": 0, "wgrad": 1, "dgrad": 2, "fwd_t": 3, "fwd_norm": 4, "wgrad_norm": 5}
+_OPS = {"fwd": 0, "wgrad": 1, "dgrad": 2, "fwd_t": 3, "fwd_norm": 4, "wgrad_norm": 5, "fwd_os": 6, "fwd_t_os": 7}
 _names: dict = {}
 
 
@@ -879,6 +880,28 @@
                "sf_conv_fwd_t")
 
 
+def conv_fwd_os_supported(op: str, n, desc: sf_conv_desc, in_sample_stride, out_sample_stride) -> bool:
+    return bool(load().sf_conv_fwd_os_supported(_OPS[op], i64(n), C.byref(desc), i64(in_sample_stride),
+                                                i64(out_sample_stride)))
+
+
+def conv_fwd_relu_mask_os(inp, in_sample_stride, index, offset, w, bias, out, out_sample_stride, relu_mask,
+                          mask_sample_stride, n, desc: sf_conv_desc) -> None:
+    with _timed(_nkey("fwd", n, desc, "fwd_os")):
+        _check(load().sf_conv_fwd_relu_mask_os(_raw_in(inp, desc), i64(in_sample_stride), ptr(index, "i32", "index"),
+                                               i64(offset), ptr(w, "f32", "w"), ptr(bias, "f32", "bias"),
+                                               _raw(out, "f32", "out"), i64(out_sample_stride),
+                                               _raw(relu_mask, "i32", "relu_mask"), i64(mask_sample_stride), i64(n),
+                                               C.byref(desc), stream()), "sf_conv_fwd_relu_mask_os")
+
+
+def conv_fwd_t_os(inp, in_sample_stride, wt, bias, out, out_sample_stride, n, desc: sf_conv_desc) -> None:
+    with _timed(_nkey("fwd_t", n, desc, "fwd_t_os")):
+        _check(load().sf_conv_fwd_t_os(_raw_in(inp, desc), i64(in_sample_stride), ptr(wt, "f32", "wt"),
+                                       ptr(bias, "f32", "bias"), _raw(out, "f32", "out"), i64(out_sample_stride), i64(n),
+                                       C.byref(desc), stream()), "sf_conv_fwd_t_os")
+
+
 def tanh_scale_fwd(x, ld, n, col0, ncols, scale) -> None:
     _check(load().sf_tanh_scale_fwd(ptr(x, "f32", "x"), int(ld), i64(n), int(col0), int(ncols), C.c_float(scale), stream()),
            "sf_tanh_scale_fwd")
diff --git a/sample_factory_amd/model/actor_critic.py b/sample_factory_amd/model/actor_critic.py
--- a/sample_factory_amd/model/actor_critic.py
+++ b/sample_factory_amd/model/actor_critic.py
@@ -8,6 +8,7 @@
 import torch
 
 from sample_factory_amd import lib
+from sample_factory_amd.algo.learning.rollout_reuse import SlotRecord, reuse_prefix, twin_name
 from sample_factory_amd.algo.utils.running_mean_std import RunningMeanStdInPlace
 from sample_factory_amd.envs.spaces import is_box, calc_num_action_parameters
 
@@ -16,6 +17,8 @@
 _LSTM_SEQ = os.environ.get("SF_LSTM_SEQ", "1") != "0"
 _CONV1_NORM = os.environ.get("SF_CONV1_NORM", "1") != "0"
 _MLP2 = os.environ.get("SF_MLP2", "1") != "0"
+_REUSE = os.environ.get("SF_REUSE_ROLLOUT_ACTS", "1") != "0"
+KEEP_MEM_SHARE = 0.5
 
 ACT_KIND = {"relu": 1, "tanh": 2, "elu": 3}
 FRAME_KINDS = {"conv_u8": lib.IN_U8_FRAME, "conv_f32frame": lib.IN_F32_FRAME}
@@ -323,6 +326,8 @@
         self._ctx: Dict = {}
         self._rnn_out: Dict = {}
         self._rnn_saved_l: Dict = {}
+        self._keep: Optional[Dict] = None
+        self._keep_same: Dict = {}
         self.initialize_weights()
 
     def seat_flat(self, flat_params: torch.Tensor, flat_grads: torch.Tensor, flat_params_t: torch.Tensor) -> None:
@@ -331,6 +336,7 @@
             flat_params.copy_(old)
             flat_params_t.copy_(self.flat_params_t)
         self.flat_params, self.flat_grads, self.flat_params_t = flat_params, flat_grads, flat_params_t
+        self.weights_gen = getattr(self, "weights_gen", 0) + 1
         self._layout_gen = getattr(self, "_layout_gen", 0) + 1
         for L, (o, ob) in zip(self.layers, self._segs):
             L.w = flat_params[o:o + L.K * L.N].view(L.K, L.N)
@@ -413,6 +419,7 @@
         return sd
 
     def load_state_dict(self, sd, strict=True):
+        self.weights_gen += 1
         with torch.no_grad():
             for L in self._body():
                 L.w.copy_(L.w_from_ref(torch.as_tensor(sd[L.wname], dtype=torch.float32)))
@@ -498,6 +505,7 @@
         return seg.to(self.device), nseg + (5 if self.nonadaptive_std else 4)
 
     def params_changed(self) -> None:
+        self.weights_gen += 1
         for L in self.layers:
             if L.wt is not None:
                 lib.transpose(L.w, L.wt, L.K, L.N)
@@ -516,6 +524,7 @@
         self._snap_tabs = [(on.mu_tab.clone(), on.rstd_tab.clone()) for _ in range(2)] if on is not None else None
 
     def publish_weights(self, slot: int) -> None:
+        self.weights_gen += 1
         self._snap[slot].copy_(self.flat_params)
         self._snap_t[slot].copy_(self.flat_params_t)
         if self._snap_tabs is not None:
@@ -543,7 +552,7 @@
         lib.conv_fwd_raw(x, stride, index, offset, w, b, out, n, d, self._workspace(wsb) if wsb else None)
 
     def forward_heads(self, obs: torch.Tensor, n: int, *, sample_stride: int, index=None, offset: int = 0,
-                      traj_T: int = 0, tag="inf", rnn=None) -> List[torch.Tensor]:
+                      traj_T: int = 0, tag="inf", rnn=None, keep=None, resume_from=None) -> List[torch.Tensor]:
         acts: List[Optional[torch.Tensor]] = [None] * len(self.layers)
         inputs: List[Optional[torch.Tensor]] = [None] * len(self.layers)
         relu_mask0 = None
@@ -579,8 +588,33 @@
                 x, stride, idx, off, tT = xn, self.obs_elems, None, 0, 0
         first_in = (x, stride, idx, off, tT)
         seq = rnn is not None and "R" in rnn
+        kp = self._keep if keep is not None else None
+        if kp is not None:
+            assert tag.startswith("inf") and first_layer == 0 and norm_tabs is None and idx is None and not tT
+            assert n == kp["n_roll"] and stride == kp["obs_stride"] and keep[1] + n <= kp["rows"] and self._snap is None
+        if resume_from is not None:
+            assert tag == "train" and first_layer == 0 and norm_tabs is None
+            first_layer = resume_from["prefix"]
+            for li in range(first_layer):
+                inputs[li] = x if li == 0 else acts[li - 1]
+                acts[li] = resume_from["acts"][li]
+            relu_mask0 = resume_from["mask"]
+            x, stride, idx, off, tT = acts[first_layer - 1], acts[first_layer - 1].numel() // n, None, 0, 0
         for li, L in enumerate(self.layers):
             if L.role == "rnn_hh" or li < first_layer:
+                continue
+            if kp is not None and li < kp["prefix"]:
+                t_, r0 = keep
+                kb = self._bufs[("keep", li)]
+                out, w_b = kb[r0:r0 + n, t_], self._wb(li, tag)
+                if li == 0:
+                    mk = self._bufs[("keep", "relu_mask0")]
+                    lib.conv_fwd_relu_mask_os(x, stride, None, 0, w_b[0], w_b[1], out, kb.stride(0), mk[r0:r0 + n, t_],
+                                              mk.stride(0), n, L.desc)
+                else:
+                    lib.conv_fwd_t_os(x, stride, w_b[2], w_b[1], out, kb.stride(0), n, L.desc)
+                inputs[li], acts[li], x = x, out, out
+                stride, idx, off, tT = kb.stride(0), None, 0, 0
                 continue
             if L.role == "rnn_ih" and seq:
                 R, Cn = rnn["R"], n // rnn["R"]
@@ -636,6 +670,99 @@
                               norm_tabs=norm_tabs)
         return acts
 
+    def _keep_rollout_ok(self, li, n, in_stride, out_stride) -> bool:
+        L = self.layers[li]
+        d = L.desc
+        if li == 0:
+            if L.kind != "conv_u8" or d.relu != 1 or self.layers[1].role != "chain":
+                return False
+            if not lib.conv_relu_mask_supported(n, d) or not lib.conv_fwd_os_supported("fwd", n, d, in_stride, out_stride):
+                return False
+            return lib.conv_kernel_name(6, n, d) == twin_name(lib.conv_kernel_name(0, n, d))
+        if L.kind != "conv" or L.wt is None or not lib.conv_fwd_t_supported(n, d) or lib.conv_fwd_t_workspace(n, d):
+            return False
+        if not lib.conv_fwd_os_supported("fwd_t", n, d, in_stride, out_stride):
+            return False
+        return lib.conv_kernel_name(7, n, d) == twin_name(lib.conv_kernel_name(3, n, d))
+
+    def _keep_same_kernel(self, li, n_roll, n_train) -> bool:
+        key = (li, n_roll, n_train)
+        ok = self._keep_same.get(key)
+        if ok is None:
+            d, op = self.layers[li].desc, 0 if li == 0 else 3
+            ok = lib.conv_kernel_name(op, n_roll, d) == lib.conv_kernel_name(op, n_train, d)
+            if li == 0:
+                ok = ok and lib.conv_relu_mask_supported(n_train, d)
+            else:
+                ok = ok and lib.conv_fwd_t_supported(n_train, d) and not lib.conv_fwd_t_workspace(n_train, d)
+            self._keep_same[key] = bool(ok)
+        return self._keep_same[key]
+
+    def configure_keep(self, rows: int, T: int, n_roll: int, obs_stride: int) -> int:
+        self._keep, cfg = None, self.cfg
+        if str(getattr(cfg, "reuse_rollout_activations", "auto")) != "auto" or not _REUSE:
+            return 0
+        if int(cfg.batch_size) * int(cfg.num_batches_per_epoch) != int(rows) * int(T) or int(cfg.batch_size) % int(T):
+            return 0
+        if (self.part != "full" or self.obs_normalizer is not None or self.rnn_kind is not None or self._snap is not None or
+                getattr(cfg, "async_rl", False) or getattr(cfg, "shuffle_minibatches", False) or len(self.obs_shape) != 3):
+            return 0
+        nconv = sum(1 for L in self.layers if L.kind in FRAME_KINDS or L.kind == "conv")
+        prefix, in_stride = 0, int(obs_stride)
+        for li in range(min(3, nconv, len(self.layers) - 1)):
+            L = self.layers[li]
+            if not self._keep_rollout_ok(li, n_roll, in_stride, T * L.out_pixels * L.N):
+                break
+            prefix, in_stride = prefix + 1, T * L.out_pixels * L.N
+        if prefix == 0:
+            return 0
+        need = sum(rows * T * self.layers[li].out_pixels * (self.layers[li].N + (1 if li == 0 else 0)) * 4 for li in range(prefix))
+        free = torch.cuda.mem_get_info(self.device)[0] + sum(t.numel() * t.element_size() for k, t in self._bufs.items()
+                                                             if isinstance(k, tuple) and k and k[0] == "keep")
+        if ("train", 0) not in self._bufs:
+            free -= 2 * 4 * int(cfg.batch_size) * sum(L.out_pixels * L.N for L in self.layers if L.role != "rnn_hh")
+        if need > KEEP_MEM_SHARE * free:
+            if not getattr(self, "_keep_refused", False):
+                self._keep_refused = True
+                print(f"reuse_rollout_activations: {need / 2**30:.1f} GiB of kept activations exceed {KEEP_MEM_SHARE:.0%} of "
+                      f"the {free / 2**30:.1f} GiB of free device memory; the first minibatch recomputes them", flush=True)
+            return 0
+        for li in range(prefix):
+            L = self.layers[li]
+            self._buf(("keep", li), (rows, T, L.out_pixels * L.N))
+        self._buf(("keep", "relu_mask0"), (rows, T, self.layers[0].out_pixels), dtype=torch.int32)
+        self._keep = dict(rows=int(rows), T=int(T), prefix=prefix, n_roll=int(n_roll), obs_stride=int(obs_stride), records={})
+        return prefix
+
+    def keep_note(self, t: int, row0: int, n: int, obs_ptr: int) -> None:
+        if self._keep is not None:
+            self._keep["records"][(int(row0), int(t))] = SlotRecord(int(row0), int(row0) + int(n), int(t), self.weights_gen,
+                                                                   int(obs_ptr))
+
+    def kept_resume(self, obs, index, offset: int, n: int, T: int, epoch: int, batch_num: int):
+        kp = self._keep
+        if kp is None:
+            return None, "nothing is kept"
+        if not isinstance(obs, torch.Tensor) or obs.dim() < 2 or obs.data_ptr() % 4:
+            return None, "frames not in one aligned slab array"
+        es = obs.element_size()
+        layer_ok = [self._keep_same_kernel(li, kp["n_roll"], n) for li in range(kp["prefix"])]
+        prefix, why = reuse_prefix(epoch=epoch, batch_num=batch_num, indexed=index is not None, offset=int(offset), n=int(n),
+                                   T=int(T), keep_T=kp["T"], keep_rows=kp["rows"], records=kp["records"],
+                                   generation=self.weights_gen, obs_ptr=obs.data_ptr(), obs_row_bytes=obs.stride(0) * es,
+                                   obs_step_bytes=obs.stride(1) * es, has_normalizer=self.obs_normalizer is not None,
+                                   has_rnn=self.rnn_kind is not None, async_rl=bool(getattr(self.cfg, "async_rl", False)),
+                                   snapshot_reads=self._snap is not None, layer_ok=layer_ok)
+        if prefix == 0:
+            return None, why
+        acts = []
+        for li in range(prefix):
+            L = self.layers[li]
+            acts.append(self._bufs[("keep", li)].view(-1, L.out_pixels * L.N)[offset:offset + n].view(n * L.out_pixels, L.N))
+        P0 = self.layers[0].out_pixels
+        mask = self._bufs[("keep", "relu_mask0")].view(-1)[offset * P0:(offset + n) * P0]
+        return dict(prefix=prefix, acts=acts, mask=mask), why
+
     def _rnn_step(self, li, gx, n, rnn, tag, x_in=None, x_stride=0):
         Lh, H, S, kind = self.layers[li + 1], self.rnn_H, self.rnn_S, self.rnn_kind
         l, SL = self.layers[li].rnn_l, self.rnn_SL
diff --git a/sample_factory_amd/train.py b/sample_factory_amd/train.py
--- a/sample_factory_amd/train.py
+++ b/sample_factory_amd/train.py
@@ -244,6 +244,11 @@
                                                 tag="inf" if e == 0 else f"inf{e}")
                          for e, env in enumerate(self.envs)]
         self.sampler = self.samplers[0]
+        ac = self.learner.actor_critic
+        if not cfg.async_rl and hasattr(ac, "configure_keep") and not self.sampler.multi_key:
+            kept = ac.configure_keep(self.num_rows, int(cfg.rollout), n, self.sampler.obs.stride(0))
+            for e, sm in enumerate(self.samplers):
+                sm.keep_on, sm.keep_row0 = kept > 0, e * n
         self._prev_rows: List = [None] * E
         S = max(1, min(int(cfg.worker_num_splits), E))
         prio = -1 if (cfg.async_rl and os.environ.get("SF_ROLLOUT_PRIORITY", "0") == "1") else 0
```

Result: faster. 2.219 million, median of 6 (+3.5%).
